# protolambda/go-kzg

Measured on AMD Instinct MI355X. Metric: KZG commitments/sec (CommitToPoly, 4096-element blob); FK20 half: value_fk20_4096, higher is better.
Workload: dtype u32; 1 GPU; CommitToPoly, 4096-coeff blobs, eth/trusted_setup.json monomial setup (s=1337), 4096 blobs/step/GPU resident in HBM, fixed-base table budget 110 GB (library default 110 GB: signed 16-bit windows, 8 of them walked by both GLV halves of every scalar, 103 GB; see table_sweep); global_batch=4096, parallelism=dp1 (independent blobs, no data-path collective)

## Files before the change

### go-kzg_amd/__init__.py

```python
import ctypes as C
import os

import numpy as np

_HERE = os.path.dirname(os.path.abspath(__file__))
LIB_PATH = os.environ.get("KZG_HIP_LIB") or os.path.join(_HERE, "libkzg_hip.so")

OK, ERR_TOO_WIDE, ERR_NOT_POW2, ERR_LEN_MISMATCH, ERR_UPPER_HALF, ERR_BAD_ARG, ERR_BAD_POINT, ERR_NO_DEVICE, ERR_HIP, ERR_UNSUPPORTED, ERR_RECOVERY, ERR_BAD_BLOB = range(12)


class KzgError(Exception):

    def __init__(self, status, msg=""):
        super().__init__("kzg_hip status %d %s" % (status, msg))
        self.status = status


class KzgPanic(KzgError):
    """The reference panics (kzg.go:22-27,44-52,74-91; fk20_single.go:60-62,140-154; bls_kilic.go:133-135)."""


class NoDeviceError(KzgError):
    pass


_lib = None


def lib():
    global _lib
    if _lib is not None:
        return _lib
    if not os.path.exists(LIB_PATH):
        raise ImportError("libkzg_hip.so is not built (run __graft_entry__.build()); there is no CPU fallback: " + LIB_PATH)
    if os.environ.get("KZG_HIP_NO_TORCH_PRELOAD") != "1":
        try:
            import torch
        except ImportError:
            pass
    L = C.CDLL(LIB_PATH)
    vp, u64, i32, u32 = C.c_void_p, C.c_uint64, C.c_int, C.c_uint
    pp = C.POINTER(C.c_void_p)
    sig = {
        "kzg_hip_device_count": (i32, []), "kzg_hip_last_error": (C.c_char_p, []), "kzg_hip_version": (C.c_char_p, []),
        "kzg_hip_host_register": (i32, [vp, u64]), "kzg_hip_host_unregister": (i32, [vp]),
        "kzg_hip_fft_settings_new": (i32, [i32, u32, pp]), "kzg_hip_fft_settings_free": (None, [vp]),
        "kzg_hip_fft_max_width": (u64, [vp]), "kzg_hip_fft_roots": (i32, [vp, i32, vp]),
        "kzg_hip_fft_fr": (i32, [vp, vp, u64, i32, vp, C.POINTER(u64)]), "kzg_hip_inplace_fft_fr": (i32, [vp, vp, vp, u64, i32]),
        "kzg_hip_fft_fr_batch": (i32, [vp, vp, u64, u64, i32, vp]), "kzg_hip_fft_g1": (i32, [vp, vp, u64, i32, vp]),
        "kzg_hip_fft_g1_batch": (i32, [vp, vp, u64, u64, i32, vp]), "kzg_hip_multi_fft_g1_batch": (i32, [vp, vp, u64, u64, i32, vp]),
        "kzg_hip_das_fft_extension": (i32, [vp, vp, u64]), "kzg_hip_das_fft_extension_batch": (i32, [vp, vp, u64, u64]),
        "kzg_hip_fft_fr_batch_dev": (i32, [vp, vp, u64, u64, i32, vp, vp]), "kzg_hip_fft_g1_batch_dev": (i32, [vp, vp, u64, u64, i32, vp, vp]),
        "kzg_hip_das_fft_extension_batch_dev": (i32, [vp, vp, u64, u64, vp]),
        "kzg_hip_fr_from_le32": (i32, [vp, vp, u64, vp, C.POINTER(i32)]), "kzg_hip_fr_to_le32": (i32, [vp, vp, u64, vp]),
        "kzg_hip_lincomb_g1": (i32, [vp, vp, vp, u64, vp]),
        "kzg_hip_points_new": (i32, [vp, vp, u64, pp]), "kzg_hip_points_free": (None, [vp]), "kzg_hip_points_count": (u64, [vp]),
        "kzg_hip_points_set_table_budget_gb": (i32, [vp, C.c_double]),
        "kzg_hip_lincomb_points": (i32, [vp, vp, u64, vp]), "kzg_hip_lincomb_points_batch": (i32, [vp, vp, u64, u64, vp]),
        "kzg_hip_lincomb_points_batch_dev": (i32, [vp, vp, u64, u64, vp, vp]), "kzg_hip_g1_to_compressed": (i32, [vp, vp, u64, vp]),
        "kzg_hip_g1_from_compressed": (i32, [vp, vp, u64, vp]), "kzg_hip_g1_mul_vec": (i32, [vp, vp, vp, u64, vp]),
        "kzg_hip_generate_testing_setup_g1": (i32, [vp, vp, u64, vp]),
        "kzg_hip_g1_marshal_text": (i32, [vp, vp, u64, vp]), "kzg_hip_g1_unmarshal_text": (i32, [vp, C.c_char_p, u64, vp]),
        "kzg_hip_trusted_setup_from_json": (i32, [vp, C.c_char_p, u64, vp, vp, u64, C.POINTER(u64), C.POINTER(u64)]),
        "kzg_hip_kzg_set_table_budget_gb": (i32, [vp, C.c_double]),
        "kzg_hip_kzg_settings_new": (i32, [vp, vp, u64, pp]), "kzg_hip_kzg_settings_free": (None, [vp]),
        "kzg_hip_commit_to_poly": (i32, [vp, vp, u64, vp]), "kzg_hip_commit_to_poly_batch": (i32, [vp, vp, u64, u64, vp]),
        "kzg_hip_commit_to_poly_batch_dev": (i32, [vp, vp, u64, u64, vp, vp]),
        "kzg_hip_compute_proof_single": (i32, [vp, vp, u64, u64, vp]),
        "kzg_hip_compute_proof_single_batch": (i32, [vp, vp, u64, u64, vp, vp]),
        "kzg_hip_compute_proof_single_batch_dev": (i32, [vp, vp, u64, u64, vp, vp, vp]),
        "kzg_hip_compute_proof_multi": (i32, [vp, vp, u64, u64, u64, vp]),
        "kzg_hip_check_proof_multi_interpolation": (i32, [vp, vp, u64, vp, vp, vp]),
        "kzg_hip_g2_from_compressed": (i32, [vp, vp, u64, vp]), "kzg_hip_pairings_verify_batch": (i32, [vp, vp, vp, vp, vp, u64, vp]),
        "kzg_hip_g2_mul_generator_vec": (i32, [vp, vp, u64, vp]), "kzg_hip_generate_testing_setup_g2": (i32, [vp, vp, u64, vp]),
        "kzg_hip_g2_to_compressed": (i32, [vp, vp, u64, vp]),
        "kzg_hip_trusted_setup_g2_from_json": (i32, [vp, C.c_char_p, u64, vp, u64, C.POINTER(u64)]),
        "kzg_hip_test_g2_table_builds": (i32, [vp, C.POINTER(u64)]),
        "kzg_hip_kzg_set_secret_g2": (i32, [vp, vp, u64]), "kzg_hip_check_proof_single_batch": (i32, [vp, vp, vp, vp, vp, u64, vp]),
        "kzg_hip_check_proof_multi_batch": (i32, [vp, vp, vp, vp, vp, u64, u64, vp]),
        "kzg_hip_check_proof_single_batch_combined": (i32, [vp, vp, vp, vp, vp, u64, vp, vp]),
        "kzg_hip_eth_verify_kzg_proof_batch_combined": (i32, [vp, vp, vp, vp, vp, u64, vp, vp]),
        "kzg_hip_test_combine_points": (i32, [vp, vp, vp, vp, vp, u64, vp, vp, vp]), "kzg_hip_test_combine_stats": (i32, [C.POINTER(u64)]),
        "kzg_hip_eth_set_setup_g2": (i32, [vp, vp, u64]), "kzg_hip_eth_verify_kzg_proof_batch": (i32, [vp, vp, vp, vp, vp, u64, vp]),
        "kzg_hip_eth_verify_aggregate_kzg_proof_batch": (i32, [vp, vp, vp, vp, vp, u64, vp, vp, vp, vp]),
        "kzg_hip_eth_kzg_to_versioned_hash_batch": (i32, [vp, vp, u64, vp]), "kzg_hip_eth_kzg_to_versioned_hash_batch_dev": (i32, [vp, vp, u64, vp]),
        "kzg_hip_eth_point_evaluation_precompile_batch": (i32, [vp, vp, u64, vp]),
        "kzg_hip_eth_point_evaluation_precompile_batch_dev": (i32, [vp, vp, u64, vp]),
        "kzg_hip_eth_precompile_return_value": (i32, [vp, vp]),
        "kzg_hip_eth_verify_kzg_commitments_against_transactions_batch": (i32, [vp, vp, vp, vp, vp, vp, u64, vp]),
        "kzg_hip_test_sha256_lanes": (i32, [vp, vp, vp, vp, u64, vp]), "kzg_hip_test_hash_to_bls_field_lanes": (i32, [vp, vp, u64, vp]),
        "kzg_hip_pairing_test": (i32, [vp, vp, vp, u64, vp]),
        "kzg_hip_pairing_test_wave": (i32, [vp, vp, vp, u64, vp]), "kzg_hip_test_wave_fp12_op": (i32, [vp, i32, vp, vp, u64, vp]),
        "kzg_hip_test_pairing_route": (i32, [u64, C.POINTER(u64)]),
        "kzg_hip_toeplitz_part2": (i32, [vp, vp, vp, u64, vp]), "kzg_hip_toeplitz_part3": (i32, [vp, vp, u64, vp]),
        "kzg_hip_fk20_single_settings_new": (i32, [vp, u64, pp]), "kzg_hip_fk20_single_settings_free": (None, [vp]),
        "kzg_hip_fk20_single_x_ext_fft": (i32, [vp, vp]), "kzg_hip_fk20_single": (i32, [vp, vp, u64, vp]),
        "kzg_hip_fk20_single_batch": (i32, [vp, vp, u64, u64, vp]), "kzg_hip_fk20_single_batch_dev": (i32, [vp, vp, u64, u64, vp, vp]),
        "kzg_hip_fk20_single_da_optimized": (i32, [vp, vp, u64, vp]), "kzg_hip_da_using_fk20": (i32, [vp, vp, u64, vp]),
        "kzg_hip_da_using_fk20_batch": (i32, [vp, vp, u64, u64, vp]), "kzg_hip_da_using_fk20_batch_dev": (i32, [vp, vp, u64, u64, vp, vp]),
        "kzg_hip_fk20_multi_settings_new": (i32, [vp, u64, u64, pp]), "kzg_hip_fk20_multi_settings_free": (None, [vp]),
        "kzg_hip_fk20_multi": (i32, [vp, vp, u64, vp]), "kzg_hip_fk20_multi_da_optimized": (i32, [vp, vp, u64, vp]),
        "kzg_hip_da_using_fk20_multi": (i32, [vp, vp, u64, vp]),
        "kzg_hip_da_using_fk20_multi_batch_dev": (i32, [vp, vp, u64, u64, vp, vp]),
        "kzg_hip_fk20_multi_hext_slice_dev": (i32, [vp, vp, u64, u64, u64, vp, vp]),
        "kzg_hip_fk20_multi_finish_dev": (i32, [vp, vp, i32, vp, vp]),
        "kzg_hip_eth_settings_new": (i32, [vp, vp, u64, pp]), "kzg_hip_eth_settings_free": (None, [vp]),
        "kzg_hip_eth_blob_to_kzg_commitment_batch": (i32, [vp, vp, u64, vp, vp]),
        "kzg_hip_eth_compute_kzg_proof": (i32, [vp, vp, u64, vp, vp, vp]),
        "kzg_hip_eth_compute_kzg_proof_batch": (i32, [vp, vp, u64, u64, vp, vp, vp, vp]),
        "kzg_hip_eth_compute_kzg_proof_batch_dev": (i32, [vp, vp, u64, u64, vp, vp, vp, vp, vp]),
        "kzg_hip_eth_compute_aggregate_kzg_proof": (i32, [vp, vp, u64, vp, vp]),
        "kzg_hip_eth_compute_aggregate_kzg_proof_batch": (i32, [vp, vp, vp, u64, vp, vp, vp]),
        "kzg_hip_eth_compute_aggregate_kzg_proof_batch_dev": (i32, [vp, vp, vp, u64, vp, vp, vp]),
        "kzg_hip_test_eth_prove_chunks": (u64, []),
        "kzg_hip_eth_compute_aggregated_poly_and_commitment": (i32, [vp, vp, vp, u64, vp, vp, vp, vp]),
        "kzg_hip_test_sha256": (None, [vp, u64, vp]),
        "kzg_hip_evaluate_poly_in_evaluation_form": (i32, [vp, vp, u64, vp, u32, vp]),
        "kzg_hip_eth_evaluate_polynomial_in_evaluation_form": (i32, [vp, vp, u64, vp, vp]),
        "kzg_hip_bench_threads_fft_fr": (i32, [vp, vp, u64, u64, u32, u32, vp, C.POINTER(C.c_double)]),
        "kzg_hip_bench_drop_in_eth_proof": (i32, [vp, vp, u64, u64, u32, u32, vp, C.POINTER(C.c_double)]),
        "kzg_hip_zero_poly_via_multiplication": (i32, [vp, vp, u64, u64, vp, vp]),
        "kzg_hip_recover_poly_from_samples": (i32, [vp, vp, vp, u64, vp]),
        "kzg_hip_recover_poly_from_samples_batch": (i32, [vp, vp, vp, u64, u64, u64, vp, vp]),
        "kzg_hip_recover_poly_from_samples_batch_dev": (i32, [vp, vp, vp, u64, u64, u64, vp, vp, vp]),
        "kzg_hip_zero_poly_via_multiplication_batch": (i32, [vp, vp, vp, u64, u64, vp, vp, vp]),
        "kzg_hip_calibrate": (i32, [vp, C.POINTER(C.c_double), C.POINTER(C.c_double), C.POINTER(C.c_double)]),
        "kzg_hip_bench_drop_in": (i32, [vp, i32, vp, u64, u64, u32, u32, vp, C.POINTER(C.c_double)]),
        "kzg_hip_coalesce_stats": (i32, [vp, i32, C.POINTER(u64)]),
        "kzg_hip_lincomb_promotions": (i32, [vp, C.POINTER(u64), C.POINTER(u64)]),
        "kzg_hip_test_fp_inv": (i32, [vp, vp, u64, vp, vp, C.POINTER(C.c_double), C.POINTER(C.c_double)]),
        "kzg_hip_test_fr_inv": (i32, [vp, vp, u64, vp, vp, vp]),
        "kzg_hip_test_g1_fft_plan": (i32, [vp, u64, u64, u64, i32, vp]),
        "kzg_hip_test_g1_fft_stage": (i32, [vp, vp, u64, u64, u64, i32, i32, i32, i32, vp, vp]),
        "kzg_hip_test_g1_fft_direct": (i32, [vp, vp, u64, u64, u64, i32, u32, i32, u64, vp]),
        "kzg_hip_kzg_table_info": (i32, [vp, C.POINTER(C.c_uint32), C.POINTER(C.c_uint32), C.POINTER(u64)]), "kzg_hip_kzg_table_additions": (u32, [vp]), "kzg_hip_kzg_set_projective_outputs": (i32, [vp, i32]),
        "kzg_hip_da_using_fk20_multi_batch": (i32, [vp, vp, u64, u64, vp]),
        "kzg_hip_multi_settings_new": (i32, [C.POINTER(i32), u32, u32, vp, u64, pp]), "kzg_hip_multi_settings_free": (None, [vp]),
        "kzg_hip_multi_device_count": (u32, [vp]), "kzg_hip_multi_device": (i32, [vp, u32]),
        "kzg_hip_multi_fft": (vp, [vp, u32]), "kzg_hip_multi_kzg": (vp, [vp, u32]),
        "kzg_hip_multi_transport": (C.c_char_p, [vp]), "kzg_hip_multi_transport_note": (C.c_char_p, [vp]), "kzg_hip_multi_transport_check": (C.c_char_p, [vp]), "kzg_hip_multi_exchanges": (u64, [vp]),
        "kzg_hip_multi_set_fft_sharding": (i32, [vp, i32]), "kzg_hip_multi_set_table_budget_gb": (i32, [vp, C.c_double]),
        "kzg_hip_multi_commit_to_poly_batch": (i32, [vp, vp, u64, u64, vp]),
        "kzg_hip_multi_compute_proof_single_batch": (i32, [vp, vp, u64, u64, vp, vp]),
        "kzg_hip_multi_fft_fr_batch": (i32, [vp, vp, u64, u64, i32, vp]), "kzg_hip_multi_das_fft_extension_batch": (i32, [vp, vp, u64, u64]),
        "kzg_hip_multi_eth_settings_new": (i32, [vp, vp, u64, pp]), "kzg_hip_multi_eth_settings_free": (None, [vp]),
        "kzg_hip_multi_eth_blob_to_kzg_commitment_batch": (i32, [vp, vp, u64, vp, vp]),
        "kzg_hip_multi_eth_compute_kzg_proof_batch": (i32, [vp, vp, u64, u64, vp, vp, vp, vp]),
        "kzg_hip_multi_fk20_single_settings_new": (i32, [vp, u64, pp]), "kzg_hip_multi_fk20_single_settings_free": (None, [vp]),
        "kzg_hip_multi_da_using_fk20_batch": (i32, [vp, vp, u64, u64, vp]), "kzg_hip_multi_da_using_fk20": (i32, [vp, vp, u64, vp]),
        "kzg_hip_multi_fk20_multi_settings_new": (i32, [vp, u64, u64, pp]), "kzg_hip_multi_fk20_multi_settings_free": (None, [vp]),
        "kzg_hip_multi_da_using_fk20_multi_batch": (i32, [vp, vp, u64, u64, vp]), "kzg_hip_multi_da_using_fk20_multi": (i32, [vp, vp, u64, vp]),
        "kzg_hip_bench_poly_lincomb_dev": (i32, [vp, vp, u64, vp, u64, u64, vp, vp]),
        "kzg_hip_prof_reset": (None, [vp, i32]), "kzg_hip_prof_read": (i32, [vp, C.c_char_p, C.POINTER(C.c_double), C.POINTER(u64)]),
    }
    for name, (res, args) in sig.items():
        if os.environ.get("KZG_HIP_LIB_ALLOW_MISSING") and not hasattr(L, name):
            continue
        f = getattr(L, name)
        f.restype, f.argtypes = res, args
    _lib = L
    return L


API_SYMBOLS = None


def device_count():
    return lib().kzg_hip_device_count()


class pinned:

    def __init__(self, array):
        self.a = array

    def __enter__(self):
        _chk(lib().kzg_hip_host_register(self.a.ctypes.data, self.a.nbytes))
        return self.a

    def __exit__(self, *exc):
        lib().kzg_hip_host_unregister(self.a.ctypes.data)
        return False


_ERR_STATUS = (ERR_TOO_WIDE, ERR_NOT_POW2)


def _chk(st, error_ok=False):
    if st == OK:
        return
    msg = ""
    if st == ERR_HIP:
        msg = lib().kzg_hip_last_error().decode()
    if st == ERR_NO_DEVICE:
        raise NoDeviceError(st, "no gfx950 device visible (the HIP path is the only path)")
    if error_ok and st in _ERR_STATUS:
        raise KzgError(st, msg)
    raise KzgPanic(st, msg)


def _p(a):
    return a.ctypes.data_as(C.c_void_p)


def _fr(a):
    a = np.ascontiguousarray(a, dtype=np.uint64)
    return a.reshape(-1, 4)


def _g1(a):
    a = np.ascontiguousarray(a, dtype=np.uint64)
    return a.reshape(-1, 3, 6)


def _g2(a):
    a = np.ascontiguousarray(a, dtype=np.uint64)
    return a.reshape(-1, 3, 2, 6)


def _seed32(seed):
    if seed is None:
        return None
    seed = bytes(seed)
    if len(seed) != 32:
        raise KzgError(ERR_LEN_MISMATCH, "a seed is 32 bytes")
    return C.c_char_p(seed)


def combine_stats():
    out = (C.c_uint64 * 6)()
    _chk(lib().kzg_hip_test_combine_stats(out))
    return {"route": "combined" if out[0] else "per_row", "groups": int(out[1]), "failed": int(out[2]), "rechecked": int(out[3]),
            "combine_from": int(out[4]), "rows": int(out[5])}


def pairing_route(n):
    out = (C.c_uint64 * 2)()
    _chk(lib().kzg_hip_test_pairing_route(n, out))
    return ("wave" if out[0] else "lane"), int(out[1])


def g2_empty(n):
    return np.zeros((n, 3, 2, 6), dtype=np.uint64)


def fr_empty(n):
    return np.zeros((n, 4), dtype=np.uint64)


def g1_empty(n):
    return np.zeros((n, 3, 6), dtype=np.uint64)


class FFTSettings:

    def __init__(self, max_scale, device=0):
        h = C.c_void_p()
        _chk(lib().kzg_hip_fft_settings_new(device, max_scale, C.byref(h)))
        self.h, self.max_scale, self.max_width, self.device = h, max_scale, 1 << max_scale, device

    def close(self):
        if getattr(self, "h", None):
            lib().kzg_hip_fft_settings_free(self.h)
            self.h = None

    def expanded_roots_of_unity(self):
        out = fr_empty(self.max_width + 1)
        _chk(lib().kzg_hip_fft_roots(self.h, 0, _p(out)))
        return out

    def reverse_roots_of_unity(self):
        out = fr_empty(self.max_width + 1)
        _chk(lib().kzg_hip_fft_roots(self.h, 1, _p(out)))
        return out

    def fft(self, vals, inv=False):
        vals = _fr(vals)
        n = vals.shape[0]
        if n > self.max_width:
            raise KzgError(ERR_TOO_WIDE)
        np2 = 1 if n == 0 else 1 << (n - 1).bit_length()
        out, on = fr_empty(np2), C.c_uint64(0)
        _chk(lib().kzg_hip_fft_fr(self.h, _p(vals), n, int(inv), _p(out), C.byref(on)), error_ok=True)
        return out

    def inplace_fft(self, vals, inv=False):
# ... 889 lines not shown
```

### go-kzg_amd/csrc/capi_core.hip

```cpp
#include "capi_common.hpp"
#include <map>

thread_local std::string g_last_error;


int kzg_hip_device_count(void) {
    int n = 0;
    if (hipGetDeviceCount(&n) != hipSuccess) return 0;
    int ok = 0;
    for (int i = 0; i < n; i++) {
        hipDeviceProp_t pr;
        if (hipGetDeviceProperties(&pr, i) == hipSuccess && strncmp(pr.gcnArchName, "gfx950", 6) == 0) ok++;
    }
    return ok;
}
const char *kzg_hip_last_error(void) { return g_last_error.c_str(); }
const char *kzg_hip_version(void) { return "kzg_hip 0.1 (gfx950)"; }

static fr scale2_root_of_unity(unsigned k) {
    uint32_t e[8]; uint32_t br = 0;
    for (int i = 0; i < 8; i++) e[i] = subb(FrP::mod(i), i == 0 ? 1u : 0u, br);
    for (unsigned s = 0; s < k; s++)
        for (int i = 0; i < 8; i++) e[i] = (e[i] >> 1) | (i < 7 ? e[i + 1] << 31 : 0);
    fr seven = fr_from_u64(7), acc = one<FrP>();
// ... 207 lines not shown
uint32_t g1_fft_direct_logr(uint64_t n, uint64_t batch) {
    if (const knobs::g1_fft_mode forced = knobs::g1_fft(); forced != knobs::g1_fft_mode::by_size) return forced == knobs::g1_fft_mode::direct ? 4u : 0u;
    if (n < 2) return 0;
    const uint64_t unit = device_simd_lanes() / 16;
    if (g1_quad_enabled()) return n * batch <= unit ? 4 : 0;
    if (n * batch <= 2 * unit) return 4;
    if (n * batch <= 4 * unit) return 3;
    return 0;
}
bool g1_fft_direct_mode(uint64_t n, uint64_t batch) { return g1_fft_direct_logr(n, batch) != 0; }
int g1_fft_direct_lanes(uint64_t n, uint64_t batch) {
    if (!g1_quad_enabled() || !knobs::g1_direct_coop()) return 1;
    const uint64_t items = (n * batch) << g1_fft_direct_logr(n, batch);
    const uint64_t one_round = device_simd_lanes();
    return items * 4 <= one_round ? 4 : items * 2 <= one_round ? 2 : 1;
}
int g1_fft_rows(kzg_hip_fft *fs, hipStream_t s, const g1j *d_in, uint64_t in_stride, uint64_t n_valid, g1j *d_data, uint64_t n, uint64_t batch, int inv,
                       const fr *scale, uint64_t n_out) {
    if (g1_fft_direct_mode(n, batch)) {
        dtmp<g1j> d_tmp(s);
        CHK(d_tmp.alloc(n * batch));
        launch_g1_fft_direct(s, d_in, in_stride, n_valid, d_data, d_tmp.p, n, batch, inv ? fs->d_reversed : fs->d_expanded, fs->W, scale, g1_fft_direct_logr(n, batch),
                             g1_fft_direct_lanes(n, batch), 0, n_out);
        return KZG_HIP_OK;
    }
    launch_g1_bitrev_copy(s, d_in, in_stride, n_valid, d_data, n, batch);
    const fr *roots = inv ? fs->d_glv_reversed : fs->d_glv_expanded;
    const int8_t *wnaf = inv ? fs->d_wnaf_reversed : fs->d_wnaf_expanded;
    for (uint64_t m = 1; m < n; m <<= 1) launch_g1_fft_stage(s, d_data, n, batch, m, roots, wnaf, fs->W);
    if (scale) launch_g1_mul_vec(s, d_data, n * batch, scale, 0, n * batch, d_data);
    return KZG_HIP_OK;
}

int kzg_hip_fft_g1(kzg_hip_fft *fs, const void *vals_g1, uint64_t n, int inv, void *out_g1) {
    if (!fs) return KZG_HIP_ERR_BAD_ARG;
    if (n > fs->W) return KZG_HIP_ERR_TOO_WIDE;
    if (!is_pow2(n)) return KZG_HIP_ERR_NOT_POW2;
    if (n == 0 || !vals_g1 || !out_g1) return KZG_HIP_ERR_BAD_ARG;
    stream_lease lease(fs);
    hipStream_t s = lease.s;
    dtmp<g1j> d_in(s), d_data(s);
    CHK(d_in.alloc(n)); CHK(d_data.alloc(n));
    HIPCHK(hipMemcpyAsync(d_in.p, vals_g1, n * sizeof(g1j), hipMemcpyHostToDevice, s));
    launch_g1_from_kilic(s, d_in.p, n);
    CHK(g1_fft_rows(fs, s, d_in.p, n, n, d_data.p, n, 1, inv, inv ? fs->d_inv_pow2 + ilog2(n) : nullptr));
    launch_g1_normalize(s, d_data.p, d_in.p, n, true);
    std::swap(d_in.p, d_data.p);
    HIPCHK(hipGetLastError());
    HIPCHK(hipMemcpyAsync(out_g1, d_data.p, n * sizeof(g1j), hipMemcpyDeviceToHost, s));
    HIPCHK(hipStreamSynchronize(s));
    return KZG_HIP_OK;
}

int das_ext_rows(kzg_hip_fft *fs, hipStream_t s, fr *d, uint64_t n, uint64_t batch) {
    const bool long_or_short = n >= fr4::N || n <= 64;
    if (2 * n == fs->W && long_or_short && fr_fft_lazy_sizes(n, batch) && fs->d_tw4096[0]) {
        dtmp<fr> d_c(s);
        CHK(d_c.alloc(n * batch));
        fr_fft_rows(fs, s, d, n, n, d_c.p, n, batch, 1);
        launch_fr_mul_table_rows(s, d_c.p, fs->d_expanded, 1, n, batch);
        fr_fft_rows(fs, s, d_c.p, n, n, d, n, batch, 0);
        return KZG_HIP_OK;
    }
    launch_das_ext(s, d, n, batch, fs->d_expanded, fs->d_reversed, fs->W, fs->d_inv_pow2 + ilog2(n), fs->d_tw_das2048);
    return KZG_HIP_OK;
}

int kzg_hip_das_fft_extension_batch(kzg_hip_fft *fs, void *vals_fr, uint64_t n, uint64_t batch) {
    if (!fs || !vals_fr) return KZG_HIP_ERR_BAD_ARG;
    if (n * 2 > fs->W) return KZG_HIP_ERR_TOO_WIDE;
    if (n < 2 || !is_pow2(n)) return KZG_HIP_ERR_BAD_ARG;
    if (!batch) return KZG_HIP_OK;
    stream_lease lease(fs);
    hipStream_t s = lease.s;
    void *dp = nullptr;
    uint8_t *hp = n <= 4096 ? lease.pinned(n * batch * sizeof(fr), &dp) : nullptr;
    if (hp) {
        memcpy(hp, vals_fr, n * batch * sizeof(fr));
        CHK(das_ext_rows(fs, s, (fr *)dp, n, batch));
        HIPCHK(hipGetLastError());
        HIPCHK(hipStreamSynchronize(s));
        memcpy(vals_fr, hp, n * batch * sizeof(fr));
        return KZG_HIP_OK;
    }
    dtmp<fr> d(s);
    CHK(d.alloc(n * batch));
    HIPCHK(hipMemcpyAsync(d.p, vals_fr, n * batch * sizeof(fr), hipMemcpyHostToDevice, s));
    CHK(das_ext_rows(fs, s, d.p, n, batch));
    HIPCHK(hipGetLastError());
    HIPCHK(hipMemcpyAsync(vals_fr, d.p, n * batch * sizeof(fr), hipMemcpyDeviceToHost, s));
    HIPCHK(hipStreamSynchronize(s));
    return KZG_HIP_OK;
}
int kzg_hip_fft_fr_batch_dev(kzg_hip_fft *fs, const void *d_vals_fr, uint64_t n, uint64_t batch, int inv, void *d_out_fr, void *stream) {
    if (!fs) return KZG_HIP_ERR_BAD_ARG;
    if (n > fs->W) return KZG_HIP_ERR_TOO_WIDE;
    if (!is_pow2(n)) return KZG_HIP_ERR_NOT_POW2;
    if (n == 0 || batch == 0) return KZG_HIP_OK;
    if (!d_vals_fr || !d_out_fr) return KZG_HIP_ERR_BAD_ARG;
    dev_select sel(fs);
    fr_fft_rows(fs, (hipStream_t)stream, (const fr *)d_vals_fr, n, n, (fr *)d_out_fr, n, batch, inv);
    HIPCHK(hipGetLastError());
    return KZG_HIP_OK;
}
int kzg_hip_fft_g1_batch(kzg_hip_fft *fs, const void *vals_g1, uint64_t n, uint64_t batch, int inv, void *out_g1) {
    if (!fs) return KZG_HIP_ERR_BAD_ARG;
    if (n > fs->W) return KZG_HIP_ERR_TOO_WIDE;
    if (!is_pow2(n)) return KZG_HIP_ERR_NOT_POW2;
    if (n == 0 || !vals_g1 || !out_g1) return KZG_HIP_ERR_BAD_ARG;
    if (!batch) return KZG_HIP_OK;
    stream_lease lease(fs);
    hipStream_t s = lease.s;
    dtmp<g1j> d_in(s), d_data(s);
    CHK(d_in.alloc(n * batch)); CHK(d_data.alloc(n * batch));
    HIPCHK(hipMemcpyAsync(d_in.p, vals_g1, n * batch * sizeof(g1j), hipMemcpyHostToDevice, s));
    launch_g1_from_kilic(s, d_in.p, n * batch);
    CHK(g1_fft_rows(fs, s, d_in.p, n, n, d_data.p, n, batch, inv, inv ? fs->d_inv_pow2 + ilog2(n) : nullptr));
    launch_g1_normalize(s, d_data.p, d_in.p, n * batch, true);
    HIPCHK(hipGetLastError());
    HIPCHK(hipMemcpyAsync(out_g1, d_in.p, n * batch * sizeof(g1j), hipMemcpyDeviceToHost, s));
    HIPCHK(hipStreamSynchronize(s));
    return KZG_HIP_OK;
}
int kzg_hip_fft_g1_batch_dev(kzg_hip_fft *fs, const void *d_vals_g1, uint64_t n, uint64_t batch, int inv, void *d_out_g1, void *stream) {
    if (!fs) return KZG_HIP_ERR_BAD_ARG;
    if (n > fs->W) return KZG_HIP_ERR_TOO_WIDE;
    if (!is_pow2(n)) return KZG_HIP_ERR_NOT_POW2;
    if (n == 0 || !d_vals_g1 || !d_out_g1) return KZG_HIP_ERR_BAD_ARG;
    if (!batch) return KZG_HIP_OK;
    dev_select sel(fs);
    hipStream_t s = (hipStream_t)stream;
    dtmp<g1j> d_in(s), d_data(s);
    CHK(d_in.alloc(n * batch)); CHK(d_data.alloc(n * batch));
    HIPCHK(hipMemcpyAsync(d_in.p, d_vals_g1, n * batch * sizeof(g1j), hipMemcpyDeviceToDevice, s));
    launch_g1_from_kilic(s, d_in.p, n * batch);
    CHK(g1_fft_rows(fs, s, d_in.p, n, n, d_data.p, n, batch, inv, inv ? fs->d_inv_pow2 + ilog2(n) : nullptr));
    launch_g1_normalize(s, d_data.p, (g1j *)d_out_g1, n * batch, true);
    HIPCHK(hipGetLastError());
    return KZG_HIP_OK;
}
static void put_stage_plan(const g1_stage_plan &p, uint32_t *out) { out[0] = (uint32_t)p.lanes; out[1] = p.wnaf ? 1u : 0u; out[2] = p.rows ? 1u : 0u; }
static bool g1_stage_shape_ok(kzg_hip_fft *fs, uint64_t n, uint64_t batch, uint64_t m) {
    return n >= 2 && n <= fs->W && is_pow2(n) && m >= 1 && m <= n / 2 && is_pow2(m) && batch >= 1 && batch <= (1ull << 32) / n;
}
int kzg_hip_test_g1_fft_plan(kzg_hip_fft *fs, uint64_t n, uint64_t batch, uint64_t m, int dif, uint32_t out[5]) {
    if (!fs || !out || !g1_stage_shape_ok(fs, n, batch, m)) return KZG_HIP_ERR_BAD_ARG;
    dev_select sel(fs);
    put_stage_plan(g1_fft_stage_plan(n, batch, m, dif != 0), out);
    out[3] = g1_fft_direct_logr(n, batch);
    out[4] = (uint32_t)g1_fft_direct_lanes(n, batch);
    return KZG_HIP_OK;
}
int kzg_hip_test_g1_fft_stage(kzg_hip_fft *fs, const void *pts_g1, uint64_t n, uint64_t batch, uint64_t m, int inv, int dif, int lanes, int mul, void *out_g1, uint32_t plan_out[3]) {
    if (!fs || !pts_g1 || !out_g1 || !g1_stage_shape_ok(fs, n, batch, m)) return KZG_HIP_ERR_BAD_ARG;
    if ((lanes != 0 && lanes != 1 && lanes != 2 && lanes != 4) || mul < 0 || mul > 2) return KZG_HIP_ERR_BAD_ARG;
    stream_lease lease(fs);
    hipStream_t s = lease.s;
    const g1_stage_plan plan = g1_fft_stage_plan(n, batch, m, dif != 0, lanes == 0 ? -1 : lanes == 1 ? 0 : lanes == 4 ? 1 : 2,
                                                 mul == 1 ? knobs::g1_mul_mode::regular : mul == 2 ? knobs::g1_mul_mode::wnaf : knobs::g1_mul_mode::by_shape);
    if (plan_out) put_stage_plan(plan, plan_out);
    dtmp<g1j> d_data(s), d_out(s);
    CHK(d_data.alloc(n * batch)); CHK(d_out.alloc(n * batch));
    HIPCHK(hipMemcpyAsync(d_data.p, pts_g1, n * batch * sizeof(g1j), hipMemcpyHostToDevice, s));
    launch_g1_from_kilic(s, d_data.p, n * batch);
    launch_g1_fft_stage_planned(s, plan, dif != 0, d_data.p, n, batch, m, inv ? fs->d_glv_reversed : fs->d_glv_expanded, inv ? fs->d_wnaf_reversed : fs->d_wnaf_expanded, fs->W);
    launch_g1_normalize(s, d_data.p, d_out.p, n * batch, true);
    HIPCHK(hipGetLastError());
    HIPCHK(hipMemcpyAsync(out_g1, d_out.p, n * batch * sizeof(g1j), hipMemcpyDeviceToHost, s));
    HIPCHK(hipStreamSynchronize(s));
    return KZG_HIP_OK;
}
int kzg_hip_test_g1_fft_direct(kzg_hip_fft *fs, const void *pts_g1, uint64_t n, uint64_t n_valid, uint64_t batch, int inv, uint32_t max_logr, int lanes, uint64_t n_out, void *out_g1) {
    if (!fs || !pts_g1 || !out_g1 || n < 2 || n > fs->W || !is_pow2(n) || !n_valid || n_valid > n || n_out > n || batch < 1 || batch > (1ull << 28) / n) return KZG_HIP_ERR_BAD_ARG;
    if (max_logr < 1 || max_logr > 4 || (lanes != 1 && lanes != 2 && lanes != 4)) return KZG_HIP_ERR_BAD_ARG;
    stream_lease lease(fs);
    hipStream_t s = lease.s;
    dtmp<g1j> d_in(s), d_data(s), d_tmp(s), d_out(s);
    CHK(d_in.alloc(n_valid * batch)); CHK(d_data.alloc(n * batch)); CHK(d_tmp.alloc(n * batch)); CHK(d_out.alloc(n * batch));
    HIPCHK(hipMemcpyAsync(d_in.p, pts_g1, n_valid * batch * sizeof(g1j), hipMemcpyHostToDevice, s));
    launch_g1_from_kilic(s, d_in.p, n_valid * batch);
    HIPCHK(hipMemsetAsync(d_data.p, 0, n * batch * sizeof(g1j), s));
    launch_g1_fft_direct(s, d_in.p, n_valid, n_valid, d_data.p, d_tmp.p, n, batch, inv ? fs->d_reversed : fs->d_expanded, fs->W, inv ? fs->d_inv_pow2 + ilog2(n) : nullptr, max_logr,
                         lanes, 0, n_out, true);
    launch_g1_normalize(s, d_data.p, d_out.p, n * batch, true);
    HIPCHK(hipGetLastError());
    HIPCHK(hipMemcpyAsync(out_g1, d_out.p, n * batch * sizeof(g1j), hipMemcpyDeviceToHost, s));
    HIPCHK(hipStreamSynchronize(s));
    return KZG_HIP_OK;
}
int kzg_hip_das_fft_extension_batch_dev(kzg_hip_fft *fs, void *d_vals_fr, uint64_t n, uint64_t batch, void *stream) {
    if (!fs || !d_vals_fr) return KZG_HIP_ERR_BAD_ARG;
    if (n * 2 > fs->W) return KZG_HIP_ERR_TOO_WIDE;
    if (n < 2 || !is_pow2(n)) return KZG_HIP_ERR_BAD_ARG;
    if (!batch) return KZG_HIP_OK;
    dev_select sel(fs);
    CHK(das_ext_rows(fs, (hipStream_t)stream, (fr *)d_vals_fr, n, batch));
    HIPCHK(hipGetLastError());
    return KZG_HIP_OK;
}
int kzg_hip_das_fft_extension(kzg_hip_fft *fs, void *vals_fr, uint64_t n) { return kzg_hip_das_fft_extension_batch(fs, vals_fr, n, 1); }

msm_plan classic_plan(uint64_t n, bool folded) {
    msm_plan p{};
    p.c = 8; p.nwin = 16; p.nb = 128; p.ngroups = folded ? 8 : 16; p.fixed = 0; p.table_n = n;
    return p;
}
void set_inf_image(void *out_g1) { g1j z = g1_to_kilic(g1_inf()); memcpy(out_g1, &z, sizeof z); }

__global__ __launch_bounds__(128, 2) void k_points_shift64(const g1a *pts, uint64_t n, g1j *out) {
    uint64_t t = blockIdx.x * (uint64_t)blockDim.x + threadIdx.x;
    if (t >= n) return;
    g1a p = pts[t];
    if (is_inf(p)) { out[t] = g1_inf(); return; }
    g1jq q = g1jq_unpack(to_jac(p));
#pragma nounroll
    for (int i = 0; i < 64; i++) q = g1jq_dbl(q);
    out[t] = g1jq_pack(q);
}
void kzg_hip_points_free(kzg_hip_points *pts) {
    if (!pts) return;
    hipSetDevice(pts->fs->device);
    hipDeviceSynchronize();
    pts->co.reset();
    if (pts->ks) kzg_hip_kzg_settings_free(pts->ks);
    hipFree(pts->d_tab);
    (void)hipGetLastError();
    delete pts;
}
int kzg_hip_points_new(kzg_hip_fft *fs, const void *points_g1, uint64_t n, kzg_hip_points **out) {
    if (!fs || !out || (n && !points_g1)) return KZG_HIP_ERR_BAD_ARG;
    *out = nullptr;
    KZG_TRY
    std::unique_ptr<kzg_hip_points, void (*)(kzg_hip_points *)> own(new kzg_hip_points, kzg_hip_points_free);
    own->fs = fs; own->n = n;
    if (n) {
        dev_guard g(fs);
        hipStream_t s = fs->stream;
        dtmp<g1j> d_raw(s), d_hi(s);
        CHK(d_raw.alloc(n)); CHK(d_hi.alloc(n));
        HIPCHK(hipMalloc((void **)&own->d_tab, 2 * n * sizeof(g1a)));
        HIPCHK(hipMemcpyAsync(d_raw.p, points_g1, n * sizeof(g1j), hipMemcpyHostToDevice, s));
        launch_g1_from_kilic(s, d_raw.p, n);
        launch_g1_to_affine(s, d_raw.p, own->d_tab, n);
        hipLaunchKernelGGL(k_points_shift64, dim3((uint32_t)((n + 127) / 128)), dim3(128), 0, s, own->d_tab, n, d_hi.p);
        launch_g1_to_affine(s, d_hi.p, own->d_tab + n, n);
        HIPCHK(hipGetLastError());
        HIPCHK(hipStreamSynchronize(s));
    }
    if (n >= 64) {
        CHK(kzg_settings_build(fs, points_g1, n, &own->ks));
        own->ks->budget_gb = table_budget_gb(knobs::points_fb_budget_gb(), 32.0, 24.0);
    }
    *out = own.release();
    return KZG_HIP_OK;
    KZG_CATCH
}
int kzg_hip_points_set_table_budget_gb(kzg_hip_points *pts, double gb) {
    if (!pts) return KZG_HIP_ERR_BAD_ARG;
    if (!pts->ks) return KZG_HIP_OK;
    return kzg_hip_kzg_set_table_budget_gb(pts->ks, gb);
}
uint64_t kzg_hip_points_count(const kzg_hip_points *pts) { return pts ? pts->n : 0; }
int lincomb_points_rows(kzg_hip_points *pts, hipStream_t s, const fr *d_sc, uint64_t n, uint64_t batch, g1j *d_out, uint64_t sc_stride, bool holds_mu) {
    if (pts->ks) {
        if (holds_mu) CHK(ensure_fixed_table(pts->ks, s));
        else { dev_guard g(pts->fs); CHK(ensure_fixed_table(pts->ks, s)); }
        std::shared_lock<std::shared_mutex> tl(pts->ks->tab_mu);
        if (pts->ks->d_fixed) return commit_rows(pts->ks, s, d_sc, n, batch, d_out, sc_stride ? sc_stride : n);
    }
    msm_plan p = classic_plan(pts->n, true);
    if (!msm_index_range_ok(p, n)) return KZG_HIP_ERR_TOO_WIDE;
    dtmp<uint8_t> d_ws(s);
    CHK(d_ws.alloc(msm_workspace_bytes(p, n, batch)));
    launch_msm(s, p, pts->d_tab, d_sc, sc_stride ? sc_stride : n, n, batch, d_ws.p, d_out, true);
    HIPCHK(hipGetLastError());
    return KZG_HIP_OK;
}
int kzg_hip_lincomb_points_batch_dev(kzg_hip_points *pts, const void *d_scalars_fr, uint64_t n, uint64_t batch, void *d_out_g1, void *stream) {
    if (!pts || !d_out_g1) return KZG_HIP_ERR_BAD_ARG;
    if (n > pts->n) return KZG_HIP_ERR_LEN_MISMATCH;
    if (!batch) return KZG_HIP_OK;
    if (n == 0 || !d_scalars_fr) return KZG_HIP_ERR_BAD_ARG;
    hipSetDevice(pts->fs->device);
    return lincomb_points_rows(pts, (hipStream_t)stream, (const fr *)d_scalars_fr, n, batch, (g1j *)d_out_g1);
}
int kzg_hip_lincomb_points_batch(kzg_hip_points *pts, const void *scalars_fr, uint64_t n, uint64_t batch, void *out_g1) {
    if (!pts || !out_g1) return KZG_HIP_ERR_BAD_ARG;
    if (n > pts->n) return KZG_HIP_ERR_LEN_MISMATCH;
    if (!batch) return KZG_HIP_OK;
    if (n == 0) { for (uint64_t b = 0; b < batch; b++) set_inf_image((uint8_t *)out_g1 + b * sizeof(g1j)); return KZG_HIP_OK; }
    if (!scalars_fr) return KZG_HIP_ERR_BAD_ARG;
    stream_lease lease(pts->fs);
    hipStream_t s = lease.s;
    dtmp<fr> d_sc(s); dtmp<g1j> d_out(s);
    CHK(d_sc.alloc(n * batch)); CHK(d_out.alloc(batch));
    HIPCHK(hipMemcpyAsync(d_sc.p, scalars_fr, n * batch * sizeof(fr), hipMemcpyHostToDevice, s));
    CHK(lincomb_points_rows(pts, s, d_sc.p, n, batch, d_out.p, 0, lease.fallback.owns_lock()));
    HIPCHK(hipMemcpyAsync(out_g1, d_out.p, batch * sizeof(g1j), hipMemcpyDeviceToHost, s));
    HIPCHK(hipStreamSynchronize(s));
    return KZG_HIP_OK;
}
int kzg_hip_lincomb_points(kzg_hip_points *pts, const void *scalars_fr, uint64_t n, void *out_g1) {
    if (pts && scalars_fr && out_g1 && n && n <= pts->n) return lincomb_points_coalesced(pts, scalars_fr, n, out_g1);
    return kzg_hip_lincomb_points_batch(pts, scalars_fr, n, 1, out_g1);
}

struct lincomb_promo {
    static constexpr int SLOTS = 6, LINCOMB_PROMO_SETS = 2;
    struct entry {
        uint64_t n = 0, fp = 0, last_use = 0; uint32_t sightings = 0;
        std::shared_ptr<const std::vector<uint8_t>> copy;
        std::shared_ptr<kzg_hip_points> set;
        bool building = false;
    };
    std::mutex mu; std::condition_variable built;
    entry e[SLOTS];
    uint64_t tick = 0, promoted = 0;
    std::atomic<uint64_t> served{0};
// ... 204 lines not shown
```

### go-kzg_amd/csrc/capi_fk20.hip

```cpp
#include "capi_common.hpp"

__global__ void k_fk20_x(const g1j *secret, uint64_t n, uint64_t l, uint64_t k, g1j *x ) {
    uint64_t t = blockIdx.x * (uint64_t)blockDim.x + threadIdx.x;
    if (t >= l * k) return;
    uint64_t off = t / k, i = t % k;
    x[t] = (i + 1 < k) ? secret[n - l - 1 - off - i * l] : g1_inf();
}

static int fk20_core_new(kzg_hip_kzg *ks, uint64_t n2, uint64_t l, fk20_core *c) {
    kzg_hip_fft *fs = ks->fs;
    dev_guard g(fs);
    hipStream_t s = fs->stream;
    uint64_t n = n2 / 2, k = n / l, k2 = 2 * k;
    c->ks = ks; c->n2 = n2; c->l = l; c->k = k;
    dtmp<g1j> d_x(s), d_f(s);
    CHK(d_x.alloc(l * k)); CHK(d_f.alloc(l * k2));
    HIPCHK(hipMalloc((void **)&c->d_files, l * k2 * sizeof(g1j)));
    hipLaunchKernelGGL(k_fk20_x, dim3((uint32_t)((l * k + 255) / 256)), dim3(256), 0, s, ks->d_secret, n, l, k, d_x.p);
    CHK(g1_fft_rows(fs, s, d_x.p, k, k, d_f.p, k2, l, 0));
    launch_g1_normalize(s, d_f.p, c->d_files, l * k2);
    HIPCHK(hipGetLastError());
    {
        double budget_gb = table_budget_gb(knobs::fk20_fb_budget_gb(), 48.0, 12.0);
        uint64_t npts = l * k2;
        const bool glv = fb_glv_enabled();
        dtmp<g1a> d_fa(s);
        if (npts >= 64) { CHK(d_fa.alloc(npts)); launch_g1_to_affine(s, c->d_files, d_fa.p, npts); }
        for (uint32_t cc = glv ? 16 : 14; cc >= 4 && npts >= 64; cc--) {
            const uint32_t nwin = glv ? fb_windows_glv(cc) : fb_windows(cc);
            if (glv && cc > 4 && fb_windows_glv(cc - 1) == nwin) continue;
            double bytes = (double)nwin * (double)npts * (double)(1u << (cc - 1)) * sizeof(g1a);
            if (bytes > budget_gb * 1e9) continue;
            g1a *tab = nullptr;
            if (hipMalloc((void **)&tab, (size_t)nwin * npts * (1u << (cc - 1)) * sizeof(g1a)) != hipSuccess) { (void)hipGetLastError(); continue; }
            hipError_t e = launch_fb_build(s, d_fa.p, npts, cc, nwin, tab);
            if (e == hipSuccess) e = hipStreamSynchronize(s);
            if (e != hipSuccess) { (void)hipGetLastError(); hipFree(tab); continue; }
            c->d_files_fb = tab; c->fb_c = cc; c->fb_nwin = nwin; c->fb_glv = glv;
            break;
        }
    }
    HIPCHK(hipStreamSynchronize(s));
    return KZG_HIP_OK;
}

int fk20_hext(fk20_core *c, hipStream_t s, const fr *d_poly, uint64_t poly_stride, uint64_t n, uint64_t batch, uint64_t j0, uint64_t cnt, g1j *d_hext) {
    kzg_hip_fft *fs = c->ks->fs;
    uint64_t l = c->l, k2 = 2 * c->k;
    dtmp<fr> d_tc(s), d_cf(s);
    CHK(d_tc.alloc(batch * l * k2)); CHK(d_cf.alloc(batch * l * k2));
    launch_toeplitz_coeffs(s, d_poly, poly_stride, n, l, batch, d_tc.p, fs->d_inv_pow2 + ilog2(k2));
    fr_fft_rows(fs, s, d_tc.p, k2, k2, d_cf.p, k2, batch * l, 0);
    if (c->d_files_fb) {
        if (l == 1) launch_fb_mul_vec(s, c->d_files_fb, l * k2, c->fb_c, c->fb_nwin, d_cf.p, k2, j0, cnt, batch, d_hext, c->fb_glv);
        else if (batch * cnt >= device_simd_lanes()) launch_fb_mul_vec_files(s, c->d_files_fb, l * k2, c->fb_c, c->fb_nwin, d_cf.p, k2, j0, cnt, batch, d_hext, c->fb_glv);
        else {
            dtmp<g1j> d_tmp(s);
            CHK(d_tmp.alloc(batch * l * cnt));
            launch_fb_mul_vec(s, c->d_files_fb, l * k2, c->fb_c, c->fb_nwin, d_cf.p, k2, j0, cnt, batch, d_tmp.p, c->fb_glv);
            launch_g1_sum_files(s, d_tmp.p, l, cnt, batch, d_hext);
        }
    } else if (l == 1 && j0 == 0 && cnt == k2) launch_g1_mul_vec(s, c->d_files, k2, d_cf.p, 1, batch * k2, d_hext);
    else HIPCHK(launch_g1_file_msm(s, c->d_files, d_cf.p, l, k2, j0, cnt, batch, d_hext));
    HIPCHK(hipGetLastError());
    return KZG_HIP_OK;
}
static int fk20_finish_from_h(fk20_core *c, hipStream_t s, g1j *d_h, uint64_t batch, int da, int bit_reverse, g1j *d_out) {
    kzg_hip_fft *fs = c->ks->fs;
    uint64_t k = c->k, k2 = 2 * k, on = da ? k2 : k;
    dtmp<g1j> d_b(s);
    CHK(d_b.alloc(batch * k2));
    CHK(g1_fft_rows(fs, s, d_h, k2, k, d_b.p, on, batch, 0));
    if (bit_reverse) { launch_g1_bitrev_copy(s, d_b.p, on, on, d_h, on, batch); launch_g1_normalize(s, d_h, d_out, batch * on, true); }
    else launch_g1_normalize(s, d_b.p, d_out, batch * on, true);
    HIPCHK(hipGetLastError());
    return KZG_HIP_OK;
}
int fk20_finish(fk20_core *c, hipStream_t s, const g1j *d_hext, uint64_t batch, int da, int bit_reverse, g1j *d_out) {
    kzg_hip_fft *fs = c->ks->fs;
    const uint64_t k2 = 2 * c->k;
    dtmp<g1j> d_a(s);
    CHK(d_a.alloc(batch * k2));
    CHK(g1_fft_rows(fs, s, d_hext, k2, k2, d_a.p, k2, batch, 1, nullptr, c->k));
    return fk20_finish_from_h(c, s, d_a.p, batch, da, bit_reverse, d_out);
}
static bool fk20_pass1_fused_ok(const fk20_core *c, uint64_t batch) {
    const uint64_t k2 = 2 * c->k;
    return knobs::fk20_pass1() && c->l == 1 && c->d_files_fb && k2 >= 32 && g1_fft_direct_mode(k2, batch) && g1_fft_direct_logr(k2, batch) == 4;
}
static int fk20_run_pass1_fused(fk20_core *c, hipStream_t s, const fr *d_poly, uint64_t poly_stride, uint64_t n, uint64_t batch, int da, int bit_reverse, g1j *d_out) {
    kzg_hip_fft *fs = c->ks->fs;
    const uint64_t k2 = 2 * c->k;
    dtmp<fr> d_tc(s), d_cf(s); dtmp<g1j> d_p1(s), d_a(s), d_tmp(s);
    CHK(d_tc.alloc(batch * k2)); CHK(d_cf.alloc(batch * k2)); CHK(d_p1.alloc(batch * k2)); CHK(d_a.alloc(batch * k2)); CHK(d_tmp.alloc(batch * k2));
    launch_toeplitz_coeffs(s, d_poly, poly_stride, n, 1, batch, d_tc.p, fs->d_inv_pow2 + ilog2(k2));
    fr_fft_rows(fs, s, d_tc.p, k2, k2, d_cf.p, k2, batch, 0);
    launch_fb_direct_pass1(s, c->d_files_fb, k2, c->fb_c, c->fb_nwin, d_cf.p, fs->d_reversed, fs->W, batch, 4, d_p1.p, c->fb_glv);
    launch_g1_fft_direct(s, d_p1.p, k2, k2, d_a.p, d_tmp.p, k2, batch, fs->d_reversed, fs->W, nullptr, 4, g1_fft_direct_lanes(k2, batch), 4, c->k);
    HIPCHK(hipGetLastError());
    return fk20_finish_from_h(c, s, d_a.p, batch, da, bit_reverse, d_out);
}
static bool fk20_fused_ok(const fk20_core *c, uint64_t batch, int da) {
    const uint64_t k2 = 2 * c->k;
    return knobs::fk20_fuse() && c->l == 1 && c->d_files_fb && k2 >= 8 && !g1_fft_direct_mode(k2, batch) && (da || !g1_fft_direct_mode(c->k, batch));
}
static int fk20_run_fused(fk20_core *c, hipStream_t s, const fr *d_poly, uint64_t poly_stride, uint64_t n, uint64_t batch, int da, int bit_reverse, g1j *d_out) {
    kzg_hip_fft *fs = c->ks->fs;
    const uint64_t k2 = 2 * c->k;
    dtmp<fr> d_tc(s), d_cf(s); dtmp<g1j> d_a(s), d_b(s);
    CHK(d_tc.alloc(batch * k2)); CHK(d_cf.alloc(batch * k2)); CHK(d_a.alloc(batch * k2)); CHK(d_b.alloc(batch * k2));
    launch_toeplitz_coeffs(s, d_poly, poly_stride, n, 1, batch, d_tc.p, fs->d_inv_pow2 + ilog2(k2));
    fr_fft_rows(fs, s, d_tc.p, k2, k2, d_cf.p, k2, batch, 0);
    launch_fb_mul_vec_dif2(s, c->d_files_fb, k2, c->fb_c, c->fb_nwin, d_cf.p, fs->d_reversed, fs->W, batch, d_a.p, c->fb_glv);
    for (uint64_t m = k2 / 8; m >= 1; m >>= 1) launch_g1_fft_stage_dif(s, d_a.p, k2, batch, m, fs->d_glv_reversed, fs->d_wnaf_reversed, fs->W);
    if (!da) {
        const uint64_t k = c->k;
        launch_g1_take_even(s, d_a.p, d_b.p, batch * k);
        for (uint64_t m = 1; m < k; m <<= 1) launch_g1_fft_stage(s, d_b.p, k, batch, m, fs->d_glv_expanded, fs->d_wnaf_expanded, fs->W);
        if (bit_reverse) { launch_g1_bitrev_copy(s, d_b.p, k, k, d_a.p, k, batch); launch_g1_normalize(s, d_a.p, d_out, batch * k, true); }
        else launch_g1_normalize(s, d_b.p, d_out, batch * k, true);
        HIPCHK(hipGetLastError());
        return KZG_HIP_OK;
    }
    launch_g1_clear_odd(s, d_a.p, batch * k2);
    for (uint64_t m = 1; m < k2; m <<= 1) launch_g1_fft_stage(s, d_a.p, k2, batch, m, fs->d_glv_expanded, fs->d_wnaf_expanded, fs->W);
    if (bit_reverse) { launch_g1_bitrev_copy(s, d_a.p, k2, k2, d_b.p, k2, batch); launch_g1_normalize(s, d_b.p, d_out, batch * k2, true); }
    else launch_g1_normalize(s, d_a.p, d_out, batch * k2, true);
    HIPCHK(hipGetLastError());
    return KZG_HIP_OK;
}
static uint64_t fk20_padded_batch(uint64_t batch) {
    if (!knobs::fk20_pad()) return batch;
    if (batch > 16 && batch < 32) return 32;
    if (batch > 32 && (batch & 7)) {
        const uint64_t p = (batch + 7) & ~7ull;
        if ((p - batch) * 32 <= batch) return p;
    }
    return batch;
}
int fk20_run_dev(fk20_core *c, hipStream_t s, const fr *d_poly, uint64_t poly_stride, uint64_t n, uint64_t batch, int da, int bit_reverse, g1j *d_out) {
    if (const uint64_t padded = fk20_padded_batch(batch); padded != batch) {
        const uint64_t on = da ? 2 * c->k : c->k;
        dtmp<fr> d_p2(s); dtmp<g1j> d_o2(s);
        CHK(d_p2.alloc(padded * n)); CHK(d_o2.alloc(padded * on));
        HIPCHK(hipMemcpy2DAsync(d_p2.p, n * sizeof(fr), d_poly, poly_stride * sizeof(fr), n * sizeof(fr), batch, hipMemcpyDeviceToDevice, s));
        for (uint64_t b = batch; b < padded; b++)
            HIPCHK(hipMemcpyAsync(d_p2.p + b * n, d_poly + (batch - 1) * poly_stride, n * sizeof(fr), hipMemcpyDeviceToDevice, s));
        if (fk20_fused_ok(c, padded, da)) CHK(fk20_run_fused(c, s, d_p2.p, n, n, padded, da, bit_reverse, d_o2.p));
        else {
            dtmp<g1j> d_hext(s);
            CHK(d_hext.alloc(padded * 2 * c->k));
            CHK(fk20_hext(c, s, d_p2.p, n, n, padded, 0, 2 * c->k, d_hext.p));
            CHK(fk20_finish(c, s, d_hext.p, padded, da, bit_reverse, d_o2.p));
        }
        HIPCHK(hipMemcpyAsync(d_out, d_o2.p, batch * on * sizeof(g1j), hipMemcpyDeviceToDevice, s));
        return KZG_HIP_OK;
    }
    if (fk20_fused_ok(c, batch, da)) return fk20_run_fused(c, s, d_poly, poly_stride, n, batch, da, bit_reverse, d_out);
    if (fk20_pass1_fused_ok(c, batch)) return fk20_run_pass1_fused(c, s, d_poly, poly_stride, n, batch, da, bit_reverse, d_out);
    uint64_t k2 = 2 * c->k;
    dtmp<g1j> d_hext(s);
    CHK(d_hext.alloc(batch * k2));
    CHK(fk20_hext(c, s, d_poly, poly_stride, n, batch, 0, k2, d_hext.p));
    return fk20_finish(c, s, d_hext.p, batch, da, bit_reverse, d_out);
}
static int fk20_run_host(fk20_core *c, const void *poly_fr, uint64_t row_len, uint64_t n, uint64_t batch, int check_upper, int da, int bit_reverse, void *out_g1) {
    kzg_hip_fft *fs = c->ks->fs;
    dev_guard g(fs);
    hipStream_t s = fs->stream;
    uint64_t on = da ? 2 * c->k : c->k;
    dtmp<fr> d_poly(s); dtmp<g1j> d_out(s); dtmp<uint32_t> d_flag(s);
    CHK(d_poly.alloc(batch * row_len)); CHK(d_out.alloc(batch * on)); CHK(d_flag.alloc(1));
    HIPCHK(hipMemcpyAsync(d_poly.p, poly_fr, batch * row_len * sizeof(fr), hipMemcpyHostToDevice, s));
    if (check_upper) {
        HIPCHK(hipMemsetAsync(d_flag.p, 0, 4, s));
        launch_fr_any_nonzero(s, d_poly.p + n, row_len - n, d_flag.p);
        uint32_t flag = 0;
        HIPCHK(hipMemcpyAsync(&flag, d_flag.p, 4, hipMemcpyDeviceToHost, s));
        HIPCHK(hipStreamSynchronize(s));
        if (flag) return KZG_HIP_ERR_UPPER_HALF;
    }
    CHK(fk20_run_dev(c, s, d_poly.p, row_len, n, batch, da, bit_reverse, d_out.p));
    return d2h_staged(c->ks->fs, s, out_g1, d_out.p, batch * on * sizeof(g1j));
}

int kzg_hip_fk20_single_settings_new(kzg_hip_kzg *ks, uint64_t n2, kzg_hip_fk20s **out) {
    if (!ks || !out) return KZG_HIP_ERR_BAD_ARG;
    *out = nullptr;
    if (n2 > ks->fs->W) return KZG_HIP_ERR_TOO_WIDE;
    if (!is_pow2(n2)) return KZG_HIP_ERR_NOT_POW2;
    if (n2 < 2) return KZG_HIP_ERR_BAD_ARG;
    kzg_hip_fk20s *fk = new kzg_hip_fk20s;
    int st = fk20_core_new(ks, n2, 1, &fk->c);
    if (st) { kzg_hip_fk20_single_settings_free(fk); return st; }
    *out = fk;
    return KZG_HIP_OK;
}
void kzg_hip_fk20_single_settings_free(kzg_hip_fk20s *fk) {
    if (!fk) return;
    if (fk->c.ks) { hipSetDevice(fk->c.ks->fs->device); hipDeviceSynchronize(); }
    hipFree(fk->c.d_files); hipFree(fk->c.d_files_fb);
    (void)hipGetLastError();
    delete fk;
}
int kzg_hip_fk20_single_x_ext_fft(const kzg_hip_fk20s *fk, void *out_g1) {
    if (!fk || !out_g1) return KZG_HIP_ERR_BAD_ARG;
    kzg_hip_fft *fs = fk->c.ks->fs;
    dev_guard g(fs);
    hipStream_t s = fs->stream;
    dtmp<g1j> d_tmp(s);
    CHK(d_tmp.alloc(fk->c.n2));
    launch_g1_normalize(s, fk->c.d_files, d_tmp.p, fk->c.n2, true);
    HIPCHK(hipGetLastError());
    HIPCHK(hipMemcpyAsync(out_g1, d_tmp.p, fk->c.n2 * sizeof(g1j), hipMemcpyDeviceToHost, s));
    HIPCHK(hipStreamSynchronize(s));
    return KZG_HIP_OK;
}
int kzg_hip_fk20_single(kzg_hip_fk20s *fk, const void *poly_fr, uint64_t n, void *out_g1) {
    if (!fk || !poly_fr || !out_g1) return KZG_HIP_ERR_BAD_ARG;
    if (2 * n != fk->c.n2) return KZG_HIP_ERR_LEN_MISMATCH;
    return fk20_run_host(&fk->c, poly_fr, n, n, 1, 0, 0, 0, out_g1);
}
int kzg_hip_fk20_single_batch(kzg_hip_fk20s *fk, const void *poly_fr, uint64_t n, uint64_t batch, void *out_g1) {
    if (!fk || !poly_fr || !out_g1) return KZG_HIP_ERR_BAD_ARG;
    if (2 * n != fk->c.n2) return KZG_HIP_ERR_LEN_MISMATCH;
    if (!batch) return KZG_HIP_OK;
    return fk20_run_host(&fk->c, poly_fr, n, n, batch, 0, 0, 0, out_g1);
}
int kzg_hip_fk20_single_batch_dev(kzg_hip_fk20s *fk, const void *d_poly_fr, uint64_t n, uint64_t batch, void *d_out_g1, void *stream) {
    if (!fk || !d_poly_fr || !d_out_g1) return KZG_HIP_ERR_BAD_ARG;
    if (2 * n != fk->c.n2) return KZG_HIP_ERR_LEN_MISMATCH;
    if (!batch) return KZG_HIP_OK;
    dev_guard g(fk->c.ks->fs);
    return fk20_run_dev(&fk->c, (hipStream_t)stream, (const fr *)d_poly_fr, n, n, batch, 0, 0, (g1j *)d_out_g1);
}
int kzg_hip_fk20_single_da_optimized(kzg_hip_fk20s *fk, const void *poly_fr, uint64_t n2, void *out_g1) {
    if (!fk || !poly_fr || !out_g1) return KZG_HIP_ERR_BAD_ARG;
    if (n2 > fk->c.ks->fs->W) return KZG_HIP_ERR_TOO_WIDE;
    if (!is_pow2(n2)) return KZG_HIP_ERR_NOT_POW2;
    if (n2 != fk->c.n2) return KZG_HIP_ERR_LEN_MISMATCH;
    return fk20_run_host(&fk->c, poly_fr, n2, n2 / 2, 1, 1, 1, 0, out_g1);
}
int kzg_hip_da_using_fk20_batch(kzg_hip_fk20s *fk, const void *poly_fr, uint64_t n, uint64_t batch, void *out_g1) {
    if (!fk || !poly_fr || !out_g1) return KZG_HIP_ERR_BAD_ARG;
    if (n > fk->c.ks->fs->W / 2) return KZG_HIP_ERR_TOO_WIDE;
    if (!is_pow2(n)) return KZG_HIP_ERR_NOT_POW2;
    if (2 * n != fk->c.n2) return KZG_HIP_ERR_LEN_MISMATCH;
    if (!batch) return KZG_HIP_OK;
    return fk20_run_host(&fk->c, poly_fr, n, n, batch, 0, 1, 1, out_g1);
}
static int fk20_da_coalesced(fk20_core *c, const void *poly_fr, uint64_t n, void *out_g1) {
    KZG_TRY
    const uint64_t on = 2 * c->k;
    coalescer *co = get_coalescer(c->ks->fs, c->co_da, n * sizeof(fr), on * sizeof(g1j), 48);
    auto exec = [c, co, n, on](coalesce_buf &b, uint64_t batch) -> int {
        hipSetDevice(c->ks->fs->device);
        hipStream_t s = b.stream;
        drain_on_exit drain(s);
        dtmp<fr> d_poly(s); dtmp<g1j> d_out(s);
// ... 101 lines not shown
```

### go-kzg_amd/csrc/g1_coop_kernels.hpp

```cpp
#pragma once
#include "internal.hpp"
#include "g1_quad.hpp"

namespace kzg {

#ifndef G1_BLOCK
#define G1_BLOCK 256
#endif
struct g1jq_slot { uint32_t w[39]; uint32_t inf; uint32_t pad; };
#define G1_DIRECT_BLOCK 64

template <bool DIF, bool WNAF, int L> __global__ __launch_bounds__(G1_BLOCK, 2) void k_g1_fft_stage_quad(g1j *data, uint32_t logn, uint64_t m, const fr *roots, const int8_t *wnaf, uint64_t W, uint64_t total, uint64_t batch) {
    const uint64_t t4 = blockIdx.x * (uint64_t)blockDim.x + threadIdx.x;
    const uint32_t role = (uint32_t)(t4 & (uint64_t)(L - 1));
    const uint64_t t = t4 / L;
    if (t >= total) return;
    const uint64_t half = 1ull << (logn - 1), groups = half / m;
    const uint64_t j = t / (groups * batch), rem = t % (groups * batch), b = rem / groups, g = rem % groups;
    g1j *row = data + (b << logn);
    const uint64_t i0 = g * 2 * m + j, i1 = i0 + m;
    g1j y = row[i1];
    g1j x = row[i0];
    const uint64_t ti = j * (W / (2 * m));
    const fr kk = roots[ti];
    glv_halves h;
#pragma unroll
    for (int i = 0; i < 4; i++) { h.k1[i] = kk.l[i]; h.k2[i] = kk.l[4 + i]; }
    h.neg1 = h.neg2 = 0;
    g1aq tbl[8]; fq dz[7]; g1j packed;
#define QMUL(pq, res) (WNAF ? g1_mul_glv_wnaf_quad<L>((pq), kk, tbl, dz, wnaf + ti * KZG_WNAF_ROW, (res), packed, role) : g1_mul_glv_regular_quad<L>((pq), h, tbl, dz, (res), packed, role))
    if (!DIF) {
        g1jq yq; int st = is_inf(y) ? 0 : 1;
        if (st == 1) {
            if (j) {
                st = QMUL(g1jq_unpack(y), yq);
                if (st == 2) y = packed; else if (st == 0) y = g1_inf();
            } else yq = g1jq_unpack(y);
        }
        if (st == 1 && !is_inf(x)) {
            g1jq sum, dif;
            if (KZG_LIKELY(g1jq_addsub(g1jq_unpack(x), yq, sum, dif))) {
                if (role == 0) {
                    fp z3 = packq(sum.z);
                    g1j o0, o1;
                    o0.x = packq(sum.x); o0.y = packq(sum.y); o0.z = z3;
                    o1.x = packq(dif.x); o1.y = packq(dif.y); o1.z = z3;
                    row[i0] = o0; row[i1] = o1;
                }
                return;
            }
        }
        if (st == 1) y = g1jq_pack(yq);
        if (role == 0) { row[i0] = g1_add(x, y); row[i1] = g1_add(x, g1_neg(y)); }
    } else {
        if (!is_inf(x) && !is_inf(y)) {
            g1jq sum, dif;
            if (KZG_LIKELY(g1jq_addsub(g1jq_unpack(x), g1jq_unpack(y), sum, dif))) {
                g1j o0; o0.x = packq(sum.x); o0.y = packq(sum.y); o0.z = packq(sum.z);
                g1j o1;
                if (j) {
                    g1jq dq;
                    const int st = QMUL(dif, dq);
                    o1 = st == 1 ? g1jq_pack(dq) : st == 2 ? packed : g1_inf();
                } else { o1.x = packq(dif.x); o1.y = packq(dif.y); o1.z = o0.z; }
                if (role == 0) { row[i0] = o0; row[i1] = o1; }
                return;
            }
        }
        g1j s_ = g1_add(x, y), d_ = g1_add(x, g1_neg(y));
        if (j && !is_inf(d_)) {
            g1jq dq;
            const int st = QMUL(g1jq_unpack(d_), dq);
            d_ = st == 1 ? g1jq_pack(dq) : st == 2 ? packed : g1_inf();
        }
        if (role == 0) { row[i0] = s_; row[i1] = d_; }
    }
}
#undef QMUL
template <bool DIF> static inline void launch_stage_coop(hipStream_t s, int lanes, bool wn, g1j *data, uint64_t n, uint64_t batch, uint64_t m, const fr *roots, const int8_t *wnaf, uint64_t W,
                                                  uint64_t total) {
    static const bool once = [] {
        hipFuncSetAttribute(reinterpret_cast<const void *>(&k_g1_fft_stage_quad<DIF, true, 4>), hipFuncAttributeMaxDynamicSharedMemorySize, 96 * 1024);
        hipFuncSetAttribute(reinterpret_cast<const void *>(&k_g1_fft_stage_quad<DIF, false, 4>), hipFuncAttributeMaxDynamicSharedMemorySize, 96 * 1024);
        hipFuncSetAttribute(reinterpret_cast<const void *>(&k_g1_fft_stage_quad<DIF, true, 2>), hipFuncAttributeMaxDynamicSharedMemorySize, 96 * 1024);
        hipFuncSetAttribute(reinterpret_cast<const void *>(&k_g1_fft_stage_quad<DIF, false, 2>), hipFuncAttributeMaxDynamicSharedMemorySize, 96 * 1024);
        return true; }();
    (void)once;
    const size_t lds = total * lanes <= device_simd_lanes() ? 96 * 1024 : 0;
    const dim3 qg((uint32_t)((lanes * total + G1_BLOCK - 1) / G1_BLOCK));
    const uint32_t logn = ilog2(n);
    if (lanes == 4) {
        if (wn) hipLaunchKernelGGL((k_g1_fft_stage_quad<DIF, true, 4>), qg, dim3(G1_BLOCK), lds, s, data, logn, m, roots, wnaf, W, total, batch);
        else hipLaunchKernelGGL((k_g1_fft_stage_quad<DIF, false, 4>), qg, dim3(G1_BLOCK), lds, s, data, logn, m, roots, wnaf, W, total, batch);
    } else {
        if (wn) hipLaunchKernelGGL((k_g1_fft_stage_quad<DIF, true, 2>), qg, dim3(G1_BLOCK), lds, s, data, logn, m, roots, wnaf, W, total, batch);
        else hipLaunchKernelGGL((k_g1_fft_stage_quad<DIF, false, 2>), qg, dim3(G1_BLOCK), lds, s, data, logn, m, roots, wnaf, W, total, batch);
    }
}
template <int L> __global__ __launch_bounds__(G1_DIRECT_BLOCK, 2) void k_g1_fft_direct_coop(const g1j *in, uint64_t in_stride, uint64_t n_valid, g1j *out, uint32_t logn,
                                                                                          uint32_t logR, uint64_t Ns, const fr *roots, uint64_t W, const fr *scale, uint64_t total,
                                                                                          uint32_t logT, uint32_t logU) {
    __shared__ g1jq_slot buf[G1_DIRECT_BLOCK / L];
    const uint32_t tid = threadIdx.x, role = tid & (uint32_t)(L - 1), item = tid / L;
    const uint64_t t = (blockIdx.x * (uint64_t)blockDim.x + tid) / L;
    const uint64_t n = 1ull << logn, R = 1ull << logR, cols = n >> logR, T = 1ull << logT;
    const uint32_t tt = (uint32_t)(t & (T - 1));
    const uint64_t u = (t >> logT) & ((1ull << logU) - 1), jb = t >> (logT + logU), j = jb % cols, b = jb / cols;
    const bool live = t < total;
    g1jq_acc acc; acc.inf = true;
    uint64_t oidx = 0;
    if (live) {
        const uint64_t k = j & (Ns - 1), idx = j + (uint64_t)tt * cols;
        oidx = b * n + (j - k) * R + k + u * Ns;
        g1j x = idx < n_valid ? in[b * in_stride + idx] : g1_inf();
        if (!is_inf(x)) {
            const uint64_t e = ((uint64_t)tt * (cols / Ns) * (Ns * u + k)) & (n - 1);
            if (e == 0 && !scale) { acc.v = g1jq_unpack(x); acc.inf = false; }
            else {
                fr sc = roots[e * (W >> logn)];
                if (scale) sc = mul(sc, *scale);
                g1aq tbl[8]; fq dz[7]; g1j packed;
                const int st = g1_mul_glv_regular_quad<L>(g1jq_unpack(x), glv_split_signed(from_mont<FrP>(sc)), tbl, dz, acc.v, packed, role);
                if (st == 2) { acc.inf = is_inf(packed); if (!acc.inf) acc.v = g1jq_unpack(packed); } else acc.inf = st == 0;
            }
        }
    }
#define COOP_STORE(i) do { _Pragma("unroll") for (int q = 0; q < 13; q++) { buf[i].w[q] = acc.v.x.l[q]; buf[i].w[13 + q] = acc.v.y.l[q]; buf[i].w[26 + q] = acc.v.z.l[q]; } \
                           buf[i].inf = acc.inf ? 1u : 0u; } while (0)
    if (role == 0) COOP_STORE(item);
    __syncthreads();
#pragma nounroll
    for (uint32_t off = (uint32_t)T / 2; off >= 1; off >>= 1) {
        if (role == 0 && tt < off && !buf[item + off].inf) {
            g1jq q;
#pragma unroll
            for (int i = 0; i < 13; i++) { q.x.l[i] = buf[item + off].w[i]; q.y.l[i] = buf[item + off].w[13 + i]; q.z.l[i] = buf[item + off].w[26 + i]; }
            acc.add(q);
            COOP_STORE(item);
        }
        __syncthreads();
    }
#undef COOP_STORE
    if (live && role == 0 && tt == 0) out[oidx] = acc.inf ? g1_inf() : g1jq_pack(acc.v);
}

}
```

### go-kzg_amd/csrc/internal.hpp

```cpp
#pragma once
#include <hip/hip_runtime.h>
#include <stdint.h>
#include "field.hpp"
#include "g1.hpp"
#include "knobs.hpp"

namespace kzg {

inline uint32_t ilog2(uint64_t v) { uint32_t r = 0; while ((1ull << r) < v) r++; return r; }

void launch_fr_fft(hipStream_t s, const fr *in, uint64_t in_stride, uint64_t n_in, fr *out, uint64_t n, uint64_t batch,
                   const fr *roots, uint64_t W, const fr *scale, const uint32_t *tw4096 = nullptr, const fr *roots_l = nullptr);
bool fr_fft_lazy_sizes(uint64_t n, uint64_t batch);
void launch_das_ext(hipStream_t s, fr *vals, uint64_t n, uint64_t batch, const fr *expanded, const fr *reversed, uint64_t W,
                    const fr *inv_n, const uint32_t *tw2048 = nullptr);
void launch_toeplitz_coeffs(hipStream_t s, const fr *poly, uint64_t poly_stride, uint64_t n, uint64_t l, uint64_t batch, fr *out,
                            const fr *scale);
void launch_quotient_linear(hipStream_t s, const fr *poly, uint64_t poly_stride, uint64_t n, uint64_t batch, const fr *x, fr *q, uint64_t q_stride);
void launch_fr_from_u64(hipStream_t s, const uint64_t *in, uint64_t in_stride, fr *out, uint64_t n);
void launch_fr_zero_tails(hipStream_t s, fr *rows, uint64_t n_max, uint64_t batch, const uint64_t *lens, uint64_t lens_stride);
void launch_fr_any_nonzero(hipStream_t s, const fr *vals, uint64_t n, uint32_t *flag);
void launch_fr_powers(hipStream_t s, const fr *base, uint64_t n, fr *out);

void launch_fr_from_le32(hipStream_t s, const uint8_t *in, fr *out, uint64_t per_blob, uint64_t batch, uint32_t *bad);
void launch_fr_to_le32(hipStream_t s, const fr *in, uint8_t *out, uint64_t n);
void launch_fr_bitrev_gather(hipStream_t s, const fr *in, fr *out, uint64_t n);
constexpr uint64_t ZERO_TREE_LEAF = 16;
void launch_zero_leaves(hipStream_t s, const fr *expanded, uint64_t stride, const uint64_t *missing, uint64_t n_missing, uint64_t leaves, fr *a);
void launch_zero_pair_products(hipStream_t s, const fr *f, uint64_t m, uint64_t pairs, fr *out);
void launch_zero_join(hipStream_t s, fr *c, const fr *a, uint64_t d, uint64_t pairs);
void launch_zero_unpad(hipStream_t s, const fr *root, uint64_t pad, uint64_t n_missing, uint64_t length, fr *poly);
void launch_fr_mul_table_rows(hipStream_t s, fr *data, const fr *table, uint64_t stride, uint64_t n, uint64_t batch);
void launch_poly_lincomb(hipStream_t s, const fr *vectors, uint64_t stride, const fr *scalars, uint64_t count, uint64_t n, fr *out);
void launch_eth_quotient(hipStream_t s, const fr *poly, uint64_t poly_stride, const fr *domain, uint64_t n, uint64_t batch, const fr *z, uint64_t z_stride,
                         const fr *inv_n, fr *q, fr *y_out, uint32_t *flag, uint64_t dom_stride = 1, fr *scratch = nullptr);
uint64_t eth_quotient_scratch_elems(uint64_t n, uint64_t batch);

void launch_fr_scale_by_inv_powers(hipStream_t s, fr *c, const fr *x, uint64_t n, fr *xpow_n);

void launch_zero_eval_direct(hipStream_t s, const fr *expanded, uint64_t stride, const uint64_t *missing, uint64_t n_missing, uint64_t length, fr *zero_eval);
void launch_fr_scale_by_powers(hipStream_t s, fr *poly, const fr *base, uint64_t n);
void launch_fr_pointwise(hipStream_t s, const fr *a, const fr *b, const uint8_t *present, fr *out, uint64_t n, int mode, uint32_t *flag);
uint32_t launch_zero_eval_direct_rows_segs(uint64_t length, uint64_t rows, uint64_t nm_hint);
void launch_zero_eval_direct_rows(hipStream_t s, const fr *expanded, uint64_t stride, const uint64_t *missing, uint64_t list_stride, const uint64_t *n_missing, const fr *corr,
                                  uint32_t segs, uint64_t length, uint64_t rows, fr *zero_eval);

void launch_rr_scan(hipStream_t s, const uint8_t *present, uint64_t n, uint64_t rows, uint64_t *list, uint32_t *count, uint64_t *nm);
void launch_rr_corr(hipStream_t s, const uint64_t *nm, uint64_t rows, uint32_t segs, fr *corr);
void launch_rr_shift_bases(hipStream_t s, const fr &inv5, const fr &five, fr *out);
void launch_rr_leaves(hipStream_t s, const fr *expanded, uint64_t stride, const uint64_t *list, uint64_t list_stride, const uint64_t *nm, uint64_t leaves, uint64_t rows, fr *a);
void launch_rr_unpad(hipStream_t s, const fr *root, uint64_t leaves, const uint64_t *nm, uint64_t length, uint64_t rows, fr *poly);
void launch_rr_mask_mul(hipStream_t s, const fr *a, const fr *b, uint64_t b_stride, const uint8_t *present, uint64_t p_stride, uint64_t n, uint64_t rows, fr *out);
void launch_rr_strip_divide(hipStream_t s, const fr *num, const fr *den, fr *out, uint64_t total);
void launch_rr_finish(hipStream_t s, const fr *recon, const fr *samples, const uint8_t *present, uint64_t p_stride, const uint32_t *count, uint64_t c_stride, uint32_t *flag,
                      uint64_t n, uint64_t rows, fr *out, uint8_t *status);

void launch_g1_mul_vec(hipStream_t s, const g1j *pts, uint64_t pts_mod, const fr *scalars, uint64_t s_stride, uint64_t n, g1j *out);
hipError_t launch_g1_file_msm(hipStream_t s, const g1j *files, const fr *scalars, uint64_t nfiles, uint64_t k2, uint64_t j0, uint64_t cnt,
                              uint64_t batch, g1j *out);
void launch_g1_bitrev_copy(hipStream_t s, const g1j *in, uint64_t in_stride, uint64_t n_valid, g1j *out, uint64_t n, uint64_t batch);
void launch_g1_fft_stage(hipStream_t s, g1j *data, uint64_t n, uint64_t batch, uint64_t m, const fr *roots, const int8_t *wnaf, uint64_t W);
struct g1_stage_plan { int lanes; bool wnaf; bool rows; };
g1_stage_plan g1_fft_stage_plan(uint64_t n, uint64_t batch, uint64_t m, bool dif, int quad, knobs::g1_mul_mode mul);
g1_stage_plan g1_fft_stage_plan(uint64_t n, uint64_t batch, uint64_t m, bool dif);
void launch_g1_fft_stage_planned(hipStream_t s, const g1_stage_plan &plan, bool dif, g1j *data, uint64_t n, uint64_t batch, uint64_t m, const fr *roots, const int8_t *wnaf, uint64_t W);
void launch_g1_fft_stage_dif(hipStream_t s, g1j *data, uint64_t n, uint64_t batch, uint64_t m, const fr *roots, const int8_t *wnaf, uint64_t W);
void launch_g1_clear_odd(hipStream_t s, g1j *data, uint64_t n_total);
void launch_g1_take_even(hipStream_t s, const g1j *in, g1j *out, uint64_t total);
bool g1_quad_enabled();
void launch_fb_direct_pass1(hipStream_t s, const g1a *table, uint64_t table_n, uint32_t c, uint32_t nwin, const fr *scalars, const fr *roots, uint64_t W, uint64_t batch,
                            uint32_t logR, g1j *out, bool glv = false);
void launch_g1_stage_coop_dif(hipStream_t s, int lanes, bool wnaf_rows, g1j *data, uint64_t n, uint64_t batch, uint64_t m, const fr *roots, const int8_t *wnaf, uint64_t W, uint64_t total);
void launch_g1_stage_coop_dit(hipStream_t s, int lanes, bool wnaf_rows, g1j *data, uint64_t n, uint64_t batch, uint64_t m, const fr *roots, const int8_t *wnaf, uint64_t W, uint64_t total);
void launch_g1_direct_coop(hipStream_t s, int lanes, uint32_t wgs, size_t pad_lds, const g1j *src, uint64_t src_stride, uint64_t src_valid, g1j *dst, uint32_t logn, uint32_t logR,
                           uint64_t Ns, const fr *roots, uint64_t W, const fr *sc, uint64_t total, uint32_t logT, uint32_t logU);
void launch_g1_fft_direct(hipStream_t s, const g1j *in, uint64_t in_stride, uint64_t n_valid, g1j *data, g1j *tmp, uint64_t n, uint64_t batch, const fr *roots,
                          uint64_t W, const fr *scale, uint32_t max_logr = 4, int lanes = 1, uint32_t bits_done = 0, uint64_t n_out = 0,
                          bool lanes_fixed = false);
void launch_g1_normalize(hipStream_t s, const g1j *in, g1j *out, uint64_t n, bool to_kilic = false);
void launch_fr_inv_test(hipStream_t s, const fr *in, uint64_t n, fr *out_coop, fr *out_lane, fr *out_block);
void launch_fp_inv_both(hipStream_t s, const fp *in, fp *out_coop, fp *out_lane, uint64_t n, int mode);
void launch_g1_from_kilic(hipStream_t s, g1j *data, uint64_t n);
void launch_g1_to_affine(hipStream_t s, const g1j *in, g1a *out, uint64_t n);
void launch_g1_compress(hipStream_t s, const g1j *in, uint8_t *out48, uint64_t n);
void launch_g1_decompress(hipStream_t s, const uint8_t *in48, g1j *out, uint64_t n, uint32_t *bad_flag);
void launch_g1_fixed_base_powers(hipStream_t s, const fr *powers, uint64_t n, g1j *out);

uint64_t device_simd_lanes();
inline uint64_t device_simds() { return device_simd_lanes() / 64; }
struct msm_plan {
    uint32_t c;
    uint32_t nwin;
    uint32_t nb;
    uint32_t ngroups;
    uint32_t fixed;
    uint32_t glv;
    uint64_t table_n;
};
inline bool msm_index_range_ok(const msm_plan &p, uint64_t n) { return n < (1ull << 27) && 2 * p.table_n < (1ull << 30); }
size_t msm_workspace_bytes(const msm_plan &p, uint64_t n, uint64_t batch);
void launch_msm(hipStream_t s, const msm_plan &p, const g1a *table, const fr *scalars, uint64_t sc_stride, uint64_t n, uint64_t batch, void *workspace, g1j *out,
                bool to_kilic, uint64_t table_stride = 0, bool crowded_buckets = false);
void launch_msm_window_table(hipStream_t s, const g1a *pts, uint64_t n, uint32_t c, uint32_t nwin, g1j *tmp, g1a *out);

size_t fb_partials_bytes(uint64_t n, uint64_t batch);
hipError_t launch_fb_build(hipStream_t s, const g1a *pts, uint64_t n, uint32_t c, uint32_t nwin, g1a *table);
void launch_fb_msm(hipStream_t s, const g1a *table, uint64_t table_n, uint32_t c, uint32_t nwin, const fr *scalars, uint64_t sc_stride, uint64_t n,
                   uint64_t batch, void *partials, g1j *out, bool to_kilic, bool glv = false, bool projective = false);

void launch_fb_mul_vec(hipStream_t s, const g1a *table, uint64_t table_n, uint32_t c, uint32_t nwin, const fr *scalars, uint64_t row, uint64_t j0,
                       uint64_t cnt, uint64_t batch, g1j *out, bool glv = false);
void launch_fb_mul_vec_dif2(hipStream_t s, const g1a *table, uint64_t table_n, uint32_t c, uint32_t nwin, const fr *scalars, const fr *roots, uint64_t W,
                            uint64_t batch, g1j *out, bool glv = false);
void launch_fb_mul_vec_files(hipStream_t s, const g1a *table, uint64_t table_n, uint32_t c, uint32_t nwin, const fr *scalars, uint64_t row, uint64_t j0,
                             uint64_t cnt, uint64_t batch, g1j *out, bool glv = false);
void launch_g1_sum_files(hipStream_t s, const g1j *tmp, uint64_t nfiles, uint64_t cnt, uint64_t batch, g1j *out);

struct g2j; struct g2_prepared;
void launch_g2_from_compressed(hipStream_t s, const uint8_t *in96, g2j *out_kilic, uint64_t n, uint32_t *bad_flag);
void launch_g2_prepare(hipStream_t s, const g2j *in_kilic, uint64_t n, g2_prepared *out);
void launch_pairs_g1_from_kilic(hipStream_t s, const g1j *a1, const g1j *b1, uint64_t n, g1j *p0, g1j *p1);
void launch_kzg_check_inputs(hipStream_t s, const g1j *c, const g1j *pi, const fr *ys, const g1j *es, const fr *bs, uint64_t n, g1j *p0, g1j *p1);
void launch_fr_rows_scale_by_inv_powers(hipStream_t s, fr *c, uint64_t np, const fr *xs, uint64_t count, fr *xpow_n);
void launch_eth_check_inputs(hipStream_t s, const uint8_t *c48, const uint8_t *zs, const uint8_t *ys, const uint8_t *pi48, uint64_t n, g1j *p0, g1j *p1, uint8_t *status);
void launch_pairing_check(hipStream_t s, bool shared_lines, const g2_prepared *q0, const g2_prepared *q1, const g1j *p0, const g1j *p1, uint64_t n, uint8_t *ok);
void launch_pairing_value(hipStream_t s, const g1j *g1_kilic, const g2_prepared *q, uint64_t n, fp *out);
bool pairing_route_is_wave(uint64_t n);

constexpr uint64_t PAIRING_WAVE_BELOW = 16385;
void launch_pairing_check_wave(hipStream_t s, bool shared_lines, const g2_prepared *q0, const g2_prepared *q1, const g1j *p0, const g1j *p1, uint64_t n, uint8_t *ok);
void launch_pairing_value_wave(hipStream_t s, const g1j *g1_kilic, const g2_prepared *q, uint64_t n, fp *out);
void launch_wave_fp12_op(hipStream_t s, int op, const fp *a, const fp *b, uint64_t n, fp *out);

struct g2a;
void launch_g2_fixed_base_table(hipStream_t s, g2a *table);
void launch_g2_fixed_base(hipStream_t s, const fr *scalars, uint64_t n, const g2a *table, g2j *out);
void launch_g2_normalize(hipStream_t s, const g2j *in, uint64_t n, g2j *out_kilic);
void launch_g2_compress(hipStream_t s, const g2j *in_kilic, uint64_t n, uint8_t *out96);

void launch_eth_transcripts(hipStream_t s, const uint8_t *blobs, const uint8_t *comms, const uint64_t *off, uint64_t n, uint64_t sidecars, fr *r_out, fr *z_out);
void launch_eth_transcript_blobs(hipStream_t s, const uint8_t *blobs, const uint64_t *off, uint64_t n, uint64_t sidecars, uint32_t *st);
void launch_eth_transcript_finish(hipStream_t s, const uint8_t *blobs, const uint8_t *comms, const uint64_t *off, uint64_t n, uint64_t sidecars, const uint32_t *st,
                                  fr *r_out, fr *z_out);
void launch_eth_prove_finish(hipStream_t s, const uint8_t *agg_status, const uint32_t *z_in_domain, const uint64_t *off, uint64_t sidecars, uint8_t code_blob,
                             uint8_t code_z, uint8_t *proofs48, uint8_t *comms48, uint8_t *status);
void launch_eth_agg_poly(hipStream_t s, const uint8_t *blobs, const uint64_t *off, const fr *r, uint64_t n, uint64_t sidecars, fr *agg, uint8_t *status);
void launch_eth_powers(hipStream_t s, const fr *r, const uint64_t *off, uint64_t sidecars, fr *pow);
void launch_g1_decompress_rows(hipStream_t s, const uint8_t *in48, g1j *out, uint64_t n, uint8_t *bad, bool to_kilic);
void launch_g1_segment_sum(hipStream_t s, const g1j *pts, const uint8_t *pt_bad, const uint64_t *off, uint64_t sidecars, g1j *out, g1j *out_kilic, uint8_t *status);
void launch_eth_agg_finish(hipStream_t s, const uint32_t *z_in_domain, const uint8_t *proof_bad, uint64_t sidecars, fr *y, uint8_t *status);
void launch_test_sha256_lanes(hipStream_t s, const uint8_t *data, const uint64_t *offsets, const uint64_t *lens, uint64_t rows, uint32_t *out);
void launch_test_hash_to_bls_field_lanes(hipStream_t s, const uint8_t *digests, uint64_t rows, fr *out);

void launch_eth_versioned_hashes(hipStream_t s, const uint8_t *c48, uint64_t n, uint8_t *out32);
void launch_eth_precompile_inputs(hipStream_t s, const uint8_t *in192, uint64_t n, g1j *p0, g1j *p1, uint8_t *status);
void launch_eth_merge_status(hipStream_t s, const uint8_t *status, const uint8_t *ok, uint64_t n, uint8_t *result);
void launch_eth_tx_hashes_check(hipStream_t s, const uint8_t *c48, const uint8_t *want32, const uint64_t *off, uint64_t total, uint64_t blocks, uint8_t *match,
                                uint8_t *result);

struct combine_seed;
void launch_combine_scalars(hipStream_t s, const combine_seed &seed, const fr *xs, const fr *ys, const uint8_t *status, uint64_t row0, uint64_t count, uint64_t R, fr *sc);
void launch_combine_points(hipStream_t s, const g1j *c, const g1j *pi, uint64_t count, uint64_t R, bool kilic, g1j *out);
void launch_combine_negate(hipStream_t s, const g1j *a, uint64_t n, g1j *out);
void launch_eth_combine_fields(hipStream_t s, const uint8_t *zs, const uint8_t *ys, const uint8_t *c_bad, const uint8_t *pi_bad, uint64_t n, fr *z_out, fr *y_out,
                               uint8_t *status);

void prof_begin(hipStream_t s, const char *name);
void prof_end(hipStream_t s, const char *name);

}
```

### go-kzg_amd/csrc/k_g1.hip

```cpp
#define KZG_MULQ_NOINLINE 1
#include "internal.hpp"
#include "coop_inv.hpp"

namespace kzg {

#ifndef G1_BLOCK
#define G1_BLOCK 256
#endif

__device__ __forceinline__ uint32_t bitrev32g(uint32_t v, uint32_t bits) { return bits ? (__brev(v) >> (32 - bits)) : 0; }

__device__ __forceinline__ g1j g1_mul_fr(const g1j &p, const fr &k_mont) {
    if (is_inf(p)) return g1_inf();
    g1aq tbl[8]; fq dz[7]; g1jq q; g1j packed;
    const int st = g1_mul_glv_regular_aq<false>(g1jq_unpack(p), glv_split_signed(from_mont<FrP>(k_mont)), tbl, dz, q, packed);
    return st == 1 ? g1jq_pack(q) : st == 2 ? packed : g1_inf();
}

__global__ __launch_bounds__(G1_BLOCK, 2) void k_g1_mul_vec(const g1j *pts, uint64_t pts_mod, const fr *scalars, uint64_t s_stride, uint64_t n,
                                                         g1j *out) {
    uint64_t t = blockIdx.x * (uint64_t)blockDim.x + threadIdx.x;
    if (t >= n) return;
    g1j p = pts[t % pts_mod];
    fr k = scalars[t * s_stride];
    out[t] = g1_mul_fr(p, k);
}
void launch_g1_mul_vec(hipStream_t s, const g1j *pts, uint64_t pts_mod, const fr *scalars, uint64_t s_stride, uint64_t n, g1j *out) {
    if (!n) return;
    prof_begin(s, "g1_mul_vec");
    hipLaunchKernelGGL(k_g1_mul_vec, dim3((uint32_t)((n + G1_BLOCK - 1) / G1_BLOCK)), dim3(G1_BLOCK), 0, s, pts, pts_mod, scalars, s_stride, n, out);
    prof_end(s, "g1_mul_vec");
}

__global__ __launch_bounds__(G1_BLOCK, 2) void k_g1_file_mul(const g1j *files, const fr *scalars, uint64_t nfiles, uint64_t k2, uint64_t j0, uint64_t cnt,
                                                          uint64_t total, g1j *tmp) {
    uint64_t t = blockIdx.x * (uint64_t)blockDim.x + threadIdx.x;
    if (t >= total) return;
    uint64_t jj = t % cnt, f = (t / cnt) % nfiles, b = t / (cnt * nfiles);
    g1j p = files[f * k2 + j0 + jj];
    fr k = scalars[(b * nfiles + f) * k2 + j0 + jj];
    tmp[t] = g1_mul_fr(p, k);
}
__global__ __launch_bounds__(G1_BLOCK, 2) void k_g1_sum_files(const g1j *tmp, uint64_t nfiles, uint64_t cnt, uint64_t total, g1j *out) {
    uint64_t t = blockIdx.x * (uint64_t)blockDim.x + threadIdx.x;
    if (t >= total) return;
    uint64_t jj = t % cnt, b = t / cnt;
    g1j acc = g1_inf();
    for (uint64_t f = 0; f < nfiles; f++) acc = g1_add(acc, tmp[(b * nfiles + f) * cnt + jj]);
    out[t] = acc;
}
void launch_g1_sum_files(hipStream_t s, const g1j *tmp, uint64_t nfiles, uint64_t cnt, uint64_t batch, g1j *out) {
    uint64_t outs = batch * cnt;
    if (!outs) return;
    hipLaunchKernelGGL(k_g1_sum_files, dim3((uint32_t)((outs + G1_BLOCK - 1) / G1_BLOCK)), dim3(G1_BLOCK), 0, s, tmp, nfiles, cnt, outs, out);
}
hipError_t launch_g1_file_msm(hipStream_t s, const g1j *files, const fr *scalars, uint64_t nfiles, uint64_t k2, uint64_t j0, uint64_t cnt, uint64_t batch,
                              g1j *out) {
    uint64_t total = batch * nfiles * cnt;
    if (!total) return hipSuccess;
    g1j *tmp = nullptr;
    hipError_t e = hipMallocAsync((void **)&tmp, total * sizeof(g1j), s);
    if (e != hipSuccess) return e;
    prof_begin(s, "g1_mul_vec");
    hipLaunchKernelGGL(k_g1_file_mul, dim3((uint32_t)((total + G1_BLOCK - 1) / G1_BLOCK)), dim3(G1_BLOCK), 0, s, files, scalars, nfiles, k2, j0, cnt, total, tmp);
    prof_end(s, "g1_mul_vec");
    uint64_t outs = batch * cnt;
    hipLaunchKernelGGL(k_g1_sum_files, dim3((uint32_t)((outs + G1_BLOCK - 1) / G1_BLOCK)), dim3(G1_BLOCK), 0, s, tmp, nfiles, cnt, outs, out);
    hipFreeAsync(tmp, s);
    return hipGetLastError();
}

__global__ void k_g1_bitrev_copy(const g1j *in, uint64_t in_stride, uint64_t n_valid, g1j *out, uint32_t logn, uint64_t total) {
    uint64_t t = blockIdx.x * (uint64_t)blockDim.x + threadIdx.x;
    if (t >= total) return;
    uint64_t n = 1ull << logn, b = t >> logn, i = t & (n - 1);
    g1j p = (i < n_valid) ? in[b * in_stride + i] : g1_inf();
    out[b * n + bitrev32g((uint32_t)i, logn)] = p;
}
void launch_g1_bitrev_copy(hipStream_t s, const g1j *in, uint64_t in_stride, uint64_t n_valid, g1j *out, uint64_t n, uint64_t batch) {
    uint64_t total = n * batch;
    if (!total) return;
    hipLaunchKernelGGL(k_g1_bitrev_copy, dim3((uint32_t)((total + 255) / 256)), dim3(256), 0, s, in, in_stride, n_valid, out, ilog2(n), total);
}

template <int MODE, bool PRE = false> __global__ __launch_bounds__(G1_BLOCK, 2) void k_g1_fft_stage(g1j *data, uint32_t logn, uint64_t m, const fr *roots, const int8_t *wnaf, uint64_t W, uint64_t total, uint64_t batch) {
    uint64_t t = blockIdx.x * (uint64_t)blockDim.x + threadIdx.x;
    if (t >= total) return;
    const uint64_t half = 1ull << (logn - 1), groups = half / m;
    const uint64_t j = t / (groups * batch), rem = t % (groups * batch), b = rem / groups, g = rem % groups;
    g1j *row = data + (b << logn);
    uint64_t i0 = g * 2 * m + j, i1 = i0 + m;
    g1j y = row[i1];
    g1j x = row[i0];
    if (MODE == 4) {
        g1jq yq; int st = is_inf(y) ? 0 : 1;
        if (st == 1) {
            if (j) {
                g1aq tbl[8]; fq dz[7]; g1j packed;
                const uint64_t ti = j * (W / (2 * m));
                if (PRE) st = g1_mul_glv_wnaf_aq_pre_q<true, true>(g1jq_unpack(y), roots[ti], tbl, dz, wnaf + ti * KZG_WNAF_ROW, yq, packed);
                else { int8_t dg1[132], dg2[132]; st = g1_mul_glv_wnaf_aq<true, true>(y, roots[ti], tbl, dz, dg1, dg2, 1, yq, packed); }
                if (st == 2) y = packed; else if (st == 0) y = g1_inf();
            } else yq = g1jq_unpack(y);
        }
        if (st == 1 && !is_inf(x)) {
            g1jq sum, dif;
            if (KZG_LIKELY(g1jq_addsub(g1jq_unpack(x), yq, sum, dif))) {
                fp z3 = packq(sum.z);
                g1j o0, o1;
                o0.x = packq(sum.x); o0.y = packq(sum.y); o0.z = z3;
                o1.x = packq(dif.x); o1.y = packq(dif.y); o1.z = z3;
                row[i0] = o0; row[i1] = o1;
                return;
            }
        }
        if (st == 1) y = g1jq_pack(yq);
    } else {
        if (j && !is_inf(y)) {
            const fr kk = roots[j * (W / (2 * m))];
            glv_halves h;
#pragma unroll
            for (int i = 0; i < 4; i++) { h.k1[i] = kk.l[i]; h.k2[i] = kk.l[4 + i]; }
            h.neg1 = h.neg2 = 0;
            g1aq tbl[8]; fq dz[7]; g1jq q; g1j packed;
            const int st = g1_mul_glv_regular_aq<true>(g1jq_unpack(y), h, tbl, dz, q, packed);
            y = st == 1 ? g1jq_pack(q) : st == 2 ? packed : g1_inf();
        }
    }
    row[i0] = g1_add(x, y);
    row[i1] = g1_add(x, g1_neg(y));
}
bool g1_quad_enabled() { return knobs::g1_quad() != 0; }
#ifndef KZG_WNAF_ROWS_MIN
#define KZG_WNAF_ROWS_MIN 512
#endif
g1_stage_plan g1_fft_stage_plan(uint64_t n, uint64_t batch, uint64_t m, bool dif, int quad, knobs::g1_mul_mode mul) {
    const uint64_t butterflies = n / 2 * batch, per_twiddle = (n / 2 / m) * batch, one_round = device_simd_lanes();
    g1_stage_plan p;
    p.lanes = quad >= 0 ? (quad == 0 ? 1 : quad == 2 ? 2 : 4) : butterflies * 4 <= one_round ? 4 : butterflies * 2 <= one_round ? 2 : 1;
    if (p.lanes > 1) {
        p.wnaf = mul != knobs::g1_mul_mode::regular && (per_twiddle * (uint64_t)p.lanes) % 64 == 0;
        p.rows = p.wnaf;
        return p;
    }
    p.wnaf = dif || (mul == knobs::g1_mul_mode::regular ? false : mul == knobs::g1_mul_mode::wnaf ? true : (per_twiddle % 64 == 0 || per_twiddle >= 256));
    p.rows = p.wnaf && per_twiddle >= (uint64_t)KZG_WNAF_ROWS_MIN;
    return p;
}
g1_stage_plan g1_fft_stage_plan(uint64_t n, uint64_t batch, uint64_t m, bool dif) { return g1_fft_stage_plan(n, batch, m, dif, knobs::g1_quad(), knobs::g1_mul()); }
template <bool PRE> __global__ __launch_bounds__(G1_BLOCK, 2) void k_g1_fft_stage_dif(g1j *data, uint32_t logn, uint64_t m, const fr *roots, const int8_t *wnaf, uint64_t W, uint64_t total, uint64_t batch) {
    uint64_t t = blockIdx.x * (uint64_t)blockDim.x + threadIdx.x;
    if (t >= total) return;
    const uint64_t half = 1ull << (logn - 1), groups = half / m;
    const uint64_t j = t / (groups * batch), rem = t % (groups * batch), b = rem / groups, g = rem % groups;
    g1j *row = data + (b << logn);
    uint64_t i0 = g * 2 * m + j, i1 = i0 + m;
    g1j y = row[i1];
    g1j x = row[i0];
    if (!is_inf(x) && !is_inf(y)) {
        g1jq sum, dif;
        if (KZG_LIKELY(g1jq_addsub(g1jq_unpack(x), g1jq_unpack(y), sum, dif))) {
            g1j o0; o0.x = packq(sum.x); o0.y = packq(sum.y); o0.z = packq(sum.z);
            row[i0] = o0;
            if (j) {
                g1aq tbl[8]; fq dz[7]; g1j packed; g1jq dq;
                const uint64_t ti = j * (W / (2 * m));
                int st;
                if (PRE) st = g1_mul_glv_wnaf_aq_pre_q<true, true>(dif, roots[ti], tbl, dz, wnaf + ti * KZG_WNAF_ROW, dq, packed);
                else { int8_t dg1[132], dg2[132]; st = g1_mul_glv_wnaf_aq_q<true, true>(dif, roots[ti], tbl, dz, dg1, dg2, 1, dq, packed); }
                row[i1] = st == 1 ? g1jq_pack(dq) : st == 2 ? packed : g1_inf();
            } else { g1j o1; o1.x = packq(dif.x); o1.y = packq(dif.y); o1.z = o0.z; row[i1] = o1; }
            return;
        }
    }
    g1j s_ = g1_add(x, y), d_ = g1_add(x, g1_neg(y));
    if (j && !is_inf(d_)) {
        g1aq tbl[8]; fq dz[7]; g1j packed; g1jq dq;
        const uint64_t ti = j * (W / (2 * m));
        int8_t dg1[132], dg2[132];
        int st = g1_mul_glv_wnaf_aq<true, true>(d_, roots[ti], tbl, dz, dg1, dg2, 1, dq, packed);
        d_ = st == 1 ? g1jq_pack(dq) : st == 2 ? packed : g1_inf();
    }
    row[i0] = s_; row[i1] = d_;
}
void launch_g1_fft_stage_dif(hipStream_t s, g1j *data, uint64_t n, uint64_t batch, uint64_t m, const fr *roots, const int8_t *wnaf, uint64_t W) {
    launch_g1_fft_stage_planned(s, g1_fft_stage_plan(n, batch, m, true), true, data, n, batch, m, roots, wnaf, W);
}
__global__ void k_g1_clear_odd(g1j *data, uint64_t total_pairs) {
    uint64_t t = blockIdx.x * (uint64_t)blockDim.x + threadIdx.x;
    if (t < total_pairs) data[2 * t + 1] = g1_inf();
}
void launch_g1_clear_odd(hipStream_t s, g1j *data, uint64_t n_total) {
    if (n_total < 2) return;
    hipLaunchKernelGGL(k_g1_clear_odd, dim3((uint32_t)((n_total / 2 + 255) / 256)), dim3(256), 0, s, data, n_total / 2);
}
__global__ void k_g1_take_even(const g1j *in, g1j *out, uint64_t total) {
    uint64_t t = blockIdx.x * (uint64_t)blockDim.x + threadIdx.x;
    if (t < total) out[t] = in[2 * t];
}
void launch_g1_take_even(hipStream_t s, const g1j *in, g1j *out, uint64_t total) {
    if (!total) return;
    hipLaunchKernelGGL(k_g1_take_even, dim3((uint32_t)((total + 255) / 256)), dim3(256), 0, s, in, out, total);
}
void launch_g1_fft_stage(hipStream_t s, g1j *data, uint64_t n, uint64_t batch, uint64_t m, const fr *roots, const int8_t *wnaf, uint64_t W) {
    launch_g1_fft_stage_planned(s, g1_fft_stage_plan(n, batch, m, false), false, data, n, batch, m, roots, wnaf, W);
}
void launch_g1_fft_stage_planned(hipStream_t s, const g1_stage_plan &plan, bool dif, g1j *data, uint64_t n, uint64_t batch, uint64_t m, const fr *roots, const int8_t *wnaf, uint64_t W) {
    uint64_t total = n / 2 * batch;
    if (!total) return;
    prof_begin(s, "g1_fft_stage");
    if (plan.lanes > 1) {
        if (dif) launch_g1_stage_coop_dif(s, plan.lanes, plan.wnaf, data, n, batch, m, roots, wnaf, W, total);
        else launch_g1_stage_coop_dit(s, plan.lanes, plan.wnaf, data, n, batch, m, roots, wnaf, W, total);
        prof_end(s, "g1_fft_stage");
        return;
    }
    const dim3 grid((uint32_t)((total + G1_BLOCK - 1) / G1_BLOCK)), block(G1_BLOCK);
    const uint32_t logn = ilog2(n);
    if (dif) {
        if (plan.rows) hipLaunchKernelGGL(k_g1_fft_stage_dif<true>, grid, block, 0, s, data, logn, m, roots, wnaf, W, total, batch);
        else hipLaunchKernelGGL(k_g1_fft_stage_dif<false>, grid, block, 0, s, data, logn, m, roots, wnaf, W, total, batch);
    } else if (plan.wnaf) {
        if (plan.rows) hipLaunchKernelGGL((k_g1_fft_stage<4, true>), grid, block, 0, s, data, logn, m, roots, wnaf, W, total, batch);
        else hipLaunchKernelGGL((k_g1_fft_stage<4, false>), grid, block, 0, s, data, logn, m, roots, wnaf, W, total, batch);
    } else hipLaunchKernelGGL(k_g1_fft_stage<0>, grid, block, 0, s, data, logn, m, roots, wnaf, W, total, batch);
    prof_end(s, "g1_fft_stage");
}

struct g1jq_slot { uint32_t w[39]; uint32_t inf; uint32_t pad; };
#define G1_DIRECT_BLOCK 64
__global__ __launch_bounds__(G1_DIRECT_BLOCK, 2) void k_g1_fft_direct(const g1j *in, uint64_t in_stride, uint64_t n_valid, g1j *out, uint32_t logn, uint32_t logR,
                                                            uint64_t Ns, const fr *roots, uint64_t W, const fr *scale, uint64_t total, uint32_t logT, uint32_t logU) {
    __shared__ g1jq_slot buf[G1_DIRECT_BLOCK];
    const uint32_t tid = threadIdx.x;
    const uint64_t t = blockIdx.x * (uint64_t)blockDim.x + tid;
    const uint64_t n = 1ull << logn, R = 1ull << logR, cols = n >> logR, T = 1ull << logT;
    const uint32_t tt = (uint32_t)(t & (T - 1));
    const uint64_t u = (t >> logT) & ((1ull << logU) - 1), jb = t >> (logT + logU), j = jb % cols, b = jb / cols;
    const bool live = t < total;
    g1jq_acc acc; acc.inf = true;
    uint64_t oidx = 0;
    if (live) {
        const uint64_t k = j & (Ns - 1), idx = j + (uint64_t)tt * cols;
        oidx = b * n + (j - k) * R + k + u * Ns;
        g1j x = idx < n_valid ? in[b * in_stride + idx] : g1_inf();
        if (!is_inf(x)) {
            const uint64_t e = ((uint64_t)tt * (cols / Ns) * (Ns * u + k)) & (n - 1);
            if (e == 0 && !scale) { acc.v = g1jq_unpack(x); acc.inf = false; }
            else {
                fr sc = roots[e * (W >> logn)];
                if (scale) sc = mul(sc, *scale);
                g1aq tbl[8]; fq dz[7]; g1j packed;
                const int st = g1_mul_glv_regular_aq<true>(g1jq_unpack(x), glv_split_signed(from_mont<FrP>(sc)), tbl, dz, acc.v, packed);
                if (st == 2) { acc.inf = is_inf(packed); if (!acc.inf) acc.v = g1jq_unpack(packed); } else acc.inf = st == 0;
            }
        }
    }
    auto store = [&](uint32_t i) {
#pragma unroll
        for (int q = 0; q < 13; q++) { buf[i].w[q] = acc.v.x.l[q]; buf[i].w[13 + q] = acc.v.y.l[q]; buf[i].w[26 + q] = acc.v.z.l[q]; }
        buf[i].inf = acc.inf ? 1u : 0u;
    };
    store(tid);
    __syncthreads();
#pragma nounroll
    for (uint32_t off = (uint32_t)T / 2; off >= 1; off >>= 1) {
        if (tt < off && !buf[tid + off].inf) {
            g1jq q;
#pragma unroll
            for (int i = 0; i < 13; i++) { q.x.l[i] = buf[tid + off].w[i]; q.y.l[i] = buf[tid + off].w[13 + i]; q.z.l[i] = buf[tid + off].w[26 + i]; }
            acc.add(q);
            store(tid);
        }
        __syncthreads();
    }
    if (live && tt == 0) out[oidx] = acc.inf ? g1_inf() : g1jq_pack(acc.v);
}
void launch_g1_fft_direct(hipStream_t s, const g1j *in, uint64_t in_stride, uint64_t n_valid, g1j *data, g1j *tmp, uint64_t n, uint64_t batch, const fr *roots,
                          uint64_t W, const fr *scale, uint32_t max_logr, int lanes, uint32_t bits_done, uint64_t n_out, bool lanes_fixed) {
    const uint32_t logn = ilog2(n);
    if (max_logr < 1 || max_logr > 4) max_logr = 4;
    uint32_t bits_left = logn - bits_done;
    uint32_t npass = (bits_left + max_logr - 1) / max_logr;
    if (!npass) { launch_g1_bitrev_copy(s, in, in_stride, n_valid, data, n, batch); return; }
    const g1j *src = in; uint64_t src_stride = in_stride, src_valid = n_valid, Ns = 1ull << bits_done;
    prof_begin(s, "g1_fft_direct");
    for (uint32_t p = 0; p < npass; p++) {
        const uint32_t logR = bits_left >= max_logr ? max_logr : bits_left;
        g1j *dst = ((npass - 1 - p) & 1u) ? tmp : data;
        uint32_t logT = logR, logU = logR;
        const uint64_t cols = n >> logR;
        while (logT > 0 && (cols << (logT - 1)) >= src_valid) logT--;
        if (p + 1 == npass && n_out && n_out < n) while (logU > 0 && (Ns << (logU - 1)) >= n_out) logU--;
        const uint64_t total = (batch * cols) << (logT + logU);
        int L = lanes;
        if (!lanes_fixed && g1_quad_enabled() && knobs::g1_direct_coop() && (logT < logR || logU < logR)) L = total * 4 <= device_simd_lanes() ? 4 : total * 2 <= device_simd_lanes() ? 2 : lanes;
        const uint64_t wgs = (total * L + G1_DIRECT_BLOCK - 1) / G1_DIRECT_BLOCK;
        const size_t pad_lds = wgs <= device_simds() ? 24 * 1024 : 0;
        const fr *sc = (p + 1 == npass) ? scale : nullptr;
        if (L > 1) launch_g1_direct_coop(s, L, (uint32_t)wgs, pad_lds, src, src_stride, src_valid, dst, logn, logR, Ns, roots, W, sc, total, logT, logU);
        else hipLaunchKernelGGL(k_g1_fft_direct, dim3((uint32_t)wgs), dim3(G1_DIRECT_BLOCK), pad_lds, s, src, src_stride, src_valid, dst, logn, logR, Ns, roots, W, sc, total, logT, logU);
        src = dst; src_stride = n; src_valid = (p + 1 == npass && n_out && n_out < n) ? n_out : n; Ns <<= logR; bits_left -= logR;
    }
    prof_end(s, "g1_fft_direct");
}

__global__ __launch_bounds__(G1_BLOCK, 2) void k_g1_normalize(const g1j *in, g1j *out, uint64_t n, int to_kilic) {
    uint64_t t = blockIdx.x * (uint64_t)blockDim.x + threadIdx.x;
    if (t >= n) return;
    g1j p = g1_normalize(in[t]);
    out[t] = to_kilic ? g1_to_kilic(p) : p;
}
__global__ __launch_bounds__(64) void k_g1_normalize_wave(const g1j *in, g1j *out, uint64_t n, int to_kilic) {
    const uint64_t t = blockIdx.x;
    const g1j p = in[t];
    g1j o;
    if (is_inf(p)) o = g1_inf();
    else {
        const fp zi = wave_inv_fp(p.z, 0), zi2 = sqr(zi);
        o.x = mul(p.x, zi2); o.y = mul(p.y, mul(zi2, zi)); o.z = one<FpP>();
    }
    if (threadIdx.x == 0) out[t] = to_kilic ? g1_to_kilic(o) : o;
}
__global__ __launch_bounds__(64) void k_fp_inv_both(const fp *in, fp *out_coop, fp *out_lane, int mode) {
    const fp x = in[blockIdx.x];
    if (mode & 1) { const fp y = wave_inv_fp(x, 0); if (threadIdx.x == 0) out_coop[blockIdx.x] = y; }
    if ((mode & 2) && threadIdx.x == 0) out_lane[blockIdx.x] = inv<FpP>(x);
}
void launch_fp_inv_both(hipStream_t s, const fp *in, fp *out_coop, fp *out_lane, uint64_t n, int mode) {
    if (n) hipLaunchKernelGGL(k_fp_inv_both, dim3((uint32_t)n), dim3(64), 0, s, in, out_coop, out_lane, mode);
}
#define NORM_NB 8
__global__ __launch_bounds__(G1_BLOCK, 2) void k_g1_normalize_batched(const g1j *in, g1j *out, uint64_t n, uint64_t lanes, int to_kilic) {
    uint64_t t = blockIdx.x * (uint64_t)blockDim.x + threadIdx.x;
    if (t >= lanes) return;
    fp pref[NORM_NB];
    fp acc = one<FpP>();
#pragma unroll
    for (int k = 0; k < NORM_NB; k++) {
        uint64_t i = t + (uint64_t)k * lanes;
        pref[k] = acc;
        if (i < n) { fp z = in[i].z; if (!is_zero<FpP>(z)) acc = mul(acc, z); }
    }
    fp inv_all = inv<FpP>(acc);
#pragma unroll
    for (int k = NORM_NB - 1; k >= 0; k--) {
        uint64_t i = t + (uint64_t)k * lanes;
        if (i >= n) continue;
        g1j p = in[i];
        g1j o;
        if (is_inf(p)) o = g1_inf();
        else {
            fp zi = mul(inv_all, pref[k]);
            inv_all = mul(inv_all, p.z);
            fp zi2 = sqr(zi);
            o.x = mul(p.x, zi2); o.y = mul(p.y, mul(zi2, zi)); o.z = one<FpP>();
        }
        out[i] = to_kilic ? g1_to_kilic(o) : o;
    }
}
void launch_g1_normalize(hipStream_t s, const g1j *in, g1j *out, uint64_t n, bool to_kilic) {
    if (!n) return;
    if (n < 1024 && knobs::coop_inv()) {
        hipLaunchKernelGGL(k_g1_normalize_wave, dim3((uint32_t)n), dim3(64), 0, s, in, out, n, to_kilic ? 1 : 0);
        return;
    }
    if (n < 1024 || in == out) {
        hipLaunchKernelGGL(k_g1_normalize, dim3((uint32_t)((n + G1_BLOCK - 1) / G1_BLOCK)), dim3(G1_BLOCK), 0, s, in, out, n, to_kilic ? 1 : 0);
        return;
    }
    uint64_t lanes = (n + NORM_NB - 1) / NORM_NB;
    hipLaunchKernelGGL(k_g1_normalize_batched, dim3((uint32_t)((lanes + G1_BLOCK - 1) / G1_BLOCK)), dim3(G1_BLOCK), 0, s, in, out, n, lanes, to_kilic ? 1 : 0);
}
__global__ __launch_bounds__(G1_BLOCK, 2) void k_g1_from_kilic(g1j *data, uint64_t n) {
    uint64_t t = blockIdx.x * (uint64_t)blockDim.x + threadIdx.x;
    if (t >= n) return;
    data[t] = g1_from_kilic(data[t]);
}
// ... 84 lines not shown
```

### go-kzg_amd/csrc/k_g1_coop_dif.hip

```cpp
#define KZG_MULQ_NOINLINE 1
#include "g1_coop_kernels.hpp"
namespace kzg {
void launch_g1_stage_coop_dif(hipStream_t s, int lanes, bool wnaf_rows, g1j *data, uint64_t n, uint64_t batch, uint64_t m, const fr *roots, const int8_t *wnaf, uint64_t W, uint64_t total) {
    launch_stage_coop<true>(s, lanes, wnaf_rows, data, n, batch, m, roots, wnaf, W, total);
}
}
```

### go-kzg_amd/csrc/k_g1_coop_dit.hip

```cpp
#define KZG_MULQ_NOINLINE 1
#include "g1_coop_kernels.hpp"
namespace kzg {
void launch_g1_stage_coop_dit(hipStream_t s, int lanes, bool wnaf_rows, g1j *data, uint64_t n, uint64_t batch, uint64_t m, const fr *roots, const int8_t *wnaf, uint64_t W, uint64_t total) {
    launch_stage_coop<false>(s, lanes, wnaf_rows, data, n, batch, m, roots, wnaf, W, total);
}
}
```

### go-kzg_amd/csrc/k_msm.hip

```cpp
#include "internal.hpp"
#include "g1_quad.hpp"
#include "coop_inv.hpp"
#include <atomic>
#include <cstring>

namespace kzg {

#define MSM_SORT_T 1024
#define MSM_ACC_BLOCK 128
#define MSM_NB 128

struct fb_partial { uint32_t w[52]; uint32_t inf; };
__device__ __forceinline__ void fb_partial_store(fb_partial &o, const g1x_acc &a) {
#pragma unroll
    for (int i = 0; i < 13; i++) { o.w[i] = a.v.x.l[i]; o.w[13 + i] = a.v.y.l[i]; o.w[26 + i] = a.v.zz.l[i]; o.w[39 + i] = a.v.zzz.l[i]; }
    o.inf = a.inf ? 1u : 0u;
}
__device__ __forceinline__ void fb_partial_load(const fb_partial &p, g1xq &v) {
#pragma unroll
    for (int i = 0; i < 13; i++) { v.x.l[i] = p.w[i]; v.y.l[i] = p.w[13 + i]; v.zz.l[i] = p.w[26 + i]; v.zzz.l[i] = p.w[39 + i]; }
}

template <uint32_t DELTA> __device__ __forceinline__ uint32_t lane_down(uint32_t v) {
    if constexpr (DELTA < 16) return (uint32_t)__builtin_amdgcn_update_dpp((int)v, (int)v, 0x100 + DELTA, 0xf, 0xf, false);
// ... 608 lines not shown
        }
        quad_tree_add(acc, w, winf, role);
    }
    quad_tree_reduce(acc, buf, tid, blocks_per_blob < 64 ? blocks_per_blob : 64);
    const bool first_wave = tid < 64;
    if (first_wave) {
        const bool own = col == 0;
        const g1x px = g1xq_pack(acc.v);
        const bool need = own && !acc.inf && !(to_kilic & 2);
        const fp i = wave_inv_any(mul(px.zz, px.zzz), need);
        const uint32_t aff = __builtin_amdgcn_readfirstlane((uint32_t)(!acc.inf && !(to_kilic & 2)));
        if (aff) {
            fp i1;
#pragma unroll
            for (int k = 0; k < 12; k++) i1.l[k] = (uint32_t)__builtin_amdgcn_readlane((int)i.l[k], 0);
            if (tid < 2) {
                fp c = mul(tid ? px.y : px.x, mul(i1, tid ? px.zz : px.zzz));
                if (to_kilic & 1) c = fp_to_kilic(c);
                fp *dst = tid ? &out[b].y : &out[b].x;
                *dst = c;
                if (tid == 0) out[b].z = (to_kilic & 1) ? fp_kilic_one() : one<FpP>();
            }
        } else if (own) {
            g1j r;
            if (acc.inf) r = g1_inf(); else r = g1x_to_jac(px);
            out[b] = (to_kilic & 1) ? g1_to_kilic(r) : r;
        }
    }
}

__global__ __launch_bounds__(64) void k_fb_finish_lanes(const fb_partial *partials, uint32_t blocks_per_blob, uint64_t batch, g1j *out, int to_kilic) {
    const uint64_t b = blockIdx.x * (uint64_t)blockDim.x + threadIdx.x;
    if (b >= batch) return;
    g1x_acc acc; acc.init();
#pragma nounroll
    for (uint32_t j = 0; j < blocks_per_blob; j++) {
        const fb_partial &pj = partials[b * blocks_per_blob + j];
        g1xq w; fb_partial_load(pj, w);
        g1x_acc_merge(acc, w, pj.inf != 0);
    }
    g1j r;
    if (acc.inf) r = g1_inf();
    else if (to_kilic & 2) r = g1x_to_jac(g1xq_pack(acc.v));
    else {
        g1x px = g1xq_pack(acc.v);
        fp i = inv<FpP>(mul(px.zz, px.zzz));
        r.x = mul(px.x, mul(i, px.zzz)); r.y = mul(px.y, mul(i, px.zz)); r.z = one<FpP>();
    }
    out[b] = (to_kilic & 1) ? g1_to_kilic(r) : r;
}

template <bool GLV> __device__ __forceinline__ void fb_walk_term(g1x_acc &acc, const g1a *table, uint64_t table_n, uint32_t c, uint32_t nwin, uint32_t D, uint64_t i,
                                                                const fr &k, uint32_t sg, bool phi) {
    uint32_t m[8];
    uint32_t sgn = sg;
    if (GLV) {
        const glv_halves h = glv_split_signed(k);
#pragma unroll
        for (int j = 0; j < 4; j++) { m[j] = phi ? h.k2[j] : h.k1[j]; m[4 + j] = 0; }
        sgn ^= phi ? h.neg2 : h.neg1;
    } else {
#pragma unroll
        for (int j = 0; j < 8; j++) m[j] = k.l[j];
    }
    auto bits = [&](uint32_t off) -> uint32_t {
        const uint32_t idx = off >> 5, sh = off & 31;
        if (idx >= (GLV ? 4u : 8u)) return 0u;
        uint64_t v = m[idx];
        if (idx + 1 < (GLV ? 4u : 8u)) v |= (uint64_t)m[idx + 1] << 32;
        return (uint32_t)(v >> sh) & ((1u << c) - 1u);
    };
    uint32_t raw = bits(0), carry, mag, ng;
    if (raw > D) { carry = 1; mag = (1u << c) - raw; ng = 1; } else { carry = 0; mag = raw; ng = 0; }
    g1a qn = table[((uint64_t)0 * table_n + i) * D + (mag ? mag - 1 : 0)];
#pragma nounroll
    for (uint32_t w = 0; w < nwin; w++) {
        g1a q = qn;
        const uint32_t cmag = mag, cng = ng ^ sgn;
        if (w + 1 < nwin) {
            raw = bits((w + 1) * c) + carry;
            if (raw > D) { carry = 1; mag = (1u << c) - raw; ng = 1; } else { carry = 0; mag = raw; ng = 0; }
            qn = table[((uint64_t)(w + 1) * table_n + i) * D + (mag ? mag - 1 : 0)];
        }
        if (cmag) {
            if (cng) q.y = neg<FpP>(q.y);
            acc.add(q);
        }
    }
}
template <bool GLV> __global__ __launch_bounds__(FB_BLOCK, 2) void k_fb_mul_vec(const g1a *table, uint64_t table_n, uint32_t c, uint32_t nwin, uint32_t D, const fr *scalars,
                                                         uint64_t i0, uint64_t cnt, uint64_t row, uint64_t total, g1j *out) {
    uint64_t t = blockIdx.x * (uint64_t)blockDim.x + threadIdx.x;
    if (t >= total) return;
    uint64_t jj = t % cnt, f = (t / cnt) % (table_n / row), b = t / (cnt * (table_n / row));
    uint64_t i = f * row + i0 + jj;
    const fr k = from_mont<FrP>(scalars[b * table_n + i]);
    g1x_acc acc; acc.init();
    if (GLV) { fb_walk_term<true>(acc, table, table_n, c, nwin, D, i, k, 0u, true); acc_apply_phi(acc); }
    fb_walk_term<GLV>(acc, table, table_n, c, nwin, D, i, k, 0u, false);
    out[t] = acc.to_jac();
}
struct fbp_slot { uint32_t w[39]; uint32_t inf; uint32_t pad; };
template <bool GLV> __global__ __launch_bounds__(64, 2) void k_fb_direct_pass1(const g1a *table, uint64_t table_n, uint32_t c, uint32_t nwin, uint32_t D, const fr *scalars, const fr *roots,
                                                           uint64_t W, uint32_t logn, uint32_t logR, uint64_t total, g1j *out) {
    __shared__ fbp_slot buf[64];
    const uint32_t tid = threadIdx.x;
    const uint64_t t = blockIdx.x * (uint64_t)blockDim.x + tid;
    const uint64_t n = 1ull << logn, R = 1ull << logR, cols = n >> logR;
    const uint32_t tt = (uint32_t)(t & (R - 1));
    const uint64_t u = (t >> logR) & (R - 1), jb = t >> (2 * logR), j = jb % cols, b = jb / cols;
    const bool live = t < total;
    g1jq_acc acc; acc.inf = true;
    if (live) {
        const uint64_t i = j + (uint64_t)tt * cols, e = ((uint64_t)tt * cols * u) & (n - 1);
        fr kmont = scalars[b * n + i];
        if (e) kmont = mul(kmont, roots[e * (W >> logn)]);
        const fr k = from_mont<FrP>(kmont);
        g1x_acc xa; xa.init();
        if (GLV) { fb_walk_term<true>(xa, table, table_n, c, nwin, D, i, k, 0u, true); acc_apply_phi(xa); }
        fb_walk_term<GLV>(xa, table, table_n, c, nwin, D, i, k, 0u, false);
        if (!xa.inf) { acc.v = g1jq_unpack(xa.to_jac()); acc.inf = false; }
    }
#define FBP_STORE(i_) do { _Pragma("unroll") for (int q_ = 0; q_ < 13; q_++) { buf[i_].w[q_] = acc.v.x.l[q_]; buf[i_].w[13 + q_] = acc.v.y.l[q_]; buf[i_].w[26 + q_] = acc.v.z.l[q_]; } \
                           buf[i_].inf = acc.inf ? 1u : 0u; } while (0)
    FBP_STORE(tid);
    __syncthreads();
#pragma nounroll
    for (uint32_t off = (uint32_t)R / 2; off >= 1; off >>= 1) {
        if (tt < off && !buf[tid + off].inf) {
            g1jq q;
#pragma unroll
            for (int i = 0; i < 13; i++) { q.x.l[i] = buf[tid + off].w[i]; q.y.l[i] = buf[tid + off].w[13 + i]; q.z.l[i] = buf[tid + off].w[26 + i]; }
            acc.add(q);
            FBP_STORE(tid);
        }
        __syncthreads();
    }
#undef FBP_STORE
    if (live && tt == 0) out[b * n + j * R + u] = acc.inf ? g1_inf() : g1jq_pack(acc.v);
}
void launch_fb_direct_pass1(hipStream_t s, const g1a *table, uint64_t table_n, uint32_t c, uint32_t nwin, const fr *scalars, const fr *roots, uint64_t W, uint64_t batch,
                            uint32_t logR, g1j *out, bool glv) {
    uint32_t logn = 0;
    while ((1ull << logn) < table_n) logn++;
    const uint64_t total = (batch * table_n) << logR, wgs = (total + 63) / 64;
    prof_begin(s, "fb_mul_vec");
    if (glv) hipLaunchKernelGGL(k_fb_direct_pass1<true>, dim3((uint32_t)wgs), dim3(64), wgs <= device_simds() ? 24 * 1024 : 0, s, table, table_n, c, nwin, 1u << (c - 1), scalars, roots, W, logn, logR,
                                total, out);
    else hipLaunchKernelGGL(k_fb_direct_pass1<false>, dim3((uint32_t)wgs), dim3(64), wgs <= device_simds() ? 24 * 1024 : 0, s, table, table_n, c, nwin, 1u << (c - 1), scalars, roots, W, logn, logR,
                            total, out);
    prof_end(s, "fb_mul_vec");
}

template <bool GLV> __global__ __launch_bounds__(FB_BLOCK, 2) void k_fb_mul_vec_dif2(const g1a *table, uint64_t table_n, uint32_t c, uint32_t nwin, uint32_t D, const fr *scalars,
                                                              const fr *roots, uint64_t W, uint64_t total, g1j *out) {
    uint64_t t = blockIdx.x * (uint64_t)blockDim.x + threadIdx.x;
    if (t >= total) return;
    const uint64_t N = table_n, q = N >> 2;
    const uint64_t i = t % q, o = (t / q) & 3u, b = t / N;
    const uint64_t rs = W / N;
    g1x_acc acc; acc.init();
#pragma nounroll
    for (uint32_t pass = GLV ? 0u : 1u; pass < 2; pass++) {
#pragma nounroll
        for (uint32_t term = 0; term < 4; term++) {
            const uint64_t pi = i + term * q;
            uint64_t e; uint32_t sg;
            if (o == 0) { e = 0; sg = 0; }
            else if (o == 1) { e = 2 * i; sg = term & 1u; }
            else if (o == 2) { e = i + ((term & 1u) ? q : 0); sg = term >> 1; }
            else { e = 3 * i + ((term & 1u) ? q : 0); sg = (term == 1 || term == 2) ? 1u : 0u; }
            fr kmont = scalars[b * N + pi];
            if (e) kmont = mul(kmont, roots[(e & (N - 1)) * rs]);
            const fr k = from_mont<FrP>(kmont);
            fb_walk_term<GLV>(acc, table, table_n, c, nwin, D, pi, k, sg, pass == 0);
        }
        if (GLV && pass == 0) acc_apply_phi(acc);
    }
    out[b * N + o * q + i] = acc.to_jac();
}
void launch_fb_mul_vec_dif2(hipStream_t s, const g1a *table, uint64_t table_n, uint32_t c, uint32_t nwin, const fr *scalars, const fr *roots, uint64_t W,
                            uint64_t batch, g1j *out, bool glv) {
    uint64_t total = batch * table_n;
    if (!total) return;
    prof_begin(s, "fb_mul_vec");
    if (glv) hipLaunchKernelGGL(k_fb_mul_vec_dif2<true>, dim3((uint32_t)((total + FB_BLOCK - 1) / FB_BLOCK)), dim3(FB_BLOCK), 0, s, table, table_n, c, nwin, 1u << (c - 1), scalars,
                                roots, W, total, out);
    else hipLaunchKernelGGL(k_fb_mul_vec_dif2<false>, dim3((uint32_t)((total + FB_BLOCK - 1) / FB_BLOCK)), dim3(FB_BLOCK), 0, s, table, table_n, c, nwin, 1u << (c - 1), scalars,
                            roots, W, total, out);
    prof_end(s, "fb_mul_vec");
}
template <bool GLV> __global__ __launch_bounds__(FB_BLOCK, 2) void k_fb_mul_vec_files(const g1a *table, uint64_t table_n, uint32_t c, uint32_t nwin, uint32_t D, const fr *scalars,
                                                               uint64_t i0, uint64_t cnt, uint64_t row, uint64_t total, g1j *out) {
    uint64_t t = blockIdx.x * (uint64_t)blockDim.x + threadIdx.x;
    if (t >= total) return;
    const uint64_t jj = t % cnt, b = t / cnt, nfiles = table_n / row;
    g1x_acc acc; acc.init();
#pragma nounroll
    for (uint32_t pass = GLV ? 0u : 1u; pass < 2; pass++) {
#pragma nounroll
        for (uint64_t f = 0; f < nfiles; f++) {
            const uint64_t i = f * row + i0 + jj;
            const fr k = from_mont<FrP>(scalars[b * table_n + i]);
            fb_walk_term<GLV>(acc, table, table_n, c, nwin, D, i, k, 0u, pass == 0);
        }
        if (GLV && pass == 0) acc_apply_phi(acc);
    }
    out[t] = acc.to_jac();
}
void launch_fb_mul_vec_files(hipStream_t s, const g1a *table, uint64_t table_n, uint32_t c, uint32_t nwin, const fr *scalars, uint64_t row, uint64_t j0,
                             uint64_t cnt, uint64_t batch, g1j *out, bool glv) {
    uint64_t total = batch * cnt;
    if (!total) return;
    prof_begin(s, "fb_mul_vec");
    if (glv) hipLaunchKernelGGL(k_fb_mul_vec_files<true>, dim3((uint32_t)((total + FB_BLOCK - 1) / FB_BLOCK)), dim3(FB_BLOCK), 0, s, table, table_n, c, nwin, 1u << (c - 1), scalars,
                                j0, cnt, row, total, out);
    else hipLaunchKernelGGL(k_fb_mul_vec_files<false>, dim3((uint32_t)((total + FB_BLOCK - 1) / FB_BLOCK)), dim3(FB_BLOCK), 0, s, table, table_n, c, nwin, 1u << (c - 1), scalars,
                            j0, cnt, row, total, out);
    prof_end(s, "fb_mul_vec");
}
void launch_fb_mul_vec(hipStream_t s, const g1a *table, uint64_t table_n, uint32_t c, uint32_t nwin, const fr *scalars, uint64_t row, uint64_t j0,
                       uint64_t cnt, uint64_t batch, g1j *out, bool glv) {
    uint64_t total = batch * (table_n / row) * cnt;
    if (!total) return;
    prof_begin(s, "fb_mul_vec");
    if (glv) hipLaunchKernelGGL(k_fb_mul_vec<true>, dim3((uint32_t)((total + FB_BLOCK - 1) / FB_BLOCK)), dim3(FB_BLOCK), 0, s, table, table_n, c, nwin, 1u << (c - 1), scalars,
                                j0, cnt, row, total, out);
    else hipLaunchKernelGGL(k_fb_mul_vec<false>, dim3((uint32_t)((total + FB_BLOCK - 1) / FB_BLOCK)), dim3(FB_BLOCK), 0, s, table, table_n, c, nwin, 1u << (c - 1), scalars,
                            j0, cnt, row, total, out);
    prof_end(s, "fb_mul_vec");
}

uint64_t device_simd_lanes() {
    static std::atomic<uint64_t> lanes_of_device[64];
    int dev = 0;
    (void)hipGetDevice(&dev);
    std::atomic<uint64_t> &slot = lanes_of_device[dev >= 0 && dev < 64 ? dev : 0];
    uint64_t lanes = slot.load(std::memory_order_relaxed);
    if (!lanes) {
        int cus = 256;
        if (hipDeviceGetAttribute(&cus, hipDeviceAttributeMultiprocessorCount, dev) != hipSuccess) { (void)hipGetLastError(); cus = 256; }
        lanes = (uint64_t)(cus > 0 ? cus : 256) * 4 * 64;
        slot.store(lanes, std::memory_order_relaxed);
    }
    return lanes;
}
static uint32_t fb_blocks_per_blob(uint64_t n, uint64_t batch, uint32_t *wsplit = nullptr) {
    uint64_t lanes = knobs::fb_lanes() ? knobs::fb_lanes() : 2 * device_simd_lanes();
    if (lanes < FB_ACC_BLOCK) lanes = FB_ACC_BLOCK;
    uint64_t target = lanes / FB_ACC_BLOCK;
    uint64_t bpb = target / (batch ? batch : 1);
    uint32_t split = 1;
    while (split < 8 && (batch ? batch : 1) * n * split * 2 <= lanes) split *= 2;
    if (wsplit) *wsplit = split;
    uint64_t maxb = (n * split + FB_ACC_BLOCK - 1) / FB_ACC_BLOCK;
    if (bpb > maxb) bpb = maxb;
    if (bpb < 1) bpb = 1;
    return (uint32_t)bpb;
}
size_t fb_partials_bytes(uint64_t n, uint64_t batch) { return (((size_t)std::max(fb_blocks_per_blob(n, batch), fb_blocks_per_blob(2 * n, batch)) * batch * sizeof(fb_partial)) + 15) / 16 * 16; }

void launch_fb_msm(hipStream_t s, const g1a *table, uint64_t table_n, uint32_t c, uint32_t nwin, const fr *scalars, uint64_t sc_stride, uint64_t n,
                   uint64_t batch, void *partials, g1j *out, bool to_kilic, bool glv, bool projective) {
    if (!batch) return;
    const int fin = (to_kilic ? 1 : 0) | (projective ? 2 : 0);
    uint32_t split = 1;
    uint32_t bpb = fb_blocks_per_blob(glv ? 2 * n : n, batch, &split);
    if (split > nwin) split = nwin;
    prof_begin(s, "fb_accumulate");
    if (glv) {
        if (split > 1) hipLaunchKernelGGL(k_fb_accumulate_glv<true>, dim3((uint32_t)(batch * bpb)), dim3(FB_ACC_BLOCK), 0, s, table, table_n, c, nwin, 1u << (c - 1), scalars, sc_stride, n,
                                          bpb, split, (fb_partial *)partials);
        else hipLaunchKernelGGL(k_fb_accumulate_glv<false>, dim3((uint32_t)(batch * bpb)), dim3(FB_ACC_BLOCK), 0, s, table, table_n, c, nwin, 1u << (c - 1), scalars, sc_stride, n, bpb,
                                1u, (fb_partial *)partials);
    } else if (split > 1) hipLaunchKernelGGL(k_fb_accumulate<true>, dim3((uint32_t)(batch * bpb)), dim3(FB_ACC_BLOCK), 0, s, table, table_n, c, nwin, 1u << (c - 1), scalars, sc_stride, n,
                                      bpb, split, (fb_partial *)partials);
    else hipLaunchKernelGGL(k_fb_accumulate<false>, dim3((uint32_t)(batch * bpb)), dim3(FB_ACC_BLOCK), 0, s, table, table_n, c, nwin, 1u << (c - 1), scalars, sc_stride, n, bpb,
                            1u, (fb_partial *)partials);
    prof_end(s, "fb_accumulate");
    if (bpb <= FB_FINISH_LANES_MAX) hipLaunchKernelGGL(k_fb_finish_lanes, dim3((uint32_t)((batch + 63) / 64)), dim3(64), 0, s, (const fb_partial *)partials, bpb, batch, out, fin);
    else hipLaunchKernelGGL(k_fb_finish, dim3((uint32_t)batch), dim3(256), 0, s, (const fb_partial *)partials, bpb, batch, out, fin);
}
hipError_t launch_fb_build(hipStream_t s, const g1a *pts, uint64_t n, uint32_t c, uint32_t nwin, g1a *table) {
    uint32_t D = 1u << (c - 1);
    g1j *rows_j = nullptr; g1a *rows = nullptr; fp *ztmp = nullptr, *ptmp = nullptr;
    uint64_t lanes_all = (uint64_t)nwin * n;
    hipError_t e;
    if ((e = hipMallocAsync((void **)&rows_j, lanes_all * sizeof(g1j), s)) != hipSuccess) return e;
    if ((e = hipMallocAsync((void **)&rows, lanes_all * sizeof(g1a), s)) != hipSuccess) { hipFreeAsync(rows_j, s); return e; }
    launch_msm_window_table(s, pts, n, c, nwin, rows_j, rows);
    uint64_t per_win = n * D * sizeof(fp);
    uint32_t slab = (uint32_t)((1ull << 30) / (per_win ? per_win : 1));
    if (slab < 1) slab = 1;
    if (slab > nwin) slab = nwin;
    if ((e = hipMallocAsync((void **)&ztmp, (uint64_t)slab * per_win, s)) != hipSuccess) { hipFreeAsync(rows_j, s); hipFreeAsync(rows, s); return e; }
    if ((e = hipMallocAsync((void **)&ptmp, (uint64_t)slab * per_win, s)) != hipSuccess) { hipFreeAsync(rows_j, s); hipFreeAsync(rows, s); hipFreeAsync(ztmp, s); return e; }
    for (uint32_t w0 = 0; w0 < nwin; w0 += slab) {
        uint32_t ws = (w0 + slab <= nwin) ? slab : nwin - w0;
        uint64_t lanes = (uint64_t)ws * n;
        uint32_t S = D;
        while (S > 64 && lanes * (D / S) < (1ull << 20)) S >>= 1;
        dim3 g((uint32_t)((lanes * (D / S) + FB_BLOCK - 1) / FB_BLOCK)), b(FB_BLOCK);
        hipLaunchKernelGGL(k_fb_build_pass1, g, b, 0, s, rows + (uint64_t)w0 * n, lanes, D, S, table + (uint64_t)w0 * n * D, ztmp);
        hipLaunchKernelGGL(k_fb_build_pass2, g, b, 0, s, lanes, D, S, table + (uint64_t)w0 * n * D, ztmp, ptmp);
    }
    hipFreeAsync(rows_j, s); hipFreeAsync(rows, s); hipFreeAsync(ztmp, s); hipFreeAsync(ptmp, s);
    return hipGetLastError();
}

__global__ __launch_bounds__(MSM_ACC_BLOCK, 2) void k_msm_window_rows(const g1a *pts, uint64_t n, uint32_t c, uint32_t nwin, g1j *tmp) {
    uint64_t i = blockIdx.x * (uint64_t)blockDim.x + threadIdx.x;
    if (i >= n) return;
    g1j q = to_jac(pts[i]);
#pragma nounroll
    for (uint32_t w = 0; w < nwin; w++) {
        tmp[(uint64_t)w * n + i] = q;
#pragma nounroll
        for (uint32_t j = 0; j < c; j++) q = g1_dbl(q);
    }
}
void launch_msm_window_table(hipStream_t s, const g1a *pts, uint64_t n, uint32_t c, uint32_t nwin, g1j *tmp, g1a *out) {
    if (!n) return;
    hipLaunchKernelGGL(k_msm_window_rows, dim3((uint32_t)((n + MSM_ACC_BLOCK - 1) / MSM_ACC_BLOCK)), dim3(MSM_ACC_BLOCK), 0, s, pts, n, c, nwin, tmp);
    launch_g1_to_affine(s, tmp, out, n * nwin);
}

}
```

### go-kzg_amd/csrc/knobs.hpp

```cpp
#pragma once
#include <limits.h>
#include <stdint.h>
#include <stdlib.h>
#include <string.h>

namespace kzg {

enum { FAULT_RCCL = 1, FAULT_RCCL_CORRUPT = 2, FAULT_PEER = 4, FAULT_PEER_CORRUPT = 8, FAULT_RCCL_HANG = 16, FAULT_PEER_HANG = 32, FAULT_PEER_STUCK = 64, FAULT_RCCL_BLOCK = 128, FAULT_RCCL_INIT_BLOCK = 256 };

namespace knobs {

enum class g1_fft_mode { by_size, direct, radix2 };
enum class g1_mul_mode { by_shape, regular, wnaf };
enum class fr_fft_mode { by_size, radix2, shared };
enum class zero_poly_mode { by_size, direct, tree };
enum class msm_reduce_mode { by_batch, scan, chunks };
enum class transcript_mode { by_count, host, device };
enum class pairing_mode { by_count, lane, wave };
enum class combine_mode { by_count, never, always };
enum class transport_mode { by_devices, rccl, host, peer };
struct opt_gb { bool set; double gb; };

inline bool is(const char *e, const char *word) { return e && !strcmp(e, word); }
inline bool starts(const char *e, char c) { return e && e[0] == c; }
inline bool list_has(const char *e, const char *word) {
    const size_t n = strlen(word);
    for (const char *at = e; e && (at = strstr(at, word)); at += n)
        if ((at == e || at[-1] == ',') && (at[n] == 0 || at[n] == ',')) return true;
    return false;
}
inline zero_poly_mode zero_poly_of(const char *e) { return is(e, "direct") ? zero_poly_mode::direct : is(e, "tree") ? zero_poly_mode::tree : zero_poly_mode::by_size; }
inline double positive_or(const char *e, double dflt) { const double v = e ? atof(e) : 0.0; return v > 0.0 ? v : dflt; }
inline unsigned multi_fault_of(const char *e) {
    if (!e) return 0;
    return (list_has(e, "rccl") ? FAULT_RCCL : 0) | (list_has(e, "rccl-corrupt") ? FAULT_RCCL_CORRUPT : 0) | (list_has(e, "peer") ? FAULT_PEER : 0) |
           (list_has(e, "peer-corrupt") ? FAULT_PEER_CORRUPT : 0) | (list_has(e, "rccl-hang") ? FAULT_RCCL_HANG : 0) |
           (list_has(e, "rccl-block") ? FAULT_RCCL_BLOCK : 0) |
           (list_has(e, "rccl-init-block") ? FAULT_RCCL_INIT_BLOCK : 0) |
           (list_has(e, "peer-hang") ? FAULT_PEER_HANG : 0) |
           (list_has(e, "peer-stuck") ? FAULT_PEER_HANG | FAULT_PEER_STUCK : 0);
}

#define KZG_KNOB_ONCE(type, fn, name, expr)                   \
    inline type parse_##fn(const char *e) { return expr; }    \
    inline type fn() { static type const v = parse_##fn(getenv(name)); return v; }
#define KZG_KNOB_PER_CALL(type, fn, name, expr)               \
    inline type parse_##fn(const char *e) { return expr; }    \
    inline type fn() { return parse_##fn(getenv(name)); }
#define KZG_KNOB_PER_HANDLE KZG_KNOB_PER_CALL

KZG_KNOB_ONCE(bool, fb_glv, "KZG_HIP_FB_GLV", !is(e, "0"))
KZG_KNOB_ONCE(bool, coalesce, "KZG_HIP_COALESCE", !starts(e, '0'))
KZG_KNOB_ONCE(bool, upload_ramp, "KZG_HIP_UPLOAD_RAMP", !starts(e, '0'))
KZG_KNOB_ONCE(bool, lincomb_promote, "KZG_HIP_LINCOMB_PROMOTE", !starts(e, '0'))
KZG_KNOB_ONCE(bool, stream_cache, "KZG_HIP_STREAM_CACHE", !starts(e, '0'))
KZG_KNOB_ONCE(bool, g1_direct_coop, "KZG_HIP_G1_DIRECT_COOP", !starts(e, '0'))
KZG_KNOB_ONCE(bool, coop_inv, "KZG_HIP_COOP_INV", !starts(e, '0'))
KZG_KNOB_ONCE(bool, fk20_pass1, "KZG_HIP_FK20_PASS1", !starts(e, '0'))
KZG_KNOB_ONCE(bool, fk20_fuse, "KZG_HIP_FK20_FUSE", !starts(e, '0'))
KZG_KNOB_ONCE(bool, fk20_pad, "KZG_HIP_FK20_PAD", !starts(e, '0'))
KZG_KNOB_PER_CALL(bool, eth_prove_overlap, "KZG_HIP_ETH_PROVE_OVERLAP", !starts(e, '0'))
KZG_KNOB_ONCE(bool, coalesce_trace, "KZG_HIP_COALESCE_TRACE", e != nullptr)
KZG_KNOB_PER_CALL(bool, coalesce_stats, "KZG_HIP_COALESCE_STATS", e != nullptr)
KZG_KNOB_ONCE(bool, eth_quotient_one, "KZG_HIP_ETH_QUOTIENT", is(e, "one"))
KZG_KNOB_ONCE(bool, sha256_portable, "KZG_HIP_SHA256", is(e, "portable"))

KZG_KNOB_ONCE(g1_fft_mode, g1_fft, "KZG_HIP_G1_FFT", !e ? g1_fft_mode::by_size : e[0] == 'd' ? g1_fft_mode::direct : g1_fft_mode::radix2)
KZG_KNOB_ONCE(int, g1_quad, "KZG_HIP_G1_QUAD", !e ? -1 : e[0] == '0' ? 0 : e[0] == '2' ? 2 : 1)
KZG_KNOB_ONCE(g1_mul_mode, g1_mul, "KZG_HIP_G1_MUL", starts(e, 'r') ? g1_mul_mode::regular : starts(e, 'w') ? g1_mul_mode::wnaf : g1_mul_mode::by_shape)
KZG_KNOB_ONCE(fr_fft_mode, fr_fft, "KZG_HIP_FR_FFT", is(e, "radix2") ? fr_fft_mode::radix2 : is(e, "shared") ? fr_fft_mode::shared : fr_fft_mode::by_size)
KZG_KNOB_ONCE(zero_poly_mode, zero_poly_once, "KZG_HIP_ZERO_POLY", zero_poly_of(e))
KZG_KNOB_PER_CALL(zero_poly_mode, zero_poly_per_call, "KZG_HIP_ZERO_POLY", zero_poly_of(e))
KZG_KNOB_ONCE(msm_reduce_mode, msm_reduce, "KZG_HIP_MSM_REDUCE", is(e, "chunks") ? msm_reduce_mode::chunks : is(e, "scan") ? msm_reduce_mode::scan : msm_reduce_mode::by_batch)
KZG_KNOB_ONCE(int, msm_seg, "KZG_HIP_MSM_SEG", e ? atoi(e) : -1)
KZG_KNOB_PER_CALL(transcript_mode, eth_transcript, "KZG_HIP_ETH_TRANSCRIPT", is(e, "host") ? transcript_mode::host : is(e, "device") ? transcript_mode::device : transcript_mode::by_count)
KZG_KNOB_PER_CALL(pairing_mode, pairing, "KZG_HIP_PAIRING", is(e, "lane") ? pairing_mode::lane : is(e, "wave") ? pairing_mode::wave : pairing_mode::by_count)
KZG_KNOB_PER_CALL(combine_mode, verify_combine, "KZG_HIP_VERIFY_COMBINE", is(e, "never") ? combine_mode::never : is(e, "always") ? combine_mode::always : combine_mode::by_count)
KZG_KNOB_PER_CALL(int, multi_fft, "KZG_HIP_MULTI_FFT", !e ? -1 : is(e, "sharded") ? 1 : 0)
KZG_KNOB_PER_HANDLE(transport_mode, multi_transport, "KZG_HIP_MULTI_TRANSPORT", !e ? transport_mode::by_devices : is(e, "rccl") ? transport_mode::rccl : is(e, "host") ? transport_mode::host : transport_mode::peer)
KZG_KNOB_PER_HANDLE(unsigned, multi_fault, "KZG_HIP_MULTI_FAULT", multi_fault_of(e))
KZG_KNOB_ONCE(const char *, rccl_lib, "KZG_HIP_RCCL_LIB", e)

KZG_KNOB_ONCE(uint32_t, lincomb_promote_after, "KZG_HIP_LINCOMB_PROMOTE_AFTER", (uint32_t)(!e ? 2 : atol(e) < 1 ? 1 : atol(e) > 1000 ? 1000 : atol(e)))
KZG_KNOB_ONCE(uint64_t, fb_lanes, "KZG_HIP_FB_LANES", e ? strtoull(e, nullptr, 10) : 0ull)
KZG_KNOB_ONCE(uint64_t, eth_stage_rows, "KZG_HIP_ETH_STAGE_ROWS", e ? (uint64_t)atol(e) : 0ull)
KZG_KNOB_PER_CALL(uint64_t, verify_combine_rows, "KZG_HIP_VERIFY_COMBINE_ROWS", e && strtoull(e, nullptr, 10) >= 1 ? strtoull(e, nullptr, 10) : 0ull)
KZG_KNOB_PER_CALL(double, eth_verify_chunk_mb, "KZG_HIP_ETH_VERIFY_CHUNK_MB", positive_or(e, 4096.0))
KZG_KNOB_PER_CALL(double, eth_prove_chunk_mb, "KZG_HIP_ETH_PROVE_CHUNK_MB", positive_or(e, 4096.0))
KZG_KNOB_PER_CALL(double, recover_chunk_mb, "KZG_HIP_RECOVER_CHUNK_MB", positive_or(e, 2048.0))
KZG_KNOB_PER_CALL(opt_gb, fb_budget_gb, "KZG_HIP_FB_BUDGET_GB", (opt_gb{e != nullptr, e ? atof(e) : 0.0}))
KZG_KNOB_PER_CALL(opt_gb, points_fb_budget_gb, "KZG_HIP_POINTS_FB_BUDGET_GB", (opt_gb{e != nullptr, e ? atof(e) : 0.0}))
KZG_KNOB_PER_CALL(opt_gb, fk20_fb_budget_gb, "KZG_HIP_FK20_FB_BUDGET_GB", (opt_gb{e != nullptr, e ? atof(e) : 0.0}))
KZG_KNOB_PER_HANDLE(long, multi_probe_timeout_ms, "KZG_HIP_MULTI_PROBE_TIMEOUT_MS", e && atol(e) >= 10 && atol(e) <= 600000 ? atol(e) : 10000)
KZG_KNOB_PER_HANDLE(long, coalesce_us, "KZG_HIP_COALESCE_US", e ? atol(e) : 150)
KZG_KNOB_PER_HANDLE(long, coalesce_spin_us, "KZG_HIP_COALESCE_SPIN_US", e ? atol(e) : 40)
KZG_KNOB_PER_CALL(int, coalesce_sim_max_bufs, "KZG_COALESCE_SIM_MAX_BUFS", e ? atoi(e) : INT_MAX)

#undef KZG_KNOB_ONCE
#undef KZG_KNOB_PER_CALL
#undef KZG_KNOB_PER_HANDLE

inline int parse_coalesce_exec(const char *e, int dflt, int max) { return !e ? dflt : atoi(e) < 1 ? 1 : atoi(e) > max ? max : atoi(e); }
inline int coalesce_exec(int dflt, int max) { return parse_coalesce_exec(getenv("KZG_HIP_COALESCE_EXEC"), dflt, max); }
inline int parse_coalesce_per_batch(const char *e, int dflt) { return !e ? dflt : atoi(e) < 1 ? 1 : atoi(e); }
inline int coalesce_per_batch(int dflt) { return parse_coalesce_per_batch(getenv("KZG_HIP_COALESCE_PER_BATCH"), dflt); }

}
}
```

### go-kzg_amd/csrc/kzg_hip_internal.h

```cpp
#ifndef KZG_HIP_INTERNAL_H
#define KZG_HIP_INTERNAL_H
#include "../../include/kzg_hip.h"
#ifdef __cplusplus
extern "C" {
#endif
#pragma GCC visibility push(default)

void kzg_hip_prof_reset(kzg_hip_fft *fs, int enable);
int kzg_hip_prof_read(kzg_hip_fft *fs, const char *kernel, double *total_ms, uint64_t *launches);
int kzg_hip_calibrate(kzg_hip_fft *fs, double *mad_per_s, double *add_per_s, double *fp_mul_per_s);
int kzg_hip_bench_drop_in(kzg_hip_kzg *ks, int op, const void *blobs_fr, uint64_t n, uint64_t nblobs, unsigned threads, unsigned calls, void *out_g1,
                          double *seconds);
int kzg_hip_bench_drop_in_eth_proof(kzg_hip_eth *eth, const void *polys_fr, uint64_t n, uint64_t npolys, unsigned threads, unsigned calls, void *out48,
                                    double *seconds);
int kzg_hip_bench_threads_fft_fr(kzg_hip_fft *fs, const void *vals_fr, uint64_t n, uint64_t nrows, unsigned threads, unsigned calls, void *out_fr, double *seconds);
int kzg_hip_bench_poly_lincomb_dev(kzg_hip_fft *fs, const void *d_vectors_fr, uint64_t stride, const void *d_scalars_fr, uint64_t count, uint64_t n, void *d_out_fr,
                                   void *stream);
int kzg_hip_coalesce_stats(kzg_hip_kzg *ks, int op, uint64_t out[8]);
int kzg_hip_test_fp_inv(kzg_hip_fft *fs, const void *in_fp, uint64_t n, void *out_coop, void *out_lane, double *ms_coop, double *ms_lane);
int kzg_hip_lincomb_promotions(kzg_hip_fft *fs, uint64_t *promoted, uint64_t *served);
int kzg_hip_test_fr_inv(kzg_hip_fft *fs, const void *in_fr, uint64_t n, void *out_coop, void *out_lane, void *out_block);
void kzg_hip_test_sha256(const void *data, uint64_t len, void *out32);
int kzg_hip_test_sha256_lanes(kzg_hip_fft *fs, const void *data, const uint64_t *offsets, const uint64_t *lens, uint64_t rows, void *out32);
int kzg_hip_test_hash_to_bls_field_lanes(kzg_hip_fft *fs, const void *digests32, uint64_t rows, void *out_fr);
uint64_t kzg_hip_test_eth_prove_chunks(void);

int kzg_hip_pairing_test(kzg_hip_fft *fs, const void *g1, const void *g2, uint64_t n, void *out_fp12);
int kzg_hip_pairing_test_wave(kzg_hip_fft *fs, const void *g1, const void *g2, uint64_t n, void *out_fp12);
int kzg_hip_test_wave_fp12_op(kzg_hip_fft *fs, int op, const void *a, const void *b, uint64_t n, void *out);
int kzg_hip_test_pairing_route(uint64_t n, uint64_t out[2]);

int kzg_hip_test_combine_points(kzg_hip_kzg *ks, const void *commitments_g1, const void *proofs_g1, const void *xs_fr, const void *ys_fr, uint64_t count,
                                const uint8_t *seed32, void *out_a_g1, void *out_b_g1);
int kzg_hip_test_combine_stats(uint64_t out[6]);

int kzg_hip_test_g2_table_builds(kzg_hip_fft *fs, uint64_t *builds);

int kzg_hip_test_g1_fft_plan(kzg_hip_fft *fs, uint64_t n, uint64_t batch, uint64_t m, int dif, uint32_t out[5]);
int kzg_hip_test_g1_fft_stage(kzg_hip_fft *fs, const void *pts_g1, uint64_t n, uint64_t batch, uint64_t m, int inv, int dif, int lanes, int mul, void *out_g1,
                              uint32_t plan_out[3]);
int kzg_hip_test_g1_fft_direct(kzg_hip_fft *fs, const void *pts_g1, uint64_t n, uint64_t n_valid, uint64_t batch, int inv, uint32_t max_logr, int lanes, uint64_t n_out,
                               void *out_g1);

#pragma GCC visibility pop
#ifdef __cplusplus
}
#endif
#endif
```

Measured before the change: 102,000 commitments/s.

## Add half-size FK20 path splitting odd/even terms with twisted G1 FFT

Adds an FK20 path for the non-DA case that works on size-k instead of 2k G1 FFTs. It multiplies the odd-indexed circulant coefficients via the fixed-base table, runs a twisted DIF/DIT G1 FFT pair of length k with a twiddle offset (toff), and adds the even-indexed terms back in a separate fixed-base kernel. The goal is to halve the G1 FFT work and the scalar-multiplication volume. The cost is an extra fixed-base walk for the even terms and more code paths. The DIF/DIT kernels gain a twiddle-offset parameter.

Result: no change. 102,100 commitments/s (median of 2 runs) (+0.1%).

```diff
diff --git a/go-kzg_amd/__init__.py b/go-kzg_amd/__init__.py
--- a/go-kzg_amd/__init__.py
+++ b/go-kzg_amd/__init__.py
@@ -132,6 +132,7 @@
         "kzg_hip_test_fr_inv": (i32, [vp, vp, u64, vp, vp, vp]),
         "kzg_hip_test_g1_fft_plan": (i32, [vp, u64, u64, u64, i32, vp]),
         "kzg_hip_test_g1_fft_stage": (i32, [vp, vp, u64, u64, u64, i32, i32, i32, i32, vp, vp]),
+        "kzg_hip_test_g1_fft_stage_toff": (i32, [vp, vp, u64, u64, u64, u64, i32, i32, i32, i32, vp, vp]),
         "kzg_hip_test_g1_fft_direct": (i32, [vp, vp, u64, u64, u64, i32, u32, i32, u64, vp]),
         "kzg_hip_kzg_table_info": (i32, [vp, C.POINTER(C.c_uint32), C.POINTER(C.c_uint32), C.POINTER(u64)]), "kzg_hip_kzg_table_additions": (u32, [vp]), "kzg_hip_kzg_set_projective_outputs": (i32, [vp, i32]),
         "kzg_hip_da_using_fk20_multi_batch": (i32, [vp, vp, u64, u64, vp]),
diff --git a/go-kzg_amd/csrc/capi_core.hip b/go-kzg_amd/csrc/capi_core.hip
--- a/go-kzg_amd/csrc/capi_core.hip
+++ b/go-kzg_amd/csrc/capi_core.hip
@@ -383,7 +383,12 @@
     return KZG_HIP_OK;
 }
 int kzg_hip_test_g1_fft_stage(kzg_hip_fft *fs, const void *pts_g1, uint64_t n, uint64_t batch, uint64_t m, int inv, int dif, int lanes, int mul, void *out_g1, uint32_t plan_out[3]) {
+    return kzg_hip_test_g1_fft_stage_toff(fs, pts_g1, n, batch, m, 0, inv, dif, lanes, mul, out_g1, plan_out);
+}
+int kzg_hip_test_g1_fft_stage_toff(kzg_hip_fft *fs, const void *pts_g1, uint64_t n, uint64_t batch, uint64_t m, uint64_t toff, int inv, int dif, int lanes, int mul, void *out_g1,
+                                   uint32_t plan_out[3]) {
     if (!fs || !pts_g1 || !out_g1 || !g1_stage_shape_ok(fs, n, batch, m)) return KZG_HIP_ERR_BAD_ARG;
+    if (toff > fs->W - (m - 1) * (fs->W / (2 * m))) return KZG_HIP_ERR_BAD_ARG;
     if ((lanes != 0 && lanes != 1 && lanes != 2 && lanes != 4) || mul < 0 || mul > 2) return KZG_HIP_ERR_BAD_ARG;
     stream_lease lease(fs);
     hipStream_t s = lease.s;
@@ -394,7 +399,7 @@
     CHK(d_data.alloc(n * batch)); CHK(d_out.alloc(n * batch));
     HIPCHK(hipMemcpyAsync(d_data.p, pts_g1, n * batch * sizeof(g1j), hipMemcpyHostToDevice, s));
     launch_g1_from_kilic(s, d_data.p, n * batch);
-    launch_g1_fft_stage_planned(s, plan, dif != 0, d_data.p, n, batch, m, inv ? fs->d_glv_reversed : fs->d_glv_expanded, inv ? fs->d_wnaf_reversed : fs->d_wnaf_expanded, fs->W);
+    launch_g1_fft_stage_planned(s, plan, dif != 0, d_data.p, n, batch, m, inv ? fs->d_glv_reversed : fs->d_glv_expanded, inv ? fs->d_wnaf_reversed : fs->d_wnaf_expanded, fs->W, toff);
     launch_g1_normalize(s, d_data.p, d_out.p, n * batch, true);
     HIPCHK(hipGetLastError());
     HIPCHK(hipMemcpyAsync(out_g1, d_out.p, n * batch * sizeof(g1j), hipMemcpyDeviceToHost, s));
diff --git a/go-kzg_amd/csrc/capi_fk20.hip b/go-kzg_amd/csrc/capi_fk20.hip
--- a/go-kzg_amd/csrc/capi_fk20.hip
+++ b/go-kzg_amd/csrc/capi_fk20.hip
@@ -104,7 +104,25 @@
     const uint64_t k2 = 2 * c->k;
     return knobs::fk20_fuse() && c->l == 1 && c->d_files_fb && k2 >= 8 && !g1_fft_direct_mode(k2, batch) && (da || !g1_fft_direct_mode(c->k, batch));
 }
+static int fk20_run_half(fk20_core *c, hipStream_t s, const fr *d_poly, uint64_t poly_stride, uint64_t n, uint64_t batch, int bit_reverse, g1j *d_out) {
+    kzg_hip_fft *fs = c->ks->fs;
+    const uint64_t k = c->k, k2 = 2 * k, W = fs->W;
+    dtmp<fr> d_tc(s), d_cf(s); dtmp<g1j> d_a(s), d_b(s);
+    CHK(d_tc.alloc(batch * k2)); CHK(d_cf.alloc(batch * k2)); CHK(d_a.alloc(batch * k));
+    launch_toeplitz_coeffs(s, d_poly, poly_stride, n, 1, batch, d_tc.p, fs->d_inv_pow2 + ilog2(k2));
+    fr_fft_rows(fs, s, d_tc.p, k2, k2, d_cf.p, k2, batch, 0);
+    launch_fb_mul_vec_odd_dif2(s, c->d_files_fb, k2, c->fb_c, c->fb_nwin, d_cf.p, fs->d_reversed, W, batch, d_a.p, c->fb_glv);
+    for (uint64_t m = k / 8; m >= 1; m >>= 1) launch_g1_fft_stage_dif(s, d_a.p, k, batch, m, fs->d_glv_reversed, fs->d_wnaf_reversed, W, W / (4 * m));
+    for (uint64_t m = 1; m < k; m <<= 1) launch_g1_fft_stage(s, d_a.p, k, batch, m, fs->d_glv_expanded, fs->d_wnaf_expanded, W);
+    g1j *sum = d_a.p;
+    if (bit_reverse) { CHK(d_b.alloc(batch * k)); sum = d_b.p; }
+    launch_fb_add_even(s, c->d_files_fb, k2, c->fb_c, c->fb_nwin, d_cf.p, d_a.p, batch, bit_reverse, sum, c->fb_glv);
+    launch_g1_normalize(s, sum, d_out, batch * k, true);
+    HIPCHK(hipGetLastError());
+    return KZG_HIP_OK;
+}
 static int fk20_run_fused(fk20_core *c, hipStream_t s, const fr *d_poly, uint64_t poly_stride, uint64_t n, uint64_t batch, int da, int bit_reverse, g1j *d_out) {
+    if (!da && knobs::fk20_half()) return fk20_run_half(c, s, d_poly, poly_stride, n, batch, bit_reverse, d_out);
     kzg_hip_fft *fs = c->ks->fs;
     const uint64_t k2 = 2 * c->k;
     dtmp<fr> d_tc(s), d_cf(s); dtmp<g1j> d_a(s), d_b(s);
diff --git a/go-kzg_amd/csrc/g1_coop_kernels.hpp b/go-kzg_amd/csrc/g1_coop_kernels.hpp
--- a/go-kzg_amd/csrc/g1_coop_kernels.hpp
+++ b/go-kzg_amd/csrc/g1_coop_kernels.hpp
@@ -10,7 +10,7 @@
 struct g1jq_slot { uint32_t w[39]; uint32_t inf; uint32_t pad; };
 #define G1_DIRECT_BLOCK 64
 
-template <bool DIF, bool WNAF, int L> __global__ __launch_bounds__(G1_BLOCK, 2) void k_g1_fft_stage_quad(g1j *data, uint32_t logn, uint64_t m, const fr *roots, const int8_t *wnaf, uint64_t W, uint64_t total, uint64_t batch) {
+template <bool DIF, bool WNAF, int L> __global__ __launch_bounds__(G1_BLOCK, 2) void k_g1_fft_stage_quad(g1j *data, uint32_t logn, uint64_t m, const fr *roots, const int8_t *wnaf, uint64_t W, uint64_t total, uint64_t batch, uint64_t toff) {
     const uint64_t t4 = blockIdx.x * (uint64_t)blockDim.x + threadIdx.x;
     const uint32_t role = (uint32_t)(t4 & (uint64_t)(L - 1));
     const uint64_t t = t4 / L;
@@ -21,7 +21,7 @@
     const uint64_t i0 = g * 2 * m + j, i1 = i0 + m;
     g1j y = row[i1];
     g1j x = row[i0];
-    const uint64_t ti = j * (W / (2 * m));
+    const uint64_t ti = j * (W / (2 * m)) + toff;
     const fr kk = roots[ti];
     glv_halves h;
 #pragma unroll
@@ -32,7 +32,7 @@
     if (!DIF) {
         g1jq yq; int st = is_inf(y) ? 0 : 1;
         if (st == 1) {
-            if (j) {
+            if (ti) {
                 st = QMUL(g1jq_unpack(y), yq);
                 if (st == 2) y = packed; else if (st == 0) y = g1_inf();
             } else yq = g1jq_unpack(y);
@@ -58,7 +58,7 @@
             if (KZG_LIKELY(g1jq_addsub(g1jq_unpack(x), g1jq_unpack(y), sum, dif))) {
                 g1j o0; o0.x = packq(sum.x); o0.y = packq(sum.y); o0.z = packq(sum.z);
                 g1j o1;
-                if (j) {
+                if (ti) {
                     g1jq dq;
                     const int st = QMUL(dif, dq);
                     o1 = st == 1 ? g1jq_pack(dq) : st == 2 ? packed : g1_inf();
@@ -68,7 +68,7 @@
             }
         }
         g1j s_ = g1_add(x, y), d_ = g1_add(x, g1_neg(y));
-        if (j && !is_inf(d_)) {
+        if (ti && !is_inf(d_)) {
             g1jq dq;
             const int st = QMUL(g1jq_unpack(d_), dq);
             d_ = st == 1 ? g1jq_pack(dq) : st == 2 ? packed : g1_inf();
@@ -78,7 +78,7 @@
 }
 #undef QMUL
 template <bool DIF> static inline void launch_stage_coop(hipStream_t s, int lanes, bool wn, g1j *data, uint64_t n, uint64_t batch, uint64_t m, const fr *roots, const int8_t *wnaf, uint64_t W,
-                                                  uint64_t total) {
+                                                  uint64_t total, uint64_t toff) {
     static const bool once = [] {
         hipFuncSetAttribute(reinterpret_cast<const void *>(&k_g1_fft_stage_quad<DIF, true, 4>), hipFuncAttributeMaxDynamicSharedMemorySize, 96 * 1024);
         hipFuncSetAttribute(reinterpret_cast<const void *>(&k_g1_fft_stage_quad<DIF, false, 4>), hipFuncAttributeMaxDynamicSharedMemorySize, 96 * 1024);
@@ -90,11 +90,11 @@
     const dim3 qg((uint32_t)((lanes * total + G1_BLOCK - 1) / G1_BLOCK));
     const uint32_t logn = ilog2(n);
     if (lanes == 4) {
-        if (wn) hipLaunchKernelGGL((k_g1_fft_stage_quad<DIF, true, 4>), qg, dim3(G1_BLOCK), lds, s, data, logn, m, roots, wnaf, W, total, batch);
-        else hipLaunchKernelGGL((k_g1_fft_stage_quad<DIF, false, 4>), qg, dim3(G1_BLOCK), lds, s, data, logn, m, roots, wnaf, W, total, batch);
+        if (wn) hipLaunchKernelGGL((k_g1_fft_stage_quad<DIF, true, 4>), qg, dim3(G1_BLOCK), lds, s, data, logn, m, roots, wnaf, W, total, batch, toff);
+        else hipLaunchKernelGGL((k_g1_fft_stage_quad<DIF, false, 4>), qg, dim3(G1_BLOCK), lds, s, data, logn, m, roots, wnaf, W, total, batch, toff);
     } else {
-        if (wn) hipLaunchKernelGGL((k_g1_fft_stage_quad<DIF, true, 2>), qg, dim3(G1_BLOCK), lds, s, data, logn, m, roots, wnaf, W, total, batch);
-        else hipLaunchKernelGGL((k_g1_fft_stage_quad<DIF, false, 2>), qg, dim3(G1_BLOCK), lds, s, data, logn, m, roots, wnaf, W, total, batch);
+        if (wn) hipLaunchKernelGGL((k_g1_fft_stage_quad<DIF, true, 2>), qg, dim3(G1_BLOCK), lds, s, data, logn, m, roots, wnaf, W, total, batch, toff);
+        else hipLaunchKernelGGL((k_g1_fft_stage_quad<DIF, false, 2>), qg, dim3(G1_BLOCK), lds, s, data, logn, m, roots, wnaf, W, total, batch, toff);
     }
 }
 template <int L> __global__ __launch_bounds__(G1_DIRECT_BLOCK, 2) void k_g1_fft_direct_coop(const g1j *in, uint64_t in_stride, uint64_t n_valid, g1j *out, uint32_t logn,
diff --git a/go-kzg_amd/csrc/internal.hpp b/go-kzg_amd/csrc/internal.hpp
--- a/go-kzg_amd/csrc/internal.hpp
+++ b/go-kzg_amd/csrc/internal.hpp
@@ -59,19 +59,20 @@
 hipError_t launch_g1_file_msm(hipStream_t s, const g1j *files, const fr *scalars, uint64_t nfiles, uint64_t k2, uint64_t j0, uint64_t cnt,
                               uint64_t batch, g1j *out);
 void launch_g1_bitrev_copy(hipStream_t s, const g1j *in, uint64_t in_stride, uint64_t n_valid, g1j *out, uint64_t n, uint64_t batch);
-void launch_g1_fft_stage(hipStream_t s, g1j *data, uint64_t n, uint64_t batch, uint64_t m, const fr *roots, const int8_t *wnaf, uint64_t W);
+void launch_g1_fft_stage(hipStream_t s, g1j *data, uint64_t n, uint64_t batch, uint64_t m, const fr *roots, const int8_t *wnaf, uint64_t W, uint64_t toff = 0);
 struct g1_stage_plan { int lanes; bool wnaf; bool rows; };
 g1_stage_plan g1_fft_stage_plan(uint64_t n, uint64_t batch, uint64_t m, bool dif, int quad, knobs::g1_mul_mode mul);
 g1_stage_plan g1_fft_stage_plan(uint64_t n, uint64_t batch, uint64_t m, bool dif);
-void launch_g1_fft_stage_planned(hipStream_t s, const g1_stage_plan &plan, bool dif, g1j *data, uint64_t n, uint64_t batch, uint64_t m, const fr *roots, const int8_t *wnaf, uint64_t W);
-void launch_g1_fft_stage_dif(hipStream_t s, g1j *data, uint64_t n, uint64_t batch, uint64_t m, const fr *roots, const int8_t *wnaf, uint64_t W);
+void launch_g1_fft_stage_planned(hipStream_t s, const g1_stage_plan &plan, bool dif, g1j *data, uint64_t n, uint64_t batch, uint64_t m, const fr *roots, const int8_t *wnaf, uint64_t W,
+                                 uint64_t toff = 0);
+void launch_g1_fft_stage_dif(hipStream_t s, g1j *data, uint64_t n, uint64_t batch, uint64_t m, const fr *roots, const int8_t *wnaf, uint64_t W, uint64_t toff = 0);
 void launch_g1_clear_odd(hipStream_t s, g1j *data, uint64_t n_total);
 void launch_g1_take_even(hipStream_t s, const g1j *in, g1j *out, uint64_t total);
 bool g1_quad_enabled();
 void launch_fb_direct_pass1(hipStream_t s, const g1a *table, uint64_t table_n, uint32_t c, uint32_t nwin, const fr *scalars, const fr *roots, uint64_t W, uint64_t batch,
                             uint32_t logR, g1j *out, bool glv = false);
-void launch_g1_stage_coop_dif(hipStream_t s, int lanes, bool wnaf_rows, g1j *data, uint64_t n, uint64_t batch, uint64_t m, const fr *roots, const int8_t *wnaf, uint64_t W, uint64_t total);
-void launch_g1_stage_coop_dit(hipStream_t s, int lanes, bool wnaf_rows, g1j *data, uint64_t n, uint64_t batch, uint64_t m, const fr *roots, const int8_t *wnaf, uint64_t W, uint64_t total);
+void launch_g1_stage_coop_dif(hipStream_t s, int lanes, bool wnaf_rows, g1j *data, uint64_t n, uint64_t batch, uint64_t m, const fr *roots, const int8_t *wnaf, uint64_t W, uint64_t total, uint64_t toff);
+void launch_g1_stage_coop_dit(hipStream_t s, int lanes, bool wnaf_rows, g1j *data, uint64_t n, uint64_t batch, uint64_t m, const fr *roots, const int8_t *wnaf, uint64_t W, uint64_t total, uint64_t toff);
 void launch_g1_direct_coop(hipStream_t s, int lanes, uint32_t wgs, size_t pad_lds, const g1j *src, uint64_t src_stride, uint64_t src_valid, g1j *dst, uint32_t logn, uint32_t logR,
                            uint64_t Ns, const fr *roots, uint64_t W, const fr *sc, uint64_t total, uint32_t logT, uint32_t logU);
 void launch_g1_fft_direct(hipStream_t s, const g1j *in, uint64_t in_stride, uint64_t n_valid, g1j *data, g1j *tmp, uint64_t n, uint64_t batch, const fr *roots,
@@ -112,6 +113,10 @@
                        uint64_t cnt, uint64_t batch, g1j *out, bool glv = false);
 void launch_fb_mul_vec_dif2(hipStream_t s, const g1a *table, uint64_t table_n, uint32_t c, uint32_t nwin, const fr *scalars, const fr *roots, uint64_t W,
                             uint64_t batch, g1j *out, bool glv = false);
+void launch_fb_mul_vec_odd_dif2(hipStream_t s, const g1a *table, uint64_t table_n, uint32_t c, uint32_t nwin, const fr *scalars, const fr *roots, uint64_t W,
+                                uint64_t batch, g1j *out, bool glv = false);
+void launch_fb_add_even(hipStream_t s, const g1a *table, uint64_t table_n, uint32_t c, uint32_t nwin, const fr *scalars, const g1j *t_in, uint64_t batch, int bit_reverse,
+                        g1j *out, bool glv = false);
 void launch_fb_mul_vec_files(hipStream_t s, const g1a *table, uint64_t table_n, uint32_t c, uint32_t nwin, const fr *scalars, uint64_t row, uint64_t j0,
                              uint64_t cnt, uint64_t batch, g1j *out, bool glv = false);
 void launch_g1_sum_files(hipStream_t s, const g1j *tmp, uint64_t nfiles, uint64_t cnt, uint64_t batch, g1j *out);
diff --git a/go-kzg_amd/csrc/k_g1.hip b/go-kzg_amd/csrc/k_g1.hip
--- a/go-kzg_amd/csrc/k_g1.hip
+++ b/go-kzg_amd/csrc/k_g1.hip
@@ -83,21 +83,21 @@
     hipLaunchKernelGGL(k_g1_bitrev_copy, dim3((uint32_t)((total + 255) / 256)), dim3(256), 0, s, in, in_stride, n_valid, out, ilog2(n), total);
 }
 
-template <int MODE, bool PRE = false> __global__ __launch_bounds__(G1_BLOCK, 2) void k_g1_fft_stage(g1j *data, uint32_t logn, uint64_t m, const fr *roots, const int8_t *wnaf, uint64_t W, uint64_t total, uint64_t batch) {
+template <int MODE, bool PRE = false> __global__ __launch_bounds__(G1_BLOCK, 2) void k_g1_fft_stage(g1j *data, uint32_t logn, uint64_t m, const fr *roots, const int8_t *wnaf, uint64_t W, uint64_t total, uint64_t batch, uint64_t toff) {
     uint64_t t = blockIdx.x * (uint64_t)blockDim.x + threadIdx.x;
     if (t >= total) return;
     const uint64_t half = 1ull << (logn - 1), groups = half / m;
     const uint64_t j = t / (groups * batch), rem = t % (groups * batch), b = rem / groups, g = rem % groups;
     g1j *row = data + (b << logn);
     uint64_t i0 = g * 2 * m + j, i1 = i0 + m;
+    const uint64_t ti = j * (W / (2 * m)) + toff;
     g1j y = row[i1];
     g1j x = row[i0];
     if (MODE == 4) {
         g1jq yq; int st = is_inf(y) ? 0 : 1;
         if (st == 1) {
-            if (j) {
+            if (ti) {
                 g1aq tbl[8]; fq dz[7]; g1j packed;
-                const uint64_t ti = j * (W / (2 * m));
                 if (PRE) st = g1_mul_glv_wnaf_aq_pre_q<true, true>(g1jq_unpack(y), roots[ti], tbl, dz, wnaf + ti * KZG_WNAF_ROW, yq, packed);
                 else { int8_t dg1[132], dg2[132]; st = g1_mul_glv_wnaf_aq<true, true>(y, roots[ti], tbl, dz, dg1, dg2, 1, yq, packed); }
                 if (st == 2) y = packed; else if (st == 0) y = g1_inf();
@@ -116,8 +116,8 @@
         }
         if (st == 1) y = g1jq_pack(yq);
     } else {
-        if (j && !is_inf(y)) {
-            const fr kk = roots[j * (W / (2 * m))];
+        if (ti && !is_inf(y)) {
+            const fr kk = roots[ti];
             glv_halves h;
 #pragma unroll
             for (int i = 0; i < 4; i++) { h.k1[i] = kk.l[i]; h.k2[i] = kk.l[4 + i]; }
@@ -148,13 +148,14 @@
     return p;
 }
 g1_stage_plan g1_fft_stage_plan(uint64_t n, uint64_t batch, uint64_t m, bool dif) { return g1_fft_stage_plan(n, batch, m, dif, knobs::g1_quad(), knobs::g1_mul()); }
-template <bool PRE> __global__ __launch_bounds__(G1_BLOCK, 2) void k_g1_fft_stage_dif(g1j *data, uint32_t logn, uint64_t m, const fr *roots, const int8_t *wnaf, uint64_t W, uint64_t total, uint64_t batch) {
+template <bool PRE> __global__ __launch_bounds__(G1_BLOCK, 2) void k_g1_fft_stage_dif(g1j *data, uint32_t logn, uint64_t m, const fr *roots, const int8_t *wnaf, uint64_t W, uint64_t total, uint64_t batch, uint64_t toff) {
     uint64_t t = blockIdx.x * (uint64_t)blockDim.x + threadIdx.x;
     if (t >= total) return;
     const uint64_t half = 1ull << (logn - 1), groups = half / m;
     const uint64_t j = t / (groups * batch), rem = t % (groups * batch), b = rem / groups, g = rem % groups;
     g1j *row = data + (b << logn);
     uint64_t i0 = g * 2 * m + j, i1 = i0 + m;
+    const uint64_t ti = j * (W / (2 * m)) + toff;
     g1j y = row[i1];
     g1j x = row[i0];
     if (!is_inf(x) && !is_inf(y)) {
@@ -162,9 +163,8 @@
         if (KZG_LIKELY(g1jq_addsub(g1jq_unpack(x), g1jq_unpack(y), sum, dif))) {
             g1j o0; o0.x = packq(sum.x); o0.y = packq(sum.y); o0.z = packq(sum.z);
             row[i0] = o0;
-            if (j) {
+            if (ti) {
                 g1aq tbl[8]; fq dz[7]; g1j packed; g1jq dq;
-                const uint64_t ti = j * (W / (2 * m));
                 int st;
                 if (PRE) st = g1_mul_glv_wnaf_aq_pre_q<true, true>(dif, roots[ti], tbl, dz, wnaf + ti * KZG_WNAF_ROW, dq, packed);
                 else { int8_t dg1[132], dg2[132]; st = g1_mul_glv_wnaf_aq_q<true, true>(dif, roots[ti], tbl, dz, dg1, dg2, 1, dq, packed); }
@@ -174,17 +174,16 @@
         }
     }
     g1j s_ = g1_add(x, y), d_ = g1_add(x, g1_neg(y));
-    if (j && !is_inf(d_)) {
+    if (ti && !is_inf(d_)) {
         g1aq tbl[8]; fq dz[7]; g1j packed; g1jq dq;
-        const uint64_t ti = j * (W / (2 * m));
         int8_t dg1[132], dg2[132];
         int st = g1_mul_glv_wnaf_aq<true, true>(d_, roots[ti], tbl, dz, dg1, dg2, 1, dq, packed);
         d_ = st == 1 ? g1jq_pack(dq) : st == 2 ? packed : g1_inf();
     }
     row[i0] = s_; row[i1] = d_;
 }
-void launch_g1_fft_stage_dif(hipStream_t s, g1j *data, uint64_t n, uint64_t batch, uint64_t m, const fr *roots, const int8_t *wnaf, uint64_t W) {
-    launch_g1_fft_stage_planned(s, g1_fft_stage_plan(n, batch, m, true), true, data, n, batch, m, roots, wnaf, W);
+void launch_g1_fft_stage_dif(hipStream_t s, g1j *data, uint64_t n, uint64_t batch, uint64_t m, const fr *roots, const int8_t *wnaf, uint64_t W, uint64_t toff) {
+    launch_g1_fft_stage_planned(s, g1_fft_stage_plan(n, batch, m, true), true, data, n, batch, m, roots, wnaf, W, toff);
 }
 __global__ void k_g1_clear_odd(g1j *data, uint64_t total_pairs) {
     uint64_t t = blockIdx.x * (uint64_t)blockDim.x + threadIdx.x;
@@ -202,28 +201,29 @@
     if (!total) return;
     hipLaunchKernelGGL(k_g1_take_even, dim3((uint32_t)((total + 255) / 256)), dim3(256), 0, s, in, out, total);
 }
-void launch_g1_fft_stage(hipStream_t s, g1j *data, uint64_t n, uint64_t batch, uint64_t m, const fr *roots, const int8_t *wnaf, uint64_t W) {
-    launch_g1_fft_stage_planned(s, g1_fft_stage_plan(n, batch, m, false), false, data, n, batch, m, roots, wnaf, W);
-}
-void launch_g1_fft_stage_planned(hipStream_t s, const g1_stage_plan &plan, bool dif, g1j *data, uint64_t n, uint64_t batch, uint64_t m, const fr *roots, const int8_t *wnaf, uint64_t W) {
+void launch_g1_fft_stage(hipStream_t s, g1j *data, uint64_t n, uint64_t batch, uint64_t m, const fr *roots, const int8_t *wnaf, uint64_t W, uint64_t toff) {
+    launch_g1_fft_stage_planned(s, g1_fft_stage_plan(n, batch, m, false), false, data, n, batch, m, roots, wnaf, W, toff);
+}
+void launch_g1_fft_stage_planned(hipStream_t s, const g1_stage_plan &plan, bool dif, g1j *data, uint64_t n, uint64_t batch, uint64_t m, const fr *roots, const int8_t *wnaf, uint64_t W,
+                                 uint64_t toff) {
     uint64_t total = n / 2 * batch;
     if (!total) return;
     prof_begin(s, "g1_fft_stage");
     if (plan.lanes > 1) {
-        if (dif) launch_g1_stage_coop_dif(s, plan.lanes, plan.wnaf, data, n, batch, m, roots, wnaf, W, total);
-        else launch_g1_stage_coop_dit(s, plan.lanes, plan.wnaf, data, n, batch, m, roots, wnaf, W, total);
+        if (dif) launch_g1_stage_coop_dif(s, plan.lanes, plan.wnaf, data, n, batch, m, roots, wnaf, W, total, toff);
+        else launch_g1_stage_coop_dit(s, plan.lanes, plan.wnaf, data, n, batch, m, roots, wnaf, W, total, toff);
         prof_end(s, "g1_fft_stage");
         return;
     }
     const dim3 grid((uint32_t)((total + G1_BLOCK - 1) / G1_BLOCK)), block(G1_BLOCK);
     const uint32_t logn = ilog2(n);
     if (dif) {
-        if (plan.rows) hipLaunchKernelGGL(k_g1_fft_stage_dif<true>, grid, block, 0, s, data, logn, m, roots, wnaf, W, total, batch);
-        else hipLaunchKernelGGL(k_g1_fft_stage_dif<false>, grid, block, 0, s, data, logn, m, roots, wnaf, W, total, batch);
+        if (plan.rows) hipLaunchKernelGGL(k_g1_fft_stage_dif<true>, grid, block, 0, s, data, logn, m, roots, wnaf, W, total, batch, toff);
+        else hipLaunchKernelGGL(k_g1_fft_stage_dif<false>, grid, block, 0, s, data, logn, m, roots, wnaf, W, total, batch, toff);
     } else if (plan.wnaf) {
-        if (plan.rows) hipLaunchKernelGGL((k_g1_fft_stage<4, true>), grid, block, 0, s, data, logn, m, roots, wnaf, W, total, batch);
-        else hipLaunchKernelGGL((k_g1_fft_stage<4, false>), grid, block, 0, s, data, logn, m, roots, wnaf, W, total, batch);
-    } else hipLaunchKernelGGL(k_g1_fft_stage<0>, grid, block, 0, s, data, logn, m, roots, wnaf, W, total, batch);
+        if (plan.rows) hipLaunchKernelGGL((k_g1_fft_stage<4, true>), grid, block, 0, s, data, logn, m, roots, wnaf, W, total, batch, toff);
+        else hipLaunchKernelGGL((k_g1_fft_stage<4, false>), grid, block, 0, s, data, logn, m, roots, wnaf, W, total, batch, toff);
+    } else hipLaunchKernelGGL(k_g1_fft_stage<0>, grid, block, 0, s, data, logn, m, roots, wnaf, W, total, batch, toff);
     prof_end(s, "g1_fft_stage");
 }
 
diff --git a/go-kzg_amd/csrc/k_g1_coop_dif.hip b/go-kzg_amd/csrc/k_g1_coop_dif.hip
--- a/go-kzg_amd/csrc/k_g1_coop_dif.hip
+++ b/go-kzg_amd/csrc/k_g1_coop_dif.hip
@@ -1,7 +1,7 @@
 #define KZG_MULQ_NOINLINE 1
 #include "g1_coop_kernels.hpp"
 namespace kzg {
-void launch_g1_stage_coop_dif(hipStream_t s, int lanes, bool wnaf_rows, g1j *data, uint64_t n, uint64_t batch, uint64_t m, const fr *roots, const int8_t *wnaf, uint64_t W, uint64_t total) {
-    launch_stage_coop<true>(s, lanes, wnaf_rows, data, n, batch, m, roots, wnaf, W, total);
+void launch_g1_stage_coop_dif(hipStream_t s, int lanes, bool wnaf_rows, g1j *data, uint64_t n, uint64_t batch, uint64_t m, const fr *roots, const int8_t *wnaf, uint64_t W, uint64_t total, uint64_t toff) {
+    launch_stage_coop<true>(s, lanes, wnaf_rows, data, n, batch, m, roots, wnaf, W, total, toff);
 }
 }
diff --git a/go-kzg_amd/csrc/k_g1_coop_dit.hip b/go-kzg_amd/csrc/k_g1_coop_dit.hip
--- a/go-kzg_amd/csrc/k_g1_coop_dit.hip
+++ b/go-kzg_amd/csrc/k_g1_coop_dit.hip
@@ -1,7 +1,7 @@
 #define KZG_MULQ_NOINLINE 1
 #include "g1_coop_kernels.hpp"
 namespace kzg {
-void launch_g1_stage_coop_dit(hipStream_t s, int lanes, bool wnaf_rows, g1j *data, uint64_t n, uint64_t batch, uint64_t m, const fr *roots, const int8_t *wnaf, uint64_t W, uint64_t total) {
-    launch_stage_coop<false>(s, lanes, wnaf_rows, data, n, batch, m, roots, wnaf, W, total);
+void launch_g1_stage_coop_dit(hipStream_t s, int lanes, bool wnaf_rows, g1j *data, uint64_t n, uint64_t batch, uint64_t m, const fr *roots, const int8_t *wnaf, uint64_t W, uint64_t total, uint64_t toff) {
+    launch_stage_coop<false>(s, lanes, wnaf_rows, data, n, batch, m, roots, wnaf, W, total, toff);
 }
 }
diff --git a/go-kzg_amd/csrc/k_msm.hip b/go-kzg_amd/csrc/k_msm.hip
--- a/go-kzg_amd/csrc/k_msm.hip
+++ b/go-kzg_amd/csrc/k_msm.hip
@@ -784,26 +784,27 @@
     prof_end(s, "fb_mul_vec");
 }
 
-template <bool GLV> __global__ __launch_bounds__(FB_BLOCK, 2) void k_fb_mul_vec_dif2(const g1a *table, uint64_t table_n, uint32_t c, uint32_t nwin, uint32_t D, const fr *scalars,
+template <bool GLV, bool ODD> __global__ __launch_bounds__(FB_BLOCK, 2) void k_fb_mul_vec_dif2(const g1a *table, uint64_t table_n, uint32_t c, uint32_t nwin, uint32_t D, const fr *scalars,
                                                               const fr *roots, uint64_t W, uint64_t total, g1j *out) {
     uint64_t t = blockIdx.x * (uint64_t)blockDim.x + threadIdx.x;
     if (t >= total) return;
-    const uint64_t N = table_n, q = N >> 2;
+    const uint64_t N = ODD ? table_n >> 1 : table_n, q = N >> 2;
     const uint64_t i = t % q, o = (t / q) & 3u, b = t / N;
-    const uint64_t rs = W / N;
+    const uint64_t rs = W / table_n;
     g1x_acc acc; acc.init();
 #pragma nounroll
     for (uint32_t pass = GLV ? 0u : 1u; pass < 2; pass++) {
 #pragma nounroll
         for (uint32_t term = 0; term < 4; term++) {
-            const uint64_t pi = i + term * q;
+            const uint64_t pi = ODD ? 2 * (i + term * q) + 1 : i + term * q;
             uint64_t e; uint32_t sg;
             if (o == 0) { e = 0; sg = 0; }
             else if (o == 1) { e = 2 * i; sg = term & 1u; }
             else if (o == 2) { e = i + ((term & 1u) ? q : 0); sg = term >> 1; }
             else { e = 3 * i + ((term & 1u) ? q : 0); sg = (term == 1 || term == 2) ? 1u : 0u; }
-            fr kmont = scalars[b * N + pi];
-            if (e) kmont = mul(kmont, roots[(e & (N - 1)) * rs]);
+            if (ODD) e = 2 * e + (o == 0 ? 0u : o == 1 ? 2u : o == 2 ? 1u : 3u);
+            fr kmont = scalars[b * table_n + pi];
+            if (e) kmont = mul(kmont, roots[(e & (table_n - 1)) * rs]);
             const fr k = from_mont<FrP>(kmont);
             fb_walk_term<GLV>(acc, table, table_n, c, nwin, D, pi, k, sg, pass == 0);
         }
@@ -816,10 +817,47 @@
     uint64_t total = batch * table_n;
     if (!total) return;
     prof_begin(s, "fb_mul_vec");
-    if (glv) hipLaunchKernelGGL(k_fb_mul_vec_dif2<true>, dim3((uint32_t)((total + FB_BLOCK - 1) / FB_BLOCK)), dim3(FB_BLOCK), 0, s, table, table_n, c, nwin, 1u << (c - 1), scalars,
+    if (glv) hipLaunchKernelGGL((k_fb_mul_vec_dif2<true, false>), dim3((uint32_t)((total + FB_BLOCK - 1) / FB_BLOCK)), dim3(FB_BLOCK), 0, s, table, table_n, c, nwin, 1u << (c - 1), scalars,
                                 roots, W, total, out);
-    else hipLaunchKernelGGL(k_fb_mul_vec_dif2<false>, dim3((uint32_t)((total + FB_BLOCK - 1) / FB_BLOCK)), dim3(FB_BLOCK), 0, s, table, table_n, c, nwin, 1u << (c - 1), scalars,
+    else hipLaunchKernelGGL((k_fb_mul_vec_dif2<false, false>), dim3((uint32_t)((total + FB_BLOCK - 1) / FB_BLOCK)), dim3(FB_BLOCK), 0, s, table, table_n, c, nwin, 1u << (c - 1), scalars,
                             roots, W, total, out);
+    prof_end(s, "fb_mul_vec");
+}
+void launch_fb_mul_vec_odd_dif2(hipStream_t s, const g1a *table, uint64_t table_n, uint32_t c, uint32_t nwin, const fr *scalars, const fr *roots, uint64_t W,
+                                uint64_t batch, g1j *out, bool glv) {
+    uint64_t total = batch * (table_n / 2);
+    if (!total) return;
+    prof_begin(s, "fb_mul_vec");
+    if (glv) hipLaunchKernelGGL((k_fb_mul_vec_dif2<true, true>), dim3((uint32_t)((total + FB_BLOCK - 1) / FB_BLOCK)), dim3(FB_BLOCK), 0, s, table, table_n, c, nwin, 1u << (c - 1), scalars,
+                                roots, W, total, out);
+    else hipLaunchKernelGGL((k_fb_mul_vec_dif2<false, true>), dim3((uint32_t)((total + FB_BLOCK - 1) / FB_BLOCK)), dim3(FB_BLOCK), 0, s, table, table_n, c, nwin, 1u << (c - 1), scalars,
+                            roots, W, total, out);
+    prof_end(s, "fb_mul_vec");
+}
+template <bool GLV> __global__ __launch_bounds__(FB_BLOCK, 2) void k_fb_add_even(const g1a *table, uint64_t table_n, uint32_t c, uint32_t nwin, uint32_t D, const fr *scalars,
+                                                          const g1j *t_in, uint32_t logn, int bit_reverse, uint64_t total, g1j *out) {
+    uint64_t t = blockIdx.x * (uint64_t)blockDim.x + threadIdx.x;
+    if (t >= total) return;
+    const uint64_t N = table_n >> 1, j = t & (N - 1), b = t >> logn, pi = 2 * j;
+    fr nn = zero<FrP>(); nn.l[0] = (uint32_t)N; nn.l[1] = (uint32_t)(N >> 32);
+    const fr k = mul(scalars[b * table_n + pi], nn);
+    g1x_acc acc; acc.init();
+    if (GLV) { fb_walk_term<true>(acc, table, table_n, c, nwin, D, pi, k, 0u, true); acc_apply_phi(acc); }
+    fb_walk_term<GLV>(acc, table, table_n, c, nwin, D, pi, k, 0u, false);
+    const uint64_t oj = bit_reverse ? (uint64_t)(__brev((uint32_t)j) >> (32 - logn)) : j;
+    out[b * N + oj] = g1_add(t_in[t], acc.to_jac());
+}
+void launch_fb_add_even(hipStream_t s, const g1a *table, uint64_t table_n, uint32_t c, uint32_t nwin, const fr *scalars, const g1j *t_in, uint64_t batch, int bit_reverse,
+                        g1j *out, bool glv) {
+    const uint64_t N = table_n / 2, total = batch * N;
+    if (!total) return;
+    uint32_t logn = 0;
+    while ((1ull << logn) < N) logn++;
+    prof_begin(s, "fb_mul_vec");
+    if (glv) hipLaunchKernelGGL(k_fb_add_even<true>, dim3((uint32_t)((total + FB_BLOCK - 1) / FB_BLOCK)), dim3(FB_BLOCK), 0, s, table, table_n, c, nwin, 1u << (c - 1), scalars, t_in,
+                                logn, bit_reverse, total, out);
+    else hipLaunchKernelGGL(k_fb_add_even<false>, dim3((uint32_t)((total + FB_BLOCK - 1) / FB_BLOCK)), dim3(FB_BLOCK), 0, s, table, table_n, c, nwin, 1u << (c - 1), scalars, t_in,
+                            logn, bit_reverse, total, out);
     prof_end(s, "fb_mul_vec");
 }
 template <bool GLV> __global__ __launch_bounds__(FB_BLOCK, 2) void k_fb_mul_vec_files(const g1a *table, uint64_t table_n, uint32_t c, uint32_t nwin, uint32_t D, const fr *scalars,
diff --git a/go-kzg_amd/csrc/knobs.hpp b/go-kzg_amd/csrc/knobs.hpp
--- a/go-kzg_amd/csrc/knobs.hpp
+++ b/go-kzg_amd/csrc/knobs.hpp
@@ -58,7 +58,8 @@
 KZG_KNOB_ONCE(bool, coop_inv, "KZG_HIP_COOP_INV", !starts(e, '0'))
 KZG_KNOB_ONCE(bool, fk20_pass1, "KZG_HIP_FK20_PASS1", !starts(e, '0'))
 KZG_KNOB_ONCE(bool, fk20_fuse, "KZG_HIP_FK20_FUSE", !starts(e, '0'))
-KZG_KNOB_ONCE(bool, fk20_pad, "KZG_HIP_FK20_PAD", !starts(e, '0'))
+KZG_KNOB_ONCE(bool, fk20_half, "KZG_HIP_FK20_HALF", !starts(e, '0'))
+KZG_KNOB_ONCE(bool, fk20_pad,"KZG_HIP_FK20_PAD", !starts(e, '0'))
 KZG_KNOB_PER_CALL(bool, eth_prove_overlap, "KZG_HIP_ETH_PROVE_OVERLAP", !starts(e, '0'))
 KZG_KNOB_ONCE(bool, coalesce_trace, "KZG_HIP_COALESCE_TRACE", e != nullptr)
 KZG_KNOB_PER_CALL(bool, coalesce_stats, "KZG_HIP_COALESCE_STATS", e != nullptr)
diff --git a/go-kzg_amd/csrc/kzg_hip_internal.h b/go-kzg_amd/csrc/kzg_hip_internal.h
--- a/go-kzg_amd/csrc/kzg_hip_internal.h
+++ b/go-kzg_amd/csrc/kzg_hip_internal.h
@@ -39,6 +39,8 @@
 int kzg_hip_test_g1_fft_plan(kzg_hip_fft *fs, uint64_t n, uint64_t batch, uint64_t m, int dif, uint32_t out[5]);
 int kzg_hip_test_g1_fft_stage(kzg_hip_fft *fs, const void *pts_g1, uint64_t n, uint64_t batch, uint64_t m, int inv, int dif, int lanes, int mul, void *out_g1,
                               uint32_t plan_out[3]);
+int kzg_hip_test_g1_fft_stage_toff(kzg_hip_fft *fs, const void *pts_g1, uint64_t n, uint64_t batch, uint64_t m, uint64_t toff, int inv, int dif, int lanes, int mul,
+                                   void *out_g1, uint32_t plan_out[3]);
 int kzg_hip_test_g1_fft_direct(kzg_hip_fft *fs, const void *pts_g1, uint64_t n, uint64_t n_valid, uint64_t batch, int inv, uint32_t max_logr, int lanes, uint64_t n_out,
                                void *out_g1);
 
```
